# facebookresearch/gtn

Measured on AMD Instinct MI355X. Metric: CTC forward+backward losses/sec (T=1000, C=256), higher is better.
Workload: dtype f32; 1 GPU; BASELINE config C3: compose(ctc_target, emissions)+forwardScore CTC loss fwd+bwd, T=1000, C=256, U=100, batch=512 per GPU; global_batch=512, parallelism=dp1 (utterance sharding, all_gather of losses), rccl_ranks=0

## Files before the change

### gtn_amd/__init__.py

```python
from . import _capi
from .api import make_api, load_txt as _load_txt

_lib = _capi.load()
_api = make_api(_lib)

Graph = _api.Graph
Batch = _api.Batch
epsilon = _api.epsilon
negate = _api.negate
add = _api.add
subtract = _api.subtract
subtract_into = getattr(_api, "subtract_into", None)
compose = _api.compose
intersect = _api.intersect
forward_score = _api.forward_score
viterbi_score = _api.viterbi_score
viterbi_path = _api.viterbi_path
backward = _api.backward
scalar_graph = _api.scalar_graph
linear_graph = _api.linear_graph
linear_graph_n = _api.linear_graph_n
equal = _api.equal
isomorphic = _api.isomorphic
items = _api.items
items_to_device = _api.items_to_device
grads_to_device = _api.grads_to_device
parallel_for = _api.parallel_for
clone = _api.clone
project_input = _api.project_input
project_output = _api.project_output
closure = _api.closure
concat = _api.concat
union = _api.union
remove = _api.remove
sample = _api.sample
rand_equivalent = _api.rand_equivalent
load = _api.load
save = _api.save
loadtxt = _api.loadtxt
savetxt = _api.savetxt
write_dot = _api.write_dot
draw = _api.draw
backend = _api.backend
device_count = _api.device_count
synchronize = _api.synchronize
set_device = _api.set_device
set_stream = _api.set_stream
compose_mode = _api.compose_mode
memory_stats = _api.memory_stats
empty_cache = _api.empty_cache
prof_enable = _api.prof_enable
prof_reset = _api.prof_reset
prof_get = _api.prof_get
prof_names = _api.prof_names
debug_symbolic_route = _api.debug_symbolic_route
debug_viterbi_ties = _api.debug_viterbi_ties
debug_tie_ranks = _api.debug_tie_ranks
debug_align_stats = getattr(_api, "debug_align_stats", None)


def load_txt(text):
    return _load_txt(_api, text)


__version__ = _lib.gtnx_version().decode()


def _shutdown():
    try:
        _lib.gtnx_set_stream(None)
        _lib.gtnx_synchronize()
        _lib.gtnx_empty_cache()
    except Exception:
        pass


import atexit as _atexit

_atexit.register(_shutdown)
```

### gtn_amd/_capi.py

```python
import ctypes as C
import os

c_graph = C.c_void_p
c_graph_p = C.POINTER(C.c_void_p)
c_i32_p = C.POINTER(C.c_int)
c_i64_p = C.POINTER(C.c_int64)
c_u8_p = C.POINTER(C.c_uint8)
c_f32_p = C.POINTER(C.c_float)

GRAD_FN = C.CFUNCTYPE(C.c_int, C.c_void_p, c_graph_p, C.c_int, c_graph)
CTX_FREE = C.CFUNCTYPE(None, C.c_void_p)

OK, INVALID_ARGUMENT, LOGIC_ERROR, RUNTIME_ERROR, OUT_OF_RANGE, DEVICE_ERROR = range(6)

_SIGS = {
    "gtnx_set_device": [C.c_int],
    "gtnx_get_device": [c_i32_p],
    "gtnx_set_stream": [C.c_void_p],
    "gtnx_compose_mode": [C.c_int, C.POINTER(C.c_int)],
    "gtnx_synchronize": [],
    "gtnx_memory_stats": [C.POINTER(C.c_uint64), C.POINTER(C.c_uint64)],
    "gtnx_empty_cache": [],
    "gtnx_reclaim": [],
    "gtnx_graph_create": [C.c_int, c_graph_p],
# ... 41 lines not shown
    "gtnx_graph_id": [c_graph, C.POINTER(C.c_size_t)],
    "gtnx_graph_create_op": [c_graph_p, C.c_int, GRAD_FN, C.c_void_p, CTX_FREE, c_graph_p],
    "gtnx_graph_num_inputs": [c_graph, c_i64_p],
    "gtnx_graph_get_input": [c_graph, C.c_int, c_graph_p],
    "gtnx_graph_set_inputs": [c_graph, c_graph_p, C.c_int],
    "gtnx_graph_set_grad_fn": [c_graph, GRAD_FN, C.c_void_p, CTX_FREE],
    "gtnx_graph_has_grad_fn": [c_graph, c_i32_p],
    "gtnx_scalar_graph": [C.c_float, C.c_int, c_graph_p],
    "gtnx_linear_graph": [C.c_int, C.c_int, C.c_int, c_graph_p],
    "gtnx_linear_graph_n": [C.c_int, C.c_int, C.c_int, C.c_int, C.c_void_p, c_graph_p],
    "gtnx_linear_graph_borrow_n": [C.c_int, C.c_int, C.c_int, C.c_int, C.c_void_p, c_graph_p],
    "gtnx_negate": [c_graph, c_graph_p],
    "gtnx_add": [c_graph, c_graph, c_graph_p],
    "gtnx_subtract": [c_graph, c_graph, c_graph_p],
    "gtnx_compose": [c_graph, c_graph, c_graph_p],
    "gtnx_intersect": [c_graph, c_graph, c_graph_p],
    "gtnx_forward_score": [c_graph, c_graph_p],
    "gtnx_viterbi_score": [c_graph, c_graph_p],
    "gtnx_viterbi_path": [c_graph, c_graph_p],
    "gtnx_negate_n": [c_graph_p, C.c_int, c_graph_p],
    "gtnx_add_n": [c_graph_p, C.c_int, c_graph_p, C.c_int, c_graph_p],
    "gtnx_subtract_n": [c_graph_p, C.c_int, c_graph_p, C.c_int, c_graph_p],
    "gtnx_compose_n": [c_graph_p, C.c_int, c_graph_p, C.c_int, c_graph_p],
    "gtnx_intersect_n": [c_graph_p, C.c_int, c_graph_p, C.c_int, c_graph_p],
    "gtnx_forward_score_n": [c_graph_p, C.c_int, c_graph_p],
    "gtnx_viterbi_score_n": [c_graph_p, C.c_int, c_graph_p],
    "gtnx_viterbi_path_n": [c_graph_p, C.c_int, c_graph_p],
    "gtnx_items_n": [c_graph_p, C.c_int, C.c_void_p],
    "gtnx_items_device_n": [c_graph_p, C.c_int, C.c_void_p],
    "gtnx_grads_device_n": [c_graph_p, C.c_int, C.c_void_p, C.c_void_p],
    "gtnx_grads_bind_device_n": [c_graph_p, C.c_int, C.c_void_p, C.c_void_p],
    "gtnx_clone": [c_graph, C.c_int, c_graph_p],
    "gtnx_concat": [c_graph_p, C.c_int, c_graph_p],
    "gtnx_closure": [c_graph, c_graph_p],
    "gtnx_union": [c_graph_p, C.c_int, c_graph_p],
    "gtnx_batch_from_graphs": [c_graph_p, C.c_int, c_graph_p],
    "gtnx_batch_ctc_targets": [C.c_void_p, C.c_void_p, C.c_int, C.c_int, C.c_int, c_graph_p],
    "gtnx_batch_asg_force_align": [C.c_void_p, C.c_void_p, C.c_int, c_graph, C.c_int, c_graph_p],
    "gtnx_batch_linear": [C.c_int, C.c_int, C.c_int, C.c_int, C.c_void_p, C.c_int, c_graph_p],
    "gtnx_batch_destroy": [c_graph],
    "gtnx_batch_size": [c_graph, c_i32_p],
    "gtnx_batch_get": [c_graph, C.c_int, c_graph_p],
    "gtnx_batch_negate": [c_graph, c_graph_p],
    "gtnx_batch_add": [c_graph, c_graph, c_graph_p],
    "gtnx_batch_subtract": [c_graph, c_graph, c_graph_p],
    "gtnx_batch_subtract_into": [c_graph, c_graph, C.c_void_p, c_graph_p],
    "gtnx_batch_compose": [c_graph, c_graph, c_graph_p],
    "gtnx_batch_intersect": [c_graph, c_graph, c_graph_p],
    "gtnx_batch_forward_score": [c_graph, c_graph_p],
    "gtnx_batch_viterbi_score": [c_graph, c_graph_p],
    "gtnx_batch_viterbi_path": [c_graph, c_graph_p],
    "gtnx_batch_viterbi_align": [c_graph, C.c_void_p, C.c_void_p, C.c_int64, C.c_void_p, C.c_void_p],
    "gtnx_batch_align_stats": [c_i64_p, c_i64_p],
    "gtnx_batch_backward": [c_graph, C.c_int],
    "gtnx_batch_items": [c_graph, C.c_void_p],
    "gtnx_batch_items_device": [c_graph, C.c_void_p],
    "gtnx_batch_grads_bind_device": [c_graph, C.c_void_p, C.c_void_p],
    "gtnx_batch_grads_device": [c_graph, C.c_void_p, C.c_void_p],
    "gtnx_backward": [c_graph, C.c_int],
    "gtnx_backward_with_grad": [c_graph, c_graph, C.c_int],
    "gtnx_backward_n": [c_graph_p, C.c_int, C.c_int],
    "gtnx_equal": [c_graph, c_graph, c_i32_p],
    "gtnx_isomorphic": [c_graph, c_graph, c_i32_p],
    "gtnx_remove": [c_graph, C.c_int, C.c_int, c_graph_p],
    "gtnx_graph_load_buffer": [C.c_void_p, C.c_size_t, c_graph_p],
    "gtnx_parallel_enter": [],
    "gtnx_parallel_leave": [],
    "gtnx_parallel_flush": [],
    "gtnx_prof_enable": [C.c_int],
    "gtnx_prof_reset": [],
    "gtnx_prof_get": [C.c_char_p, C.POINTER(C.c_double), c_i64_p, C.POINTER(C.c_double)],
    "gtnx_prof_names": [C.c_char_p, C.c_size_t],
    "gtnx_debug_symbolic_route": [c_graph, C.c_int, c_i32_p],
    "gtnx_debug_route_name": [C.c_int, C.c_char_p, C.c_size_t],
    "gtnx_debug_viterbi_ties": [c_i64_p, c_i64_p],
    "gtnx_debug_tie_ranks": [c_graph, C.c_void_p, C.c_void_p, C.c_void_p],
    "gtnx_comm_create": [c_i32_p, C.c_int, C.POINTER(C.c_void_p)],
    "gtnx_comm_destroy": [C.c_void_p],
    "gtnx_comm_size": [C.c_void_p, c_i32_p],
    "gtnx_comm_all_gather_f32": [C.c_void_p, C.POINTER(C.c_void_p), C.POINTER(C.c_void_p), C.c_int64],
    "gtnx_comm_all_reduce_sum_f32": [C.c_void_p, C.POINTER(C.c_void_p), C.c_int64],
}

_RESTYPE = {
    "gtnx_last_error": (C.c_char_p, []),
    "gtnx_version": (C.c_char_p, []),
    "gtnx_backend": (C.c_char_p, []),
    "gtnx_device_count": (C.c_int, []),
}

ALL_SYMBOLS = sorted(list(_SIGS) + list(_RESTYPE))


def default_library_path():
    return os.path.join(os.path.dirname(os.path.abspath(__file__)), "lib", "libgtn_amd.so")


def load(path=None):
    path = path or default_library_path()
    if not os.path.exists(path):
        raise ImportError(
            f"gtn_amd: native library not found at {path}. Build it with "
            "`python -c 'import __graft_entry__ as g; g.build()'` (hipcc, gfx950). "
            "There is no CPU fallback."
        )
    lib = C.CDLL(path, mode=C.RTLD_GLOBAL if hasattr(C, "RTLD_GLOBAL") else 0)
# ... 17 lines not shown
```

### gtn_amd/api.py

```python
import ctypes as C
import types

import numpy as np

from . import _capi

_EXC = {
    _capi.INVALID_ARGUMENT: ValueError,
    _capi.LOGIC_ERROR: RuntimeError,
    _capi.RUNTIME_ERROR: RuntimeError,
    _capi.OUT_OF_RANGE: IndexError,
    _capi.DEVICE_ERROR: RuntimeError,
}


class GtnError(RuntimeError):
    pass


def _is_seq(x):
    return isinstance(x, (list, tuple))


def make_api(lib):
# ... 635 lines not shown

        def viterbi_align(self, labels_out, tokens_out=None, scores_out=None, frames=None, row_stride=None):
            n = len(self)
            stride = row_stride
            for t in (labels_out, tokens_out):
                if t is None or not hasattr(t, "data_ptr"):
                    continue
                if t.element_size() != 4 or t.dim() != 2 or t.shape[0] < n or (t.shape[1] > 1 and t.stride(1) != 1):
                    raise ValueError("viterbi_align: outputs must be int32 tensors [B, T] with contiguous rows")
                if stride is not None and t.stride(0) != stride:
                    raise ValueError("viterbi_align: labels_out and tokens_out must have the same row stride")
                stride = t.stride(0)
            if stride is None:
                raise ValueError("viterbi_align: a device address needs row_stride")
            fr = None if frames is None else np.ascontiguousarray(frames, dtype=np.int32)
            if fr is not None and fr.shape != (n,):
                raise ValueError("viterbi_align: one frame count per element")
            check(lib.gtnx_batch_viterbi_align(self._h, fr.ctypes.data if fr is not None else None,
                                               _as_dev_ptr(labels_out), int(stride),
                                               _as_dev_ptr(tokens_out) if tokens_out is not None else None,
                                               _as_dev_ptr(scores_out) if scores_out is not None else None))

    ns.Batch = Batch

    def _batch_fn(cfn, *args):
        h = C.c_void_p()
        check(cfn(*[a._h for a in args], C.byref(h)))
        return Batch._from_handle(h.value)

    def _with_batches(plain, cfn):
        def f(*args, **kw):
            if args and all(isinstance(a, Batch) for a in args) and not kw:
                return _batch_fn(cfn, *args)
            return plain(*args, **kw)
        f.__doc__ = plain.__doc__
        f.__name__ = getattr(plain, "__name__", "f")
        return f

    if hasattr(lib, "gtnx_batch_negate"):
        for _name in ("negate", "add", "subtract", "compose", "intersect", "forward_score", "viterbi_score",
                      "viterbi_path"):
            setattr(ns, _name, _with_batches(getattr(ns, _name), getattr(lib, "gtnx_batch_" + _name)))

    def subtract_into(a, b, items_device):
        h = C.c_void_p()
        check(lib.gtnx_batch_subtract_into(a._h, b._h, _as_dev_ptr(items_device), C.byref(h)))
        r = Batch._from_handle(h.value)
        r._keep = items_device
        return r

    if hasattr(lib, "gtnx_batch_subtract_into"):
        ns.subtract_into = subtract_into

    _plain_backward = ns.backward

    def backward(g, grad_or_retain=None, retain_graph=False):
        if isinstance(g, Batch):
            r = grad_or_retain if isinstance(grad_or_retain, bool) else retain_graph
            check(lib.gtnx_batch_backward(g._h, int(bool(r))))
            return
        return _plain_backward(g, grad_or_retain, retain_graph)

    ns.backward = backward

    def parallel_for(fn, iterable):
        for i in iterable:
            fn(i)

    ns.parallel_for = parallel_for

    def backend():
        return lib.gtnx_backend().decode()

    def device_count():
        return lib.gtnx_device_count()

    def synchronize():
        check(lib.gtnx_synchronize())

    def set_device(i):
        check(lib.gtnx_set_device(int(i)))

    def set_stream(stream):
        check(lib.gtnx_set_stream(int(stream) if stream else None))

    def compose_mode(mode):
        prev = C.c_int()
        check(lib.gtnx_compose_mode(int(mode), C.byref(prev)))
        return prev.value

    def memory_stats():
        r, u = C.c_uint64(), C.c_uint64()
        check(lib.gtnx_memory_stats(C.byref(r), C.byref(u)))
        return {"reserved": r.value, "in_use": u.value}

    def prof_enable(on=True):
        check(lib.gtnx_prof_enable(int(bool(on))))

    def prof_reset():
        check(lib.gtnx_prof_reset())

    def prof_get(name):
        ms, n, b = C.c_double(), C.c_int64(), C.c_double()
        check(lib.gtnx_prof_get(name.encode(), C.byref(ms), C.byref(n), C.byref(b)))
        return {"total_ms": ms.value, "launches": n.value, "algorithmic_bytes": b.value}

# ... 74 lines not shown
```

### gtn_amd/criteria/ctc_criterion.h

```cpp
#pragma once

#include <chrono>
#include <cstdint>
#include <vector>

#include "gtn/gtn.h"

namespace gtn {
namespace criteria {

inline Graph ctcTargetGraph(const std::vector<int>& target, int blank = 0, bool calcGrad = true) {
  const int L = 2 * (int)target.size() + 1;
  std::vector<uint8_t> st(L, 0), ac(L, 0);
  std::vector<int> src, dst, lab;
  src.reserve(3 * L);
  dst.reserve(3 * L);
  lab.reserve(3 * L);
  for (int l = 0; l < L; l++) {
    const int idx = (l - 1) / 2;
    st[l] = l == 0;
    ac[l] = l == L - 1 || l + 2 == L;
    const int label = l % 2 ? target[idx] : blank;
    src.push_back(l), dst.push_back(l), lab.push_back(label);
    if (l > 0) src.push_back(l - 1), dst.push_back(l), lab.push_back(label);
    if (l % 2 && l > 1 && label != target[idx - 1]) src.push_back(l - 2), dst.push_back(l), lab.push_back(label);
  }
  Graph ctc(calcGrad);
  detail::check(gtnx_graph_add_nodes(ctc.handle(), L, st.data(), ac.data()));
  detail::check(gtnx_graph_add_arcs(ctc.handle(), (int)src.size(), src.data(), dst.data(), lab.data(), lab.data(), nullptr));
  ctc.arcSort();
  return ctc;
}

struct CtcStepTimes {
  double build = 0, linear = 0, intersect = 0, forward = 0, backward = 0;
};

inline void ctcLossBatch(
    const void* emissions,
    const int* labels,
    const int* lengths,
    int B,
    int T,
    int C,
    int blank,
    void* lossDev,
    void* gradDev,
    bool targetGrad = true,
    CtcStepTimes* times = nullptr,
    Batch* targetsOut = nullptr) {
  auto now = [] { return std::chrono::steady_clock::now(); };
  auto ms = [](auto a, auto b) { return std::chrono::duration<double, std::milli>(b - a).count(); };
  auto t0 = now();
  Batch ctcs = Batch::ctcTargets(labels, lengths, B, blank, targetGrad);
  auto t1 = now();
  Batch ems = Batch::linear(B, T, C, emissions, gradDev != nullptr, true);
  std::vector<int64_t> off(B);
  for (int b = 0; b < B; ++b) off[b] = (int64_t)b * T * C;
  if (gradDev) ems.bindGrads(gradDev, off.data());
  auto t2 = now();
  Batch comp = batched::intersect(ctcs, ems);
  auto t3 = now();
  Batch score = batched::forwardScore(comp);
  Batch norm = batched::forwardScore(ems);
  Batch losses = batched::subtract(norm, score, lossDev);
  auto t4 = now();
  if (gradDev) batched::backward(losses);
  auto t5 = now();
  if (times) *times = {ms(t0, t1), ms(t1, t2), ms(t2, t3), ms(t3, t4), ms(t4, t5)};
  losses.itemsToDevice(lossDev);
  if (gradDev) ems.gradsToDevice(gradDev, off.data());
  if (targetsOut) *targetsOut = std::move(ctcs);
}

inline void ctcLossBatch(
    const void* emissions,
    const std::vector<std::vector<int>>& targets,
    int T,
    int C,
    int blank,
    void* lossDev,
    void* gradDev,
    bool targetGrad = true,
    CtcStepTimes* times = nullptr) {
  std::vector<int> flat, len;
  for (auto& t : targets) {
    flat.insert(flat.end(), t.begin(), t.end());
    len.push_back((int)t.size());
  }
  ctcLossBatch(emissions, flat.data(), len.data(), (int)targets.size(), T, C, blank, lossDev, gradDev, targetGrad, times);
}

inline void ctcAlignBatch(
    const void* emissions,
    const int* targets,
    const int* lengths,
    int B,
    int T,
    int C,
    int blank,
    const int* frames,
    void* labels,
    void* tokens,
    void* scores) {
  Batch ctcs = Batch::ctcTargets(targets, lengths, B, blank, false);
  Batch ems = Batch::linear(B, T, C, emissions, false, true);
  Batch comp = batched::intersect(ctcs, ems);
  batched::viterbiAlign(comp, static_cast<int*>(labels), T, static_cast<int*>(tokens), static_cast<float*>(scores), frames);
}

}
}
```

### gtn_amd/csrc/band.hip

```cpp
#include <hip/hip_runtime.h>

#include <algorithm>
#include <cstdlib>
#include <stdexcept>
#include <type_traits>

#include "kernels.h"

#ifdef GTNX_BAND_TIMING
__device__ long long g_band_timing[256];
#endif

namespace gtnx {
namespace {

constexpr float NEGF = -1.0e30f;
constexpr float DEADF = -1.0e29f;
constexpr float LOG2E = 1.44269504088896340736f;
constexpr double LN2 = 0.693147180559945309417;
constexpr int BW = 256;
constexpr int WG = 512;
constexpr int WGB = 768;
constexpr int NBE = 5;
constexpr int NBG = 7;
// ... 256 lines not shown
        }
      }
    }
  }
};

struct BandLds {
  int CS;
  int o_ering, o_aring, o_oring, o_snode, o_misc, total;
};
__host__ __device__ inline BandLds band_lds(int C, int K, int NSmax, bool backward) {
  BandLds L;
  L.CS = C + 4;
  int o = 0;
  L.o_ering = o;
  o += (backward ? NBGE : NBE) * K * L.CS;
  o = (o + 3) & ~3;
  L.o_aring = o;
  o += backward ? NBE * K * NSmax : 0;
  o = (o + 3) & ~3;
  L.o_oring = o;
  o += backward ? max(NBG * K * NSmax, 2 * C) : 0;
  o = (o + 3) & ~3;
  L.o_snode = o;
  o += backward ? 512 : 0;
  L.o_misc = o;
  o += 160 + 32 + 8 + 2 * NBE * K * 4 + 40 * K + 8 + 512;
  L.total = o;
  return L;
}
struct BandMisc {
  double *offr, *red, *find, *aofr;
  float *bndr, *fin, *lsep;
};
template <int K>
__device__ __forceinline__ BandMisc band_misc(float* lds, const BandLds& L) {
  BandMisc m;
  m.offr = reinterpret_cast<double*>(lds + L.o_misc);
  m.red = m.offr + 80;
  m.find = m.red + 16;
  m.aofr = m.find + 4;
  m.bndr = lds + L.o_misc + 200 + 2 * NBE * K * 4;
  m.fin = m.bndr + 40 * K;
  m.lsep = m.fin + 8;
  return m;
}

__device__ __forceinline__ float wave_max_of(const float* v, int n) {
  float mx = v[0];
  for (int j = 1; j < n; ++j) mx = fmaxf(mx, v[j]);
  return wave_max(mx);
}

template <int NPL, bool UNIT, int K, bool VEC>
__global__ __launch_bounds__(WG) void band_forward_kernel(const BandPair* __restrict__ pairs, int NSmax) {
#define GTNX_BAND_PAIR pairs[blockIdx.x]
#include "band_forward_body.inc"
#undef GTNX_BAND_PAIR
}
template <int NPL, bool UNIT, int K, bool VEC>
__global__ __launch_bounds__(WG) void band_forward_one_kernel(BandPair one, int NSmax) {
#define GTNX_BAND_PAIR one
#include "band_forward_body.inc"
#undef GTNX_BAND_PAIR
}

__device__ __forceinline__ BandPair band_patched(BandPair P, const BandPatch& pt) {
  if (pt.on) {
    const int b = P.bidx;
    P.delta = pt.delta + b;
    P.delta_norm = pt.delta_norm ? pt.delta_norm + b : nullptr;
    P.rowlse = pt.rowlse ? pt.rowlse + int64_t(b) * pt.M : nullptr;
    P.norm = nullptr;
    P.em_copy = nullptr;
    P.grad_em = pt.grad_em ? pt.grad_em + int64_t(b) * pt.A : nullptr;
    P.grad_fixed = pt.grad_fixed ? pt.grad_fixed + P.goff : nullptr;
  }
  return P;
}
template <int NPL, bool UNIT, bool GRADG, int K, bool VEC, bool BIG>
__global__ __launch_bounds__(WGB, BIG ? 3 : 6) void band_backward_kernel(const BandPair* __restrict__ pairs, int NSmax, BandPatch patch) {
#define GTNX_BAND_PAIR band_patched(pairs[blockIdx.x], patch)
#include "band_backward_body.inc"
#undef GTNX_BAND_PAIR
}
template <int NPL, bool UNIT, bool GRADG, int K, bool VEC, bool BIG>
__global__ __launch_bounds__(WGB, BIG ? 3 : 6) void band_backward_one_kernel(BandPair one, int NSmax) {
#define GTNX_BAND_PAIR one
#include "band_backward_body.inc"
#undef GTNX_BAND_PAIR
}


__global__ __launch_bounds__(512) void ctc_targets_kernel(const CtcTargetArgs* __restrict__ args, int blank) {
  const CtcTargetArgs a = args[blockIdx.x];
  __shared__ __attribute__((aligned(16))) int tl[256 + 4];
  __shared__ __attribute__((aligned(16))) int tk[256 + 4];
  const int N = a.N, U = (N - 1) >> 1, m = threadIdx.x;
  if (m < 260) {
    const int v = m < U ? a.labels[m] : 0x7fffffff;
    tl[m] = v;
    tk[m] = (m > 0 && m < U && v != a.labels[m - 1]) ? 1 : 0;
  }
  __syncthreads();
  if (m >= N) return;
  const bool odd = (m & 1) != 0;
  const int my = odd ? tl[(m - 1) >> 1] : blank;
  const int skip = odd ? tk[(m - 1) >> 1] : 0;
  const int mi = (m - 1) >> 1;
  const int before = odd ? mi : (m >> 1);
  int rank = 0, skips = 0;
  for (int o = 0; o < U; o += 4) {
    const gtnx_i4 l4 = *reinterpret_cast<const gtnx_i4*>(tl + o), k4 = *reinterpret_cast<const gtnx_i4*>(tk + o);
    const int lo[4] = {l4.x, l4.y, l4.z, l4.w}, ko[4] = {k4.x, k4.y, k4.z, k4.w};
#pragma unroll
    for (int k = 0; k < 4; ++k) {
      const bool front = o + k < before;
      rank += (lo[k] < my || (lo[k] == my && front)) ? 1 : 0;
      skips += front ? ko[k] : 0;
    }
  }
  rank += blank < my ? U + 1 : (blank == my ? (m + 1) >> 1 : 0);
  const int base = (m > 0 ? 2 * m - 1 : 0) + skips;
  GTNX_G BandNode* nd = const_cast<GTNX_G BandNode*>(a.nodes);
  nd[m].lab = my;
  nd[m].aid[0] = base;
  nd[m].aid[1] = m > 0 ? base + 1 : -1;
  nd[m].aid[2] = skip ? base + 2 : -1;
  a.nflags[m] = uint8_t((m == 0 ? NF_START : 0) | (m + 2 >= N ? NF_ACCEPT : 0));
  a.snode[rank] = m;
  a.slab[rank] = my;
  if (m == N - 1 && a.n_arcs) a.n_arcs[0] = base + 1 + (m > 0 ? 1 : 0) + skip;
}

__global__ __launch_bounds__(512) void band_viterbi_kernel(const BandDecode* __restrict__ pairs) {
  const BandDecode P = pairs[blockIdx.x];
  const int T = P.T, C = P.C, N = P.N, NS = P.NS;
  extern __shared__ float lds[];
  const float NINF = -__builtin_inff();
  float* a0 = lds;
  float* a1 = lds + 516;
  float* stage = lds + 1032;
  const int m = threadIdx.x;
  const GTNX_G gtnx_i4* nodes = reinterpret_cast<const GTNX_G gtnx_i4*>(P.nodes);
  int lab = 0;
  float wi[3] = {NINF, NINF, NINF};
  bool accept = false, start = false;
  if (m < N) {
    const gtnx_i4 q = nodes[m];
    lab = q.x >= 0 ? q.x : 0;
    const int a[3] = {q.y, q.z, q.w};
#pragma unroll
    for (int k = 0; k < 3; ++k)
      if (a[k] >= 0) wi[k] = P.w ? P.w[a[k]] : 0.0f;
    const uint8_t f = P.nflags[m];
    start = (f & NF_START) != 0;
    accept = (f & NF_ACCEPT) != 0;
  }
  if (m < 2) a0[m] = a1[m] = NINF;
  a0[2 + m] = start ? 0.0f : NINF;
  a1[2 + m] = NINF;
  int tie = 0;
  const int R = max(1, min(64, P.stage_floats / C));
  float* cur = a0;
  float* nxt = a1;
  __syncthreads();
  for (int t0 = 0; t0 < T; t0 += R) {
    const int rows = min(R, T - t0);
    for (int e = threadIdx.x; e < rows * C; e += blockDim.x) stage[e] = P.em[int64_t(t0) * C + e];
    __syncthreads();
    for (int i = 0; i < rows; ++i) {
      const float e = stage[i * C + lab];
      const float c0 = cur[2 + m] + (wi[0] + e), c1 = cur[1 + m] + (wi[1] + e), c2 = cur[m] + (wi[2] + e);
      float best = c0;
      int k = 0;
      if (c1 > best) best = c1, k = 1;
      if (c2 > best) best = c2, k = 2;
      if (best > NINF && ((k != 0 && c0 == best) || (k != 1 && c1 == best) || (k != 2 && c2 == best))) tie = 1;
      if (m < NS) P.bp[int64_t(t0 + i) * NS + m] = uint8_t(best > NINF ? k : 3);
      nxt[2 + m] = m < N ? best : NINF;
      __syncthreads();
      float* sw = cur;
      cur = nxt;
      nxt = sw;
    }
  }
// ... 292 lines not shown
    P.path_arc[t] = arc;
    P.path_lab[t] = q.x;
    P.path_w[t] = (arc >= 0 && P.w ? P.w[arc] : 0.0f) + P.em[int64_t(t) * C + (q.x >= 0 ? q.x : 0)];
  }
}

__global__ __launch_bounds__(512) void asg_fal_targets_kernel(const AsgFalArgs* __restrict__ args, int NL) {
  const AsgFalArgs a = args[blockIdx.x];
  __shared__ int lab[512];
  const int U = a.U, m = threadIdx.x;
  int my = -1;
  if (m >= 1 && m <= U) my = a.labels[m - 1];
  lab[m] = my;
  __syncthreads();
  if (m > U) return;
  GTNX_G BandNode* nd = const_cast<GTNX_G BandNode*>(a.nodes);
  nd[m].lab = my;
  nd[m].aid[0] = m >= 1 ? 2 * m - 1 : -1;
  nd[m].aid[1] = m >= 1 ? 2 * m - 2 : -1;
  nd[m].aid[2] = -1;
  a.nflags[m] = uint8_t((m == 0 ? NF_START : 0) | (m == U ? NF_ACCEPT : 0));
  if (m >= 1) {
    int rank = 0;
    for (int o = 1; o <= U; ++o) {
      const int lo = lab[o];
      rank += (lo < my || (lo == my && o < m)) ? 1 : 0;
    }
    a.snode[rank] = m;
    a.slab[rank] = my;
    const int step = m == 1 ? my : NL + my * NL + lab[m - 1];
    const int self = NL + my * NL + my;
    a.arc_map[2 * m - 2] = step;
    a.arc_map[2 * m - 1] = self;
    a.w[2 * m - 2] = a.trans_w[step];
    a.w[2 * m - 1] = a.trans_w[self];
  }
}
__global__ void asg_fal_scatter_kernel(const float* __restrict__ g, const int* __restrict__ maps,
                                       const int64_t* __restrict__ tab, float* __restrict__ trans_grad) {
  const int64_t* e = tab + int64_t(blockIdx.y) * 3;
  const int64_t n = e[2];
  const float* gb = g + e[0];
  const int* mb = maps + e[1];
  for (int64_t i = int64_t(blockIdx.x) * blockDim.x + threadIdx.x; i < n; i += int64_t(gridDim.x) * blockDim.x)
    if (mb[i] >= 0 && gb[i] != 0.0f) atomicAdd(trans_grad + mb[i], gb[i]);
}

template <class K>
void big_lds(K kern) {
  (void)hipFuncSetAttribute(reinterpret_cast<const void*>(kern), hipFuncAttributeMaxDynamicSharedMemorySize, 160 * 1024 - 512);
}

template <int NPL, int K, bool VEC>
void launch_fwd2(const BandPair* d, const BandPair* one, int n, int ns, size_t lds, bool unit, hipStream_t st) {
  static std::atomic<uint64_t> done{0};
  if (gtnx_first_on_device first{done}) {
    big_lds(band_forward_kernel<NPL, true, K, VEC>);
    big_lds(band_forward_kernel<NPL, false, K, VEC>);
    if constexpr (NPL == 1 && VEC) {
      big_lds(band_forward_one_kernel<NPL, true, K, VEC>);
      big_lds(band_forward_one_kernel<NPL, false, K, VEC>);
    }
  }
  if constexpr (NPL == 1 && VEC) {
    if (one) {
      if (unit) hipLaunchKernelGGL((band_forward_one_kernel<NPL, true, K, VEC>), dim3(1), dim3(WG), lds, st, *one, ns);
      else hipLaunchKernelGGL((band_forward_one_kernel<NPL, false, K, VEC>), dim3(1), dim3(WG), lds, st, *one, ns);
      return;
    }
  }
  if (unit) hipLaunchKernelGGL((band_forward_kernel<NPL, true, K, VEC>), dim3(n), dim3(WG), lds, st, d, ns);
  else hipLaunchKernelGGL((band_forward_kernel<NPL, false, K, VEC>), dim3(n), dim3(WG), lds, st, d, ns);
}
template <int NPL, int K>
void launch_fwd(const BandPair* d, const BandPair* one, int n, int ns, size_t lds, bool unit, bool vec, hipStream_t st) {
  if (vec) launch_fwd2<NPL, K, true>(d, one, n, ns, lds, unit, st);
  else launch_fwd2<NPL, K, false>(d, one, n, ns, lds, unit, st);
}
template <int NPL, int K, bool VEC, bool BIG>
void launch_bwd3(const BandPair* d, const BandPair* one, int n, int ns, size_t lds, bool unit, bool gradg, hipStream_t st,
                 const BandPatch& pt) {
  constexpr bool ONE = NPL == 1 && VEC && !BIG;
  static std::atomic<uint64_t> done{0};
  if (gtnx_first_on_device first{done}) {
    big_lds(band_backward_kernel<NPL, true, true, K, VEC, BIG>);
    big_lds(band_backward_kernel<NPL, true, false, K, VEC, BIG>);
    big_lds(band_backward_kernel<NPL, false, true, K, VEC, BIG>);
    big_lds(band_backward_kernel<NPL, false, false, K, VEC, BIG>);
    if constexpr (ONE) {
      big_lds(band_backward_one_kernel<NPL, true, true, K, VEC, BIG>);
      big_lds(band_backward_one_kernel<NPL, true, false, K, VEC, BIG>);
      big_lds(band_backward_one_kernel<NPL, false, true, K, VEC, BIG>);
      big_lds(band_backward_one_kernel<NPL, false, false, K, VEC, BIG>);
    }
  }
  if constexpr (ONE) {
    if (one) {
      if (unit) {
        if (gradg) hipLaunchKernelGGL((band_backward_one_kernel<NPL, true, true, K, VEC, BIG>), dim3(1), dim3(WGB), lds, st, *one, ns);
        else hipLaunchKernelGGL((band_backward_one_kernel<NPL, true, false, K, VEC, BIG>), dim3(1), dim3(WGB), lds, st, *one, ns);
      } else {
        if (gradg) hipLaunchKernelGGL((band_backward_one_kernel<NPL, false, true, K, VEC, BIG>), dim3(1), dim3(WGB), lds, st, *one, ns);
        else hipLaunchKernelGGL((band_backward_one_kernel<NPL, false, false, K, VEC, BIG>), dim3(1), dim3(WGB), lds, st, *one, ns);
      }
      return;
    }
  }
  if (unit) {
    if (gradg) hipLaunchKernelGGL((band_backward_kernel<NPL, true, true, K, VEC, BIG>), dim3(n), dim3(WGB), lds, st, d, ns, pt);
    else hipLaunchKernelGGL((band_backward_kernel<NPL, true, false, K, VEC, BIG>), dim3(n), dim3(WGB), lds, st, d, ns, pt);
  } else {
    if (gradg) hipLaunchKernelGGL((band_backward_kernel<NPL, false, true, K, VEC, BIG>), dim3(n), dim3(WGB), lds, st, d, ns, pt);
    else hipLaunchKernelGGL((band_backward_kernel<NPL, false, false, K, VEC, BIG>), dim3(n), dim3(WGB), lds, st, d, ns, pt);
  }
}
template <int NPL, int K>
void launch_bwd(const BandPair* d, const BandPair* one, int n, int ns, size_t lds, bool unit, bool gradg, bool vec, bool big,
                hipStream_t st, const BandPatch& pt) {
  if constexpr (K == 2) {
    if (big) {
      if (vec) launch_bwd3<NPL, K, true, true>(d, one, n, ns, lds, unit, gradg, st, pt);
      else launch_bwd3<NPL, K, false, true>(d, one, n, ns, lds, unit, gradg, st, pt);
      return;
    }
  }
  if (vec) launch_bwd3<NPL, K, true, false>(d, one, n, ns, lds, unit, gradg, st, pt);
  else launch_bwd3<NPL, K, false, false>(d, one, n, ns, lds, unit, gradg, st, pt);
}

constexpr size_t LDS_TWO = 78 * 1024;
constexpr size_t LDS_ONE = 156 * 1024;

}

int band_block_rows(int C, int max_NS, bool backward);
static int band_backward_lds_stride(int K, int max_NS) { return K == 4 ? (max_NS + 15) / 16 * 16 : max_NS; }
int band_max_nodes() { return 512; }
int band_max_labels() { return 1024; }
int band_min_labels() { return 4; }
int band_npl(int max_nodes) { return max_nodes <= 256 ? 1 : 2; }
int band_row_stride(int N, int) { return (N + 3) / 4 * 4; }
#ifndef GTNX_FWD_SHIFT_ROWS
#define GTNX_FWD_SHIFT_ROWS 4
#endif
int band_forward_lgrn(int C) {
  const int K = band_block_rows(C, 0, false);
  return K >= GTNX_FWD_SHIFT_ROWS ? (GTNX_FWD_SHIFT_ROWS == 8 ? 3 : 2) : (K >= 4 ? 2 : 1);
}
int band_block_rows(int C, int max_NS, bool backward) {
  for (int k = backward ? 4 : 8; k >= 2; k /= 2) {
    if (k * C > 2048 || k * max_NS > 2048) continue;
    if (backward && k > 2 && (k * C > 1024 || k * max_NS > 1024)) continue;
    const int ns_lds = backward ? band_backward_lds_stride(k, max_NS) : max_NS;
    if (4 * size_t(band_lds(C, k, ns_lds, backward).total) + 64 <= LDS_TWO) return k;
  }
  if (4 * size_t(band_lds(C, 2, max_NS, backward).total) + 64 <= LDS_ONE) return 2;
  return 0;
}

bool band_one_ok(int npl, int C, int max_NS, bool vec, bool backward) {
  if (npl != 1 || !vec) return false;
  if (!backward) return true;
  const int K = band_block_rows(C, max_NS, true);
  return !(K * C > 1024 || K * max_NS > 1024);
}
void launch_band_forward(const BandPair* d_pairs, int n, int npl, int C, int max_NS, bool unit, bool vec, hipStream_t st,
                         const BandPair* one) {
  if (n <= 0) return;
  if (one && (n != 1 || !band_one_ok(npl, C, max_NS, vec, false))) throw std::logic_error("band.hip: not a single-pair launch");
  const int K = band_block_rows(C, 0, false);
  const size_t lds = 4 * size_t(band_lds(C, K, max_NS, false).total) + 64;
  if (npl == 1) {
    if (K == 8) launch_fwd<1, 8>(d_pairs, one, n, max_NS, lds, unit, vec, st);
    else if (K == 4) launch_fwd<1, 4>(d_pairs, one, n, max_NS, lds, unit, vec, st);
    else launch_fwd<1, 2>(d_pairs, one, n, max_NS, lds, unit, vec, st);
  } else {
    if (K == 8) launch_fwd<2, 8>(d_pairs, one, n, max_NS, lds, unit, vec, st);
    else if (K == 4) launch_fwd<2, 4>(d_pairs, one, n, max_NS, lds, unit, vec, st);
    else launch_fwd<2, 2>(d_pairs, one, n, max_NS, lds, unit, vec, st);
  }
}

void launch_band_backward(const BandPair* d_pairs, int n, int npl, int C, int max_NS, bool unit, bool gradg, bool vec,
                          hipStream_t st, const BandPair* one, const BandPatch* patch) {
  if (n <= 0) return;
  if (one && patch) throw std::logic_error("band.hip: a patched launch reads a device table");
  BandPatch pt{};
  if (patch) pt = *patch;
  if (one && (n != 1 || !band_one_ok(npl, C, max_NS, vec, true))) throw std::logic_error("band.hip: not a single-pair launch");
  const int K = band_block_rows(C, max_NS, true);
  const bool big = K * C > 1024 || K * max_NS > 1024;
  const int ns_lds = band_backward_lds_stride(K, max_NS);
  const size_t lds = 4 * size_t(band_lds(C, K, ns_lds, true).total) + 64;
  if (npl == 1) {
    if (K == 4) launch_bwd<1, 4>(d_pairs, one, n, ns_lds, lds, unit, gradg, vec, big, st, pt);
    else launch_bwd<1, 2>(d_pairs, one, n, ns_lds, lds, unit, gradg, vec, big, st, pt);
  } else {
    if (K == 4) throw std::logic_error("band.hip: four rows per block with two nodes per lane");
    launch_bwd<2, 2>(d_pairs, one, n, ns_lds, lds, unit, gradg, vec, big, st, pt);
  }
}

template <int NPL>
static void launch_viterbi_wave(const BandDecode* d_pairs, int n, int ranked, hipStream_t st) {
  if (ranked) hipLaunchKernelGGL((band_viterbi_wave_kernel<NPL, true>), dim3(n), dim3(64), 0, st, d_pairs);
  else hipLaunchKernelGGL((band_viterbi_wave_kernel<NPL, false>), dim3(n), dim3(64), 0, st, d_pairs);
}
bool band_viterbi_wave_ok(int max_nodes, int max_labels, int vec) {
  static const bool force_wg = std::getenv("GTNX_VITERBI_WG") != nullptr;
  return !force_wg && vec && max_nodes <= 512 && max_labels <= VBLK;
}
void launch_band_viterbi(const BandDecode* d_pairs, int n, int stage_floats, int max_nodes, int max_labels, int vec,
                         hipStream_t st, int ranked) {
  if (n <= 0) return;
  if (band_viterbi_wave_ok(max_nodes, max_labels, vec)) {
    if (max_nodes <= 64) launch_viterbi_wave<1>(d_pairs, n, ranked, st);
    else if (max_nodes <= 128) launch_viterbi_wave<2>(d_pairs, n, ranked, st);
    else if (max_nodes <= 256) launch_viterbi_wave<4>(d_pairs, n, ranked, st);
    else launch_viterbi_wave<8>(d_pairs, n, ranked, st);
    return;
  }
  if (ranked) return;
  static std::atomic<uint64_t> done{0};
  if (gtnx_first_on_device first{done}) big_lds(band_viterbi_kernel);
  hipLaunchKernelGGL(band_viterbi_kernel, dim3(n), dim3(512), 4 * size_t(1032 + stage_floats) + 64, st, d_pairs);
}

void launch_asg_fal_targets(const AsgFalArgs* d_args, int n, int n_labels, hipStream_t st) {
  if (n > 0) hipLaunchKernelGGL(asg_fal_targets_kernel, dim3(n), dim3(512), 0, st, d_args, n_labels);
}
void launch_asg_fal_scatter(const float* g, const int* maps, const int64_t* tab, int n_seq, int64_t longest, float* trans_grad,
                            hipStream_t st) {
// ... 10 lines not shown
```

### gtn_amd/csrc/band_backward_body.inc

```
  constexpr int RNk = K >= 4 ? 4 : K;
  constexpr int NP = K / RNk;
  const BandPair P = GTNX_BAND_PAIR;
  const int T = P.T, C = P.C, NS = P.NS;
  extern __shared__ float lds[];
  const BandLds L = band_lds(C, K, NSmax, true);
  float* ering = lds + L.o_ering;
  float* aring = lds + L.o_aring;
  float* oring = lds + L.o_oring;
  int* snode = reinterpret_cast<int*>(lds + L.o_snode);
  const BandMisc M = band_misc<K>(lds, L);
  float* lser = M.lsep;
  const int CS = L.CS;
  const int wv = __builtin_amdgcn_readfirstlane(threadIdx.x >> 6);
  const bool sweeper = wv < 4;
  const int l = threadIdx.x & 63;
  const int nblocks = (T + K - 1) / K;
  const int nticks = nblocks + 5;
  const GTNX_G double* ao = P.aoff;
  const double z2 = uniform(ao[0]);
  const bool dead = !(z2 > double(DEADF));
  const float ds = uniform(P.delta[0]);
  const bool want_em = P.grad_em != nullptr;
  GTNX_TM_INIT(128);
  constexpr bool SPLIT = !BIG && K >= 2 && GTNX_BWD_SPLIT;
  const float dn_k = P.delta_norm ? uniform(P.delta_norm[0]) : 0.0f;
  float* const rnorm_k = lser + NBG * K;
  auto rows_of_k = [&](int c) { return c < nblocks ? min(K, T - c * K) : 0; };
  auto ring_start = [](int c, int M) { return ((c % M) + M) % M; };
  static_assert((NBGE & (NBGE - 1)) == 0, "the emission ring's position is a mask");
  auto ge_of = [](int c) { return int(unsigned(c) & unsigned(NBGE - 1)); };
  auto ring_step = [](int& v, int M) { v = v + 1 == M ? 0 : v + 1; };
  struct RowSumRegs {
    float in[NPL];
    gtnx_f4 hot[NPL];
  };
  auto rowsum_init = [&](RowSumRegs& R) {
#pragma unroll
    for (int q = 0; q < NPL; ++q) {
      const int mb = 256 * q + 4 * l;
      R.in[q] = mb < NSmax ? 1.0f : 0.0f;
      float hm[4];
#pragma unroll
      for (int k = 0; k < 4; ++k) {
        const int m = mb + k;
        int lab = -1;
        if (m < P.N) lab = P.nodes[m].lab;
        settle(lab);
        hm[k] = (P.hot >= 0 && lab == P.hot) ? 1.0f : 0.0f;
      }
      R.hot[q] = gtnx_f4{hm[0], hm[1], hm[2], hm[3]};
    }
  };
  auto rowsum_do = [&](const RowSumRegs& R, int c, int cg , int r, auto steady_tag) -> float {
    constexpr bool STEADY = decltype(steady_tag)::value;
    if (!want_em || (K < 4 && r >= K)) return 0.0f;
    if constexpr (!STEADY) {
      if (r >= rows_of_k(c)) return 0.0f;
    }
    const bool dead_r = STEADY ? false : dead;
    const float* ob = oring + (cg * K + r) * NSmax;
    gtnx_f4 v[NPL];
#pragma unroll
    for (int q = 0; q < NPL; ++q) v[q] = *reinterpret_cast<const gtnx_f4*>(ob + min(256 * q + 4 * l, NSmax - 4));
    const float em_hot = ering[(ge_of(c) * K + r) * CS + max(P.hot, 0)];
    const float ls_hot = lser[cg * K + r];
    float all = (v[0].x * R.in[0] + v[0].y * R.in[0]) + (v[0].z * R.in[0] + v[0].w * R.in[0]);
    float hotp = (v[0].x * R.hot[0].x + v[0].y * R.hot[0].y) + (v[0].z * R.hot[0].z + v[0].w * R.hot[0].w);
#pragma unroll
    for (int q = 1; q < NPL; ++q) {
      all += (v[q].x * R.in[q] + v[q].y * R.in[q]) + (v[q].z * R.in[q] + v[q].w * R.in[q]);
      hotp += (v[q].x * R.hot[q].x + v[q].y * R.hot[q].y) + (v[q].z * R.hot[q].z + v[q].w * R.hot[q].w);
    }
    if (dead_r) all = hotp = 0.0f;
    wave_sum63x2(all, hotp);
    all = __int_as_float(__builtin_amdgcn_readlane(__float_as_int(all), 63));
    const bool have = all != 0.0f && !dead_r;
    const float f = have ? ds * __builtin_amdgcn_rcpf(all) : 1.0f;
    if (l == 63 && P.hot >= 0) {
// ... 349 lines not shown
            if (FULL || i < rows) {
#pragma unroll
              for (int j = 0; j < NPL; ++j) ob[i * NSmax + j] = postv[i][j];
            }
        }
        if (GRADG) {
#pragma unroll
          for (int j = 0; j < NPL; ++j)
#pragma unroll
            for (int k = 0; k < 3; ++k) acc[k][j] += accb[k][j] * gscale;
        }
        if (NPL == 1 ? l < 2 : l == 0) {
#pragma unroll
          for (int i = 0; i < K; ++i)
            if (FULL || i < rows) {
              float* bp = bnd_own + ((beta & 3) * K + i) * 2;
              if (NPL == 1) {
                bp[l] = qh[i][0];
              } else {
                bp[0] = qh[i][0];
                bp[1] = qh[i][NPL - 1];
              }
            }
        }
      };
      if constexpr (STEADY) {
        block(std::true_type{});
      } else if (beta >= 0 && beta < nblocks && !dead) {
        if (beta * K + K <= T) block(std::true_type{});
        else block(std::false_type{});
      }
      GTNX_TM(5);
      lds_barrier();
      GTNX_TM(6);
      GTNX_TM_TICK();
    };
    {
      const int s0 = min(RS4 ? 5 : 4, nticks), s1 = dead ? s0 : max(s0, min(nticks, T / K + lag));
      auto step_rings = [&]() { ring_step(bm5, NBE), ring_step(bm7, NBG), ring_step(rm7, NBG); };
      int tau = 0;
      for (; tau < s0; ++tau, step_rings()) tick(tau, std::false_type{});
      for (; tau < s1; ++tau, step_rings()) tick(tau, std::true_type{});
      for (; tau < nticks; ++tau, step_rings()) tick(tau, std::false_type{});
    }
    GTNX_TM_DUMP();
    if (GRADG && P.grad_fixed) {
#pragma unroll
      for (int j = 0; j < NPL; ++j)
#pragma unroll
        for (int k = 0; k < 3; ++k)
          if (g.ao[k][j] >= 0) P.grad_fixed[g.ao[k][j]] = dead ? 0.0f : acc[k][j];
    }
  } else if (wv < 8) {
    const bool soft = P.delta_norm != nullptr && P.rowlse != nullptr;
    lds_barrier();
    if constexpr (!BIG) {
      const int h = wv - 4, q = h & 1;
      auto rows_of = [&](int c) { return c < nblocks ? min(K, T - c * K) : 0; };
      auto tlo_of = [&](int c) { return T - c * K - rows_of(c); };
      DrainRegs dr_s;
      const int hid_s = threadIdx.x - BW;
      auto drain_upper = [&](int tau) {
        if constexpr (SPLIT) {
          if (tau >= 5) drain_block(dr_s, hid_s, tau - 5, (tau - 5) % NBG, std::integral_constant<int, KH>{}, std::integral_constant<int, K>{});
        }
      };
      if (h < 2) {
        Stage<16, 64> se;
        if constexpr (VEC) se.init_offsets(C, CS, K, l);
        auto issue_em = [&](int c, auto steady_tag) {
          constexpr bool ST = decltype(steady_tag)::value;
          const int rows = ST ? K : rows_of(c);
          se.template issue<VEC>(P.em + int64_t(T - c * K - rows) * C, rows * C, l);
        };
        auto land_em = [&](int c, auto steady_tag) {
          constexpr bool ST = decltype(steady_tag)::value;
          const int rows = ST ? K : rows_of(c);
          se.settle_all();
          GTNX_TM(4);
          if (rows <= 0) return;
          float* eb = ering + ge_of(c) * K * CS;
          if constexpr (VEC) {
            se.each_vec(rows * C, (K - rows) * CS, l, [&](int, int o, gtnx_f4 v4) {
              typedef float f2v __attribute__((ext_vector_type(2)));
              const f2v lo = f2v{v4.x, v4.y} * LOG2E, hi = f2v{v4.z, v4.w} * LOG2E;
              *reinterpret_cast<gtnx_f4*>(eb + o) = gtnx_f4{fmaxf(lo.x, NEGF), fmaxf(lo.y, NEGF), fmaxf(hi.x, NEGF), fmaxf(hi.y, NEGF)};
            });
          } else {
            se.template each<false>(rows * C, C, l, [&](int, int, int r, int col, gtnx_f4 v4) {
              eb[(rows - 1 - r) * CS + col] = em2(v4.x);
            });
          }
        };
        issue_em(q, std::false_type{});
        land_em(q, std::false_type{});
        issue_em(q + 2, std::false_type{});
        RowSum4Regs rs4;
        if constexpr (RS4) rowsum4_init(rs4);
        lds_barrier();
        if constexpr (SPLIT) drain_init(dr_s, hid_s);
        lds_barrier();
        int r7 = ring_start(-4, NBG);
        auto tick = [&](int tau, auto steady_tag) {
          constexpr bool ST = decltype(steady_tag)::value;
          GTNX_TM(0);
#ifndef GTNX_EXP_NO_STAGE
          if (((tau + 2) & 1) == q) {
// ... 107 lines not shown
      float* eb = ering + ge_of(c) * K * CS;
      if constexpr (VEC) {
        se.each_vec(rows * C, (K - rows) * CS, l, [&](int, int o, gtnx_f4 q) {
          *reinterpret_cast<gtnx_f4*>(eb + o) = gtnx_f4{em2(q.x), em2(q.y), em2(q.z), em2(q.w)};
        });
      } else {
        se.template each<false>(rows * C, C, l, [&](int, int, int r, int col, gtnx_f4 q) {
          eb[(rows - 1 - r) * CS + col] = em2(q.x);
        });
      }
    };
    auto land_rest = [&](int c) {
      const int rows = rows_of(c);
      sa.settle_all();
      asm volatile("" : "+v"(lse_s), "+v"(af_s));
      if (rows <= 0) return;
      float* ab = aring + (c % NBE) * K * NSmax;
      sa.each_vec(rows * NS, (K - rows) * NSmax, l, [&](int, int o, gtnx_f4 q) { *reinterpret_cast<gtnx_f4*>(ab + o) = q; });
      if (l < rows) lser[(c % NBG) * K + rows - 1 - l] = lse_s;
      if (l < 4 * rows) M.aofr[((c % NBE) * K) * 4 + l] = af_s;
    };
    issue(h);
    if (h == 0) {
      land_em(0);
      land_rest(0);
      issue(4);
    }
    if (h == 1) land_em(1);
    lds_barrier();
    lds_barrier();
    for (int tau = 0; tau < nticks; ++tau) {
      GTNX_TM(0);
#ifndef GTNX_EXP_NO_STAGE
      if (((tau + 1) & 3) == h) {
        land_rest(tau + 1);
        GTNX_TM(1);
        issue(tau + 5);
        GTNX_TM(2);
      }
      if (((tau + 2) & 3) == h) {
        land_em(tau + 2);
        GTNX_TM(1);
      }
#endif
      GTNX_TM(3);
      lds_barrier();
      GTNX_TM(6);
      GTNX_TM_TICK();
    }
    GTNX_TM_DUMP();
    }
  } else {
    const int hid = threadIdx.x - 2 * BW;
    const bool soft = P.delta_norm != nullptr && P.rowlse != nullptr;
    int* cls = reinterpret_cast<int*>(oring);
    for (int c = hid; c < 2 * C; c += BW) cls[c] = 0;
    lds_barrier();
    for (int i = hid; i < P.n_lab; i += BW) {
      const int lab = P.slab[i];
      snode[i] = P.snode[i];
      if (i == 0 || P.slab[i - 1] != lab) cls[lab] = i;
      if (i == P.n_lab - 1 || P.slab[i + 1] != lab) cls[C + lab] = i + 1;
    }
    lds_barrier();
    DrainRegs dr;
    drain_init(dr, hid);
    RowSumRegs rsr;
    if constexpr (SPLIT) rowsum_init(rsr);
    const int dw = wv - 8;
    lds_barrier();
    int d7 = ring_start(-5, NBG);
    for (int tau = 0; tau < nticks; ++tau, ring_step(d7, NBG)) {
      GTNX_TM(0);
#ifndef GTNX_EXP_NO_DRAIN
      if (tau >= 5) drain_block(dr, hid, tau - 5, d7, std::integral_constant<int, 0>{}, std::integral_constant<int, KH>{});
#endif
      if constexpr (SPLIT) {
        if (tau >= 4) rowsum_do(rsr, tau - 4, (tau - 4) % NBG, dw, std::false_type{});
      }
      GTNX_TM(3);
      lds_barrier();
      GTNX_TM(6);
      GTNX_TM_TICK();
    }
    GTNX_TM_DUMP();
  }
```

### gtn_amd/csrc/band_forward_body.inc

```
#ifndef GTNX_FWD_SHIFT_ROWS
#define GTNX_FWD_SHIFT_ROWS 4
#endif
  constexpr int RNk = K >= GTNX_FWD_SHIFT_ROWS ? GTNX_FWD_SHIFT_ROWS : (K >= 4 ? 4 : K);
  constexpr int NP = K / RNk;
  constexpr int D = 8 / K > GTNX_FWD_DEPTH ? 8 / K : GTNX_FWD_DEPTH;
  const BandPair P = GTNX_BAND_PAIR;
  const int T = P.T, C = P.C, NS = P.NS;
  extern __shared__ float lds[];
  const BandLds L = band_lds(C, K, NSmax, false);
  float* ering = lds + L.o_ering;
  const BandMisc M = band_misc<K>(lds, L);
  const int CS = L.CS;
  const int wv = __builtin_amdgcn_readfirstlane(threadIdx.x >> 6);
  const bool sweeper = wv < 4;
  const int l = threadIdx.x & 63;
  const int nblocks = (T + K - 1) / K;
  const int nticks = nblocks + 3;
  GTNX_TM_INIT(0);

  if (sweeper) {
    __builtin_amdgcn_s_setprio(1);
    const int w = wv;
    const int m0 = threadIdx.x * NPL;
    NodeRegs<NPL> g;
// ... 279 lines not shown
      constexpr int DC = GTNX_FWD_COPY_DEPTH < 8 / K ? 8 / K : GTNX_FWD_COPY_DEPTH;
      constexpr int R = DC + 1;
      Stage<8> sc[R];
      issue(sc[0], 0);
      land(sc[0], 0, 0, std::true_type{});
#pragma unroll
      for (int c = 1; c <= DC; ++c) issue(sc[c % R], c);
      lds_barrier();
      int t5 = 0;
      for (int tau0 = 0; tau0 < nticks; tau0 += R) {
#pragma unroll
        for (int d = 0; d < R; ++d) {
          const int tau = tau0 + d;
          if (tau >= nticks) break;
          GTNX_TM(0);
          const int n5 = t5 + 1 == NBE ? 0 : t5 + 1;
          sc[(d + 1) % R].settle_all();
          issue(sc[d % R], tau + 1 + DC);
          GTNX_TM(2);
          land(sc[(d + 1) % R], tau + 1, n5, std::true_type{});
          GTNX_TM(1);
          if (want_lse) {
            if (tau >= 1 && tau - 1 < nblocks) lse_b(tau - 1);
            if (tau < nblocks) lse_a(tau, t5);
          }
          t5 = n5;
          GTNX_TM(4);
          lds_barrier();
          GTNX_TM(6);
          GTNX_TM_TICK();
        }
      }
    };
    if (em_copy) {
      if (GTNX_FWD_COPY_ROTATE) run_copy();
      else run(std::true_type{});
    } else {
      run(std::false_type{});
    }
    if (hid < 16) M.red[hid] = normacc;
  }
  GTNX_TM_DUMP();
  lds_barrier();
  if (threadIdx.x == 0) {
    double Mx = double(NEGF);
    for (int k = 0; k < 4; ++k)
      if (M.fin[2 * k] > DEADF) Mx = fmax(Mx, M.find[k] + double(M.fin[2 * k]));
    const bool dead = !(Mx > double(DEADF));
    float S = 0.0f;
    for (int k = 0; k < 4; ++k)
      if (M.fin[2 * k] > DEADF) S += M.fin[2 * k + 1] * ex2(float(M.find[k] + double(M.fin[2 * k]) - Mx));
    const double z2 = dead ? double(NEGF) : Mx + double(lg2(S));
    P.aoff[0] = z2;
    P.score[0] = dead ? -__builtin_inff() : float(z2 * LN2);
    if (P.norm) {
      double n2 = 0.0;
      for (int k = 0; k < 16; ++k) n2 += M.red[k];
      P.norm[0] = n2 < double(DEADF) ? -__builtin_inff() : float(n2 * LN2);
    }
  }
```

### gtn_amd/csrc/batch.cpp

```cpp
#include "batch.h"

#include <algorithm>
#include <atomic>
#include <limits>
#include <unordered_map>
#include <unordered_set>

namespace gtnx {

namespace {

std::atomic<uint64_t> g_batch_seq{1};

struct CompMode {
  int old;
  CompMode() : old(compose_mode_hint(2)) {}
  ~CompMode() { compose_mode_hint(old); }
};

BatchP make_batch(Batch::Kind k, int n, bool cg) {
  auto b = std::make_shared<Batch>();
  b->kind = k;
  b->n = n;
  b->calc_grad = cg;
// ... 15 lines not shown
  Runtime& rt = Runtime::get();
  b.g_off.resize(size_t(b.n) + 1);
  b.g_off[0] = 0;
  for (int i = 0; i < b.n; ++i) b.g_off[size_t(i) + 1] = b.g_off[size_t(i)] + b.elem_size(i);
  const size_t bytes = sizeof(float) * size_t(b.g_off[size_t(b.n)]);
  if (b.dest) {
    b.g_mem = b.dest_mem;
    b.g_dev = b.dest;
    b.dest = nullptr;
    if (zero && bytes) HIP_CHECK(hipMemsetAsync(b.g_dev, 0, bytes, rt.stream()));
  } else {
    b.g_mem = zero ? rt.alloc_zero(bytes ? bytes : 4) : rt.alloc(bytes ? bytes : 4);
    b.g_dev = b.g_mem->as<float>();
  }
}

struct GradTarget {
  float* ptr = nullptr;
  DevMemP scratch;
};
GradTarget grad_target(Batch& b, bool zero) {
  GradTarget t;
  if (!b.g_dev) {
    alloc_grad(b, zero);
    t.ptr = b.g_dev;
    return t;
  }
  Runtime& rt = Runtime::get();
  const size_t bytes = sizeof(float) * size_t(b.g_off[size_t(b.n)]);
  t.scratch = zero ? rt.alloc_zero(bytes ? bytes : 4) : rt.alloc(bytes ? bytes : 4);
  t.ptr = t.scratch->as<float>();
  return t;
}
void add_scratch(Batch& b, const GradTarget& t) {
  if (!t.scratch) return;
  launch_vec_axpby(b.g_dev, t.ptr, nullptr, size_t(b.g_off[size_t(b.n)]), 1.0f, 0.0f, 1, Runtime::get().stream());
}

struct BScalarOp : BatchOp {
  ScalarKind kind;
  void backward(Batch& out) override {
    Runtime& rt = Runtime::get();
    for (size_t i = 0; i < inputs.size(); ++i) {
      Batch& in = *inputs[i];
      if (!in.calc_grad) continue;
      const float s = (kind == SK_NEGATE || (kind == SK_SUBTRACT && i == 1)) ? -1.0f : 1.0f;
      const bool have = in.g_dev != nullptr;
      if (!have) alloc_grad(in, false);
      launch_vec_axpby(in.g_dev, out.g_dev, nullptr, size_t(in.n), s, 0.0f, have ? 1 : 0, rt.stream());
    }
  }
};

struct BackwardPlan {
  std::unordered_map<Batch*, Batch*> lin;
  std::unordered_set<Batch*> fused;
};
thread_local BackwardPlan* t_plan = nullptr;
thread_local bool t_batch_retain = false;

struct BFsLinearOp : BatchOp {
  void backward(Batch& out) override {
    Batch& e = *inputs[0];
    if (!e.calc_grad) return;
    if (t_plan && e.nc_rowlse && !t_plan->lin.count(&e)) {
      t_plan->lin[&e] = &out;
      return;
    }
    run(out);
  }
  void run(Batch& out) {
    Batch& e = *inputs[0];
    Runtime& rt = Runtime::get();
    if (e.w_pend) e.w_pend->settle();
    const bool have = e.g_dev != nullptr;
    if (!have) alloc_grad(e, false);
    std::vector<LinArgs> args;
    args.resize(size_t(e.n));
    const size_t A = size_t(e.M) * size_t(e.C);
    for (int b = 0; b < e.n; ++b) {
      LinArgs& a = args[size_t(b)];
      a.w = e.w_dev + size_t(b) * A;
      a.M = e.M;
      a.C = e.C;
      a.out_score = nullptr;
      a.partial = nullptr;
      a.delta = out.g_dev + b;
      a.grad = e.g_dev + size_t(b) * A;
      a.accumulate = have ? 1 : 0;
    }
    DevMemP d = upload_vec(args);
    const bool vec_rows = e.C % 4 == 0 && e.C <= 1024 && (reinterpret_cast<uintptr_t>(e.w_dev) & 15) == 0 &&
                          (reinterpret_cast<uintptr_t>(e.g_dev) & 15) == 0;
    GTNX_PROF("linear_forward_grad", (have ? 12.0 : 8.0) * double(A) * e.n);
    launch_linear_backward(d->as<LinArgs>(), e.n, 0, vec_rows ? 1 : 0, rt.stream());
  }
};

struct BFsBandOp : BatchOp {
  std::vector<BandPair> pairs;
  DevMemP arena;
  DevMemP fwd_table;
  DevMemP through_acc;
  void backward(Batch& out) override {
    Batch& prod = *inputs[0];
    Batch& fx = *prod.fixed;
    Batch& ch = *prod.chain;
    Runtime& rt = Runtime::get();
    const float* delta = out.g_dev;
    if (through_acc || t_batch_retain) {
      const size_t n = size_t(prod.n);
      if (!through_acc) through_acc = rt.alloc_zero(sizeof(float) * (n ? n : 1));
      launch_vec_axpby(through_acc->as<float>(), out.g_dev, nullptr, n, 1.0f, 0.0f, 1, rt.stream());
      delta = through_acc->as<float>();
    }
    GradTarget ge, gf;
    if (ch.calc_grad) ge = grad_target(ch, false);
    if (fx.calc_grad) gf = grad_target(fx, fx.fal);
    Batch* lin_out = nullptr;
    if (t_plan && ch.calc_grad && !ge.scratch) {
      auto it = t_plan->lin.find(&ch);
      if (it != t_plan->lin.end() && !t_plan->fused.count(&ch)) {
        lin_out = it->second;
        t_plan->fused.insert(&ch);
      }
    }
    std::vector<std::pair<BandLaunchKey, BandPair>> tab;
    tab.reserve(pairs.size());
    double bytes = 0;
    const size_t A = size_t(ch.M) * size_t(ch.C);
    bool one_key = true;
    int max_ns = 0;
    for (int b = 0; b < prod.n; ++b) {
      BandPair p = pairs[size_t(b)];
      p.delta = delta + b;
      p.delta_norm = lin_out ? lin_out->g_dev + b : nullptr;
      p.rowlse = lin_out ? ch.nc_rowlse + size_t(b) * size_t(ch.M) : nullptr;
      p.norm = nullptr;
      p.grad_em = ge.ptr ? ge.ptr + size_t(b) * A : nullptr;
      p.grad_fixed = gf.ptr ? gf.ptr + fx.g_off[size_t(b)] : nullptr;
      tab.push_back({BandLaunchKey{p.C, band_npl(p.N), fx.fal ? 0 : 1, p.grad_fixed ? 1 : 0, band_vec_ok(p)}, p});
      one_key = one_key && tab.back().first == tab.front().first;
      max_ns = std::max(max_ns, p.NS);
      bytes += 4.0 * p.T * p.C * (p.grad_em ? 2 : 1) + 4.0 * double(p.T + 1) * p.NS +
               (p.grad_fixed ? 4.0 * double(fx.elem_size(b)) : 0.0);
    }
    static const bool no_patch = std::getenv("GTNX_NO_BAND_PATCH") != nullptr;
    if (fwd_table && one_key && prod.n > 1 && !no_patch) {
      BandPatch pt{};
      pt.on = 1;
      pt.M = ch.M;
      pt.delta = delta;
      pt.delta_norm = lin_out ? lin_out->g_dev : nullptr;
      pt.rowlse = lin_out ? ch.nc_rowlse : nullptr;
      pt.grad_em = ge.ptr;
      pt.grad_fixed = gf.ptr;
      pt.A = int64_t(A);
      band_launch_patched(fwd_table, prod.n, tab.front().first, max_ns, pt, "band_forward_score_grad", bytes);
    } else {
      band_launch(tab, true, "band_forward_score_grad", bytes);
    }
    if (ch.calc_grad) add_scratch(ch, ge);
    if (fx.calc_grad) add_scratch(fx, gf);
    (void)rt;
  }
};


struct BFalOp : BatchOp {
  void backward(Batch& out) override {
    Graph& tr = out.trans;
    if (!tr.calc_grad() || !out.g_dev) return;
    Runtime& rt = Runtime::get();
    const int64_t A = tr.num_arcs();
    DevMemP gm = rt.alloc_zero(sizeof(float) * size_t(A ? A : 1));
    std::vector<int64_t> tab(size_t(out.n) * 3);
    int64_t longest = 0;
    for (int b = 0; b < out.n; ++b) {
      const int64_t len = out.g_off[size_t(b) + 1] - out.g_off[size_t(b)];
      tab[size_t(b) * 3 + 0] = out.g_off[size_t(b)];
      tab[size_t(b) * 3 + 1] = int64_t(out.map_off[size_t(b)] / sizeof(int));
      tab[size_t(b) * 3 + 2] = len;
      longest = std::max(longest, len);
    }
    DevMemP dt = upload_vec(tab);
    launch_asg_fal_scatter(out.g_dev, out.rec_mem->as<int>(), dt->as<int64_t>(), out.n, longest, gm->as<float>(), rt.stream());
    tr.add_grad_device(gm, gm->as<float>(), true);
  }
};

struct BFromGraphsOp : BatchOp {
  DevMemP passed;
  void backward(Batch& out) override {
    Batch& src = *inputs[0];
    Runtime& rt = Runtime::get();
    const size_t n = size_t(src.n);
    DevMemP delta = rt.alloc(sizeof(float) * (n ? n : 1));
    if (passed)
      launch_vec_axpby(delta->as<float>(), out.g_dev, passed->as<float>(), n, 1.0f, -1.0f, 0, rt.stream());
    else
      rt.d2d(delta->ptr, out.g_dev, sizeof(float) * n);
    if (retain) {
      if (!passed) passed = rt.alloc(sizeof(float) * (n ? n : 1));
      rt.d2d(passed->ptr, out.g_dev, sizeof(float) * n);
    }
    std::vector<Graph> roots;
// ... 29 lines not shown
    const size_t e = std::min(graphs.size(), i + 32);
    part->reserve(e - i);
    for (size_t k = i; k < e; ++k) part->push_back(std::move(graphs[k]));
    rt.defer_delete(part, [](void* q) { delete static_cast<std::vector<Graph>*>(q); }, e - i);
  }
  graphs.clear();
}

int64_t Batch::elem_size(int b) const {
  switch (kind) {
    case SCALAR: return 1;
    case LINEAR: return int64_t(M) * C;
    case CTC_TARGETS:
      if (fal) return 2 * int64_t(lab_off[size_t(b) + 1] - lab_off[size_t(b)]);
      return 3 * int64_t(2 * (lab_off[size_t(b) + 1] - lab_off[size_t(b)]) + 1);
    default: return 0;
  }
}

BatchP batch_from_graphs(std::vector<Graph> gs) {
  bool cg = false;
  for (auto& g : gs) cg |= g.calc_grad();
  BatchP b = make_batch(Batch::GRAPHS, int(gs.size()), cg);
  b->graphs = std::move(gs);
  b->materialised = true;
  return b;
}

namespace {
Graph ctc_target_graph_host(const int* t, int U, int blank, bool cg) {
  const int L = 2 * U + 1;
  std::vector<uint8_t> st(size_t(L), 0), ac(size_t(L), 0);
  std::vector<int> src, dst, lab;
  src.reserve(size_t(3 * L));
  dst.reserve(size_t(3 * L));
  lab.reserve(size_t(3 * L));
  for (int l = 0; l < L; ++l) {
    const int idx = (l - 1) / 2;
    st[size_t(l)] = l == 0;
    ac[size_t(l)] = l == L - 1 || l + 2 == L;
    const int label = l % 2 ? t[idx] : blank;
    src.push_back(l), dst.push_back(l), lab.push_back(label);
    if (l > 0) src.push_back(l - 1), dst.push_back(l), lab.push_back(label);
    if (l % 2 && l > 1 && label != t[idx - 1]) src.push_back(l - 2), dst.push_back(l), lab.push_back(label);
  }
  Graph g(cg);
  g.add_nodes(L, st.data(), ac.data());
  g.add_arcs(int(src.size()), src.data(), dst.data(), lab.data(), lab.data(), nullptr);
  g.arc_sort(false);
  return g;
}
}

BatchP batch_ctc_targets(const int* labels, const int* lengths, int n, int blank, bool calc_grad) {
  GTNX_HOST_T("batch.ctc_targets");
  if (n < 0) throw_invalid("[gtnx_batch_ctc_targets] negative batch size");
  BatchP b = make_batch(Batch::CTC_TARGETS, n, calc_grad);
  b->blank = blank;
  b->lab_off.resize(size_t(n) + 1);
  b->lab_off[0] = 0;
  for (int i = 0; i < n; ++i) {
    if (lengths[i] < 0) throw_invalid("[gtnx_batch_ctc_targets] negative length");
    b->lab_off[size_t(i) + 1] = b->lab_off[size_t(i)] + lengths[i];
    b->max_nodes = std::max(b->max_nodes, 2 * lengths[i] + 1);
  }
  const size_t total = size_t(b->lab_off[size_t(n)]);
  b->labels.assign(labels, labels + total);
  int mn = blank;
  b->max_label = blank;
  for (size_t i = 0; i < total; ++i) {
    b->max_label = std::max(b->max_label, labels[i]);
    mn = std::min(mn, labels[i]);
  }
  if (mn < 0 || b->max_nodes > band_max_nodes() || n == 0) {
    std::vector<Graph> gs;
    gs.reserve(size_t(n));
    for (int i = 0; i < n; ++i)
      gs.push_back(ctc_target_graph_host(labels + b->lab_off[size_t(i)], lengths[i], blank, calc_grad));
    return batch_from_graphs(std::move(gs));
  }
  Runtime& rt = Runtime::get();
  const size_t lab_bytes = align_up(sizeof(int) * (total ? total : 1), 256);
  const size_t arg_bytes = align_up(sizeof(CtcTargetArgs) * size_t(n), 256);
  size_t bytes = lab_bytes + arg_bytes;
  b->rec_off.resize(size_t(n));
  for (int i = 0; i < n; ++i) {
    const size_t N = size_t(2 * lengths[i] + 1);
    b->rec_off[size_t(i)] = bytes;
    bytes += align_up(sizeof(BandNode) * N, 64) + align_up(N, 64) + 2 * align_up(4 * N, 64) + 64;
  }
  b->rec_mem = rt.alloc(bytes);
  PinnedMemP pin = rt.alloc_pinned(lab_bytes + arg_bytes);
  std::memcpy(pin->ptr, labels, sizeof(int) * total);
  CtcTargetArgs* args = reinterpret_cast<CtcTargetArgs*>(static_cast<char*>(pin->ptr) + lab_bytes);
  for (int i = 0; i < n; ++i) {
    const size_t N = size_t(2 * lengths[i] + 1);
    char* base = b->rec_mem->as<char>(b->rec_off[size_t(i)]);
    CtcTargetArgs& a = args[size_t(i)];
    a.labels = b->rec_mem->as<int>() + b->lab_off[size_t(i)];
    a.nodes = reinterpret_cast<BandNode*>(base);
    base += align_up(sizeof(BandNode) * N, 64);
    a.nflags = reinterpret_cast<uint8_t*>(base);
    base += align_up(N, 64);
    a.snode = reinterpret_cast<int*>(base);
    base += align_up(4 * N, 64);
    a.slab = reinterpret_cast<int*>(base);
    base += align_up(4 * N, 64);
    a.n_arcs = reinterpret_cast<int*>(base);
    a.N = int(N);
    a.pad = 0;
  }
  rt.h2d_pinned(b->rec_mem->ptr, pin->ptr, lab_bytes + arg_bytes);
  launch_ctc_targets(reinterpret_cast<const CtcTargetArgs*>(b->rec_mem->as<char>(lab_bytes)), n, blank, rt.stream());
  return b;
}


BatchP batch_asg_force_align(const int* labels, const int* lengths, int n, Graph& transitions, int n_labels) {
  if (n < 0) throw_invalid("[gtnx_batch_asg_force_align] negative batch size");
  if (transitions.num_nodes() != int64_t(n_labels) + 1 || transitions.num_arcs() != int64_t(n_labels) * (n_labels + 1))
    throw_invalid("[gtnx_batch_asg_force_align] the transitions graph must have the asgTransitions(N) layout");
  BatchP b = make_batch(Batch::CTC_TARGETS, n, transitions.calc_grad());
  b->fal = true;
  b->trans = transitions;
  b->trans_labels = n_labels;
  b->lab_off.resize(size_t(n) + 1);
  b->lab_off[0] = 0;
  int max_u = 0;
  for (int i = 0; i < n; ++i) {
    if (lengths[i] < 0) throw_invalid("[gtnx_batch_asg_force_align] negative length");
    b->lab_off[size_t(i) + 1] = b->lab_off[size_t(i)] + lengths[i];
    max_u = std::max(max_u, lengths[i]);
  }
  b->max_nodes = max_u + 1;
  const size_t total = size_t(b->lab_off[size_t(n)]);
  b->labels.assign(labels, labels + total);
  int mn = 0;
  for (size_t i = 0; i < total; ++i) {
    b->max_label = std::max(b->max_label, labels[i]);
    mn = std::min(mn, labels[i]);
  }
  if (mn < 0 || b->max_label >= n_labels || b->max_nodes > band_max_nodes() || n == 0) {
    b->kind = Batch::GRAPHS;
    batch_materialise(*b);
    return b;
  }
  Runtime& rt = Runtime::get();
  std::vector<Weights*> ws{transitions.w.get()};
  ensure_weights_device_batch(ws);
  size_t bytes = align_up(sizeof(int) * (total ? total : 1), 256);
  b->rec_off.resize(size_t(n));
  b->w_off.resize(size_t(n));
  b->map_off.resize(size_t(n));
  for (int i = 0; i < n; ++i) {
    const size_t N = size_t(lengths[i]) + 1, A = 2 * size_t(lengths[i]);
    b->rec_off[size_t(i)] = bytes;
    bytes += align_up(sizeof(BandNode) * N, 64) + align_up(N, 64) + 2 * align_up(4 * N, 64);
    b->w_off[size_t(i)] = bytes;
    bytes += align_up(4 * (A ? A : 1), 64);
    b->map_off[size_t(i)] = bytes;
    bytes += align_up(4 * (A ? A : 1), 64);
  }
  b->rec_mem = rt.alloc(bytes);
  {
    PinnedMemP pin = rt.alloc_pinned(sizeof(int) * (total ? total : 1));
    std::memcpy(pin->ptr, labels, sizeof(int) * total);
// ... 255 lines not shown
          w.version++;
          gs.push_back(std::move(g));
        }
        break;
      }
      for (auto& in : x.op->inputs) batch_materialise(*in);
      if (auto* so = dynamic_cast<BScalarOp*>(x.op.get())) {
        std::vector<Graph> none;
        gs = op_scalar(so->kind, so->inputs[0]->graphs, so->inputs.size() > 1 ? so->inputs[1]->graphs : none);
      } else {
        gs = op_shortest_distance(x.op->inputs[0]->graphs, false);
      }
      break;
    }
  }
  if (x.kind != Batch::GRAPHS || x.fal) x.graphs = std::move(gs);
  x.materialised = true;
  if (x.g_dev && ((x.kind == Batch::CTC_TARGETS && !x.fal) || x.kind == Batch::LINEAR)) {
    for (int i = 0; i < x.n; ++i) x.graphs[size_t(i)].add_grad_device(x.g_mem, x.g_dev + x.g_off[size_t(i)], true);
    x.g_dev = nullptr;
    x.g_mem.reset();
  }
}

Graph batch_get(const BatchP& x, int i) {
  if (i < 0 || i >= x->n) throw_range("[gtnx_batch_get] element index out of range");
  batch_materialise(*x);
  return x->graphs[size_t(i)];
}

BatchP batch_compose(const BatchP& a, const BatchP& b, bool intersect) {
  const Batch *fx = nullptr, *ch = nullptr;
  bool chain_first = false;
  if (native(*a, Batch::CTC_TARGETS) && native(*b, Batch::LINEAR)) fx = a.get(), ch = b.get();
  if (native(*a, Batch::LINEAR) && native(*b, Batch::CTC_TARGETS)) fx = b.get(), ch = a.get(), chain_first = true;
  if (fx && a->n == b->n && ch->C >= band_min_labels() && ch->C <= band_max_labels() && fx->max_label < ch->C && ch->M <= (1 << 20)) {
    struct Op : BatchOp {
      void backward(Batch&) override {}
    };
    auto op = std::make_shared<Op>();
    op->inputs = {a, b};
    BatchP r = result(Batch::PRODUCT, a->n, op);
    r->fixed = chain_first ? b : a;
    r->chain = chain_first ? a : b;
    r->chain_first = chain_first;
    r->intersect = intersect;
    return r;
  }
  batch_materialise(*a);
  batch_materialise(*b);
  return batch_from_graphs(op_compose(a->graphs, b->graphs, intersect));
}

BatchP batch_shortest_distance(const BatchP& x, bool tropical) {
  GTNX_HOST_T("batch.shortest_distance");
  Runtime& rt = Runtime::get();
  if (!tropical && native(*x, Batch::PRODUCT) && !x->materialised) {
    Batch& fx = *x->fixed;
    Batch& ch = *x->chain;
    const int n = x->n, T = ch.M, C = ch.C;
    auto op = std::make_shared<BFsBandOp>();
    op->inputs = {x};
    const bool want_norm = ch.nc_norm == nullptr;
    size_t bytes = align_up(4 * size_t(n), 256);
    const size_t o_norm = bytes;
    bytes = align_up(bytes + 4 * size_t(n), 256);
    const size_t o_lse = bytes;
    bytes = align_up(bytes + 4 * size_t(n) * size_t(T > 0 ? T : 1), 256);
    std::vector<size_t> oo, ao;
    oo.resize(size_t(n));
    ao.resize(size_t(n));
    for (int b = 0; b < n; ++b) {
      const int Ub = fx.lab_off[size_t(b) + 1] - fx.lab_off[size_t(b)];
      const int N = fx.fal ? Ub + 1 : 2 * Ub + 1;
      const int ns = band_row_stride(N, band_npl(N));
      oo[size_t(b)] = bytes;
      bytes = align_up(bytes + 8 * (4 * size_t(T) + 16), 256);
      ao[size_t(b)] = bytes;
      bytes = align_up(bytes + 4 * size_t(T + 1) * size_t(ns), 256);
    }
    op->arena = rt.alloc(bytes);
    op->pairs.resize(size_t(n));
    std::vector<std::pair<BandLaunchKey, BandPair>> tab;
    tab.reserve(size_t(n));
    double abytes = 0;
    std::shared_ptr<PendingCopy> pend = ch.w_pend;
    std::unique_lock<std::mutex> pend_lock;
    bool fuse_copy = false;
    if (pend && !pend->done.load(std::memory_order_acquire)) {
      pend_lock = std::unique_lock<std::mutex>(pend->mu);
      fuse_copy = !pend->done.load(std::memory_order_relaxed) && pend->device == rt.device();
      const size_t A = size_t(T) * size_t(C);
      for (int b = 0; b < n && fuse_copy; ++b) fuse_copy = pend->src_of(ch.w_dev + size_t(b) * A) != nullptr;
      fuse_copy = fuse_copy && pend->segs.size() == size_t(n);
      if (!fuse_copy) {
        pend_lock.unlock();
        pend->settle();
      }
    }
    int64_t goff_run = 0;
    for (int b = 0; b < n; ++b) {
      BandPair& p = op->pairs[size_t(b)];
      p = BandPair{};
      const int U = fx.lab_off[size_t(b) + 1] - fx.lab_off[size_t(b)];
      const size_t N = fx.fal ? size_t(U) + 1 : size_t(2 * U + 1);
      char* base = fx.rec_mem->as<char>(fx.rec_off[size_t(b)]);
      p.nodes = reinterpret_cast<BandNode*>(base);
      base += align_up(sizeof(BandNode) * N, 64);
      p.nflags = reinterpret_cast<uint8_t*>(base);
      base += align_up(N, 64);
      p.snode = reinterpret_cast<int*>(base);
      base += align_up(4 * N, 64);
      p.slab = reinterpret_cast<int*>(base);
      p.n_lab = fx.fal ? U : int(N);
      p.w = fx.fal ? fx.rec_mem->as<float>(fx.w_off[size_t(b)]) : nullptr;
      p.em = ch.w_dev + size_t(b) * size_t(T) * size_t(C);
      p.N = int(N);
      p.T = T;
      p.C = C;
      p.NS = band_row_stride(p.N, band_npl(p.N));
      p.alpha = op->arena->as<float>(ao[size_t(b)]);
      p.aoff = op->arena->as<double>(oo[size_t(b)]);
      p.score = op->arena->as<float>(4 * size_t(b));
      if (want_norm) {
        p.norm = op->arena->as<float>(o_norm + 4 * size_t(b));
        p.rowlse = op->arena->as<float>(o_lse + 4 * size_t(b) * size_t(T));
      }
      p.hot = (!fx.fal && U + 1 >= 8) ? fx.blank : -1;
      p.lgrn = band_forward_lgrn(C);
      p.bidx = b;
      p.goff = goff_run;
      goff_run += int64_t(fx.elem_size(b));
      BandPair q = p;
      if (fuse_copy) {
        q.em = static_cast<const float*>(pend->src_of(p.em));
        q.em_copy = const_cast<float*>(p.em);
      }
      tab.push_back({BandLaunchKey{C, band_npl(q.N), fx.fal ? 0 : 1, 0, band_vec_ok(q)}, q});
      abytes += 4.0 * T * C + 4.0 * double(T + 1) * p.NS + (fuse_copy ? 4.0 * T * C : 0.0);
    }
    band_launch(tab, false, "band_forward_score", abytes, fuse_copy ? nullptr : &op->fwd_table);
    if (fuse_copy) pend->done.store(true, std::memory_order_release);
    if (want_norm) {
      ch.nc_mem = op->arena;
      ch.nc_norm = op->arena->as<float>(o_norm);
      ch.nc_rowlse = op->arena->as<float>(o_lse);
    }
    DevMemP arena = op->arena;
    BatchP r = result(Batch::SCALAR, n, op);
    r->v_mem = arena;
    r->v_dev = arena->as<float>();
    return r;
  }
  if (!tropical && native(*x, Batch::LINEAR) && !x->materialised && x->nc_norm) {
    auto op = std::make_shared<BFsLinearOp>();
    op->inputs = {x};
    BatchP r = result(Batch::SCALAR, x->n, op);
    r->v_mem = x->nc_mem;
    r->v_dev = x->nc_norm;
    return r;
  }
  if (!tropical && native(*x, Batch::LINEAR) && !x->materialised && x->n > 0 && x->M > 0) {
    if (x->w_pend) x->w_pend->settle();
    auto op = std::make_shared<BFsLinearOp>();
    op->inputs = {x};
    const int n = x->n;
    DevMemP res = rt.alloc(sizeof(float) * size_t(n) * 9);
    float* scal = res->as<float>();
    float* partial = scal + n;
    std::vector<LinArgs> args;
    args.resize(size_t(n));
    const size_t A = size_t(x->M) * size_t(x->C);
    for (int b = 0; b < n; ++b) {
      LinArgs& a = args[size_t(b)];
      a.w = x->w_dev + size_t(b) * A;
      a.M = x->M;
      a.C = x->C;
      a.out_score = scal + b;
      a.partial = partial + size_t(b) * 8;
      a.delta = nullptr;
      a.grad = nullptr;
      a.accumulate = 0;
    }
    DevMemP d = upload_vec(args);
    const bool vec_rows = x->C % 4 == 0 && x->C <= 1024 && (reinterpret_cast<uintptr_t>(x->w_dev) & 15) == 0 && (A % 4) == 0;
    {
      GTNX_PROF("linear_forward", 4.0 * double(A) * n);
      launch_linear_forward(d->as<LinArgs>(), n, 0, vec_rows ? 1 : 0, rt.stream());
    }
    BatchP r = result(Batch::SCALAR, n, op);
    r->v_mem = res;
    r->v_dev = scal;
    return r;
  }
  batch_materialise(*x);
  return batch_from_graphs(op_shortest_distance(x->graphs, tropical));
}

BatchP batch_viterbi_path(const BatchP& x) {
  batch_materialise(*x);
  return batch_from_graphs(op_viterbi_path(x->graphs));
}

namespace {
std::atomic<int64_t> g_align_fast{0}, g_align_fallback{0};

// ... 72 lines not shown
    for (int b = 0; b < n; ++b)
      if (frames[b] < 0 || frames[b] > T) throw_invalid("[gtnx_batch_viterbi_align] a frame count outside 0 .. T");
  if (ch.w_pend) ch.w_pend->settle();
  const int npl = align_npl(fx.max_nodes);
  const size_t plane = align_up((size_t(T) * size_t(npl) + 15) / 16 * 256 + 256, 256);
  DevMemP work = rt.alloc(plane * size_t(n));
  std::vector<AlignArgs> tab(static_cast<size_t>(n));
  double abytes = 0;
  for (int b = 0; b < n; ++b) {
    AlignArgs& a = tab[size_t(b)];
    a = AlignArgs{};
    const int* t = fx.labels.data() + fx.lab_off[size_t(b)];
    const int U = fx.lab_off[size_t(b) + 1] - fx.lab_off[size_t(b)];
    const size_t N = size_t(2 * U + 1);
    char* base = fx.rec_mem->as<char>(fx.rec_off[size_t(b)]);
    a.nodes = reinterpret_cast<BandNode*>(base);
    a.nflags = reinterpret_cast<uint8_t*>(base + align_up(sizeof(BandNode) * N, 64));
    a.em = ch.w_dev + size_t(b) * size_t(T) * size_t(C);
    a.bp = work->as<unsigned>(plane * size_t(b));
    a.labels = labels_dev + int64_t(b) * row_stride;
    a.tokens = tokens_dev ? tokens_dev + int64_t(b) * row_stride : nullptr;
    a.score = scores_dev ? scores_dev + b : nullptr;
    a.N = int(N);
    a.T = frames ? frames[b] : T;
    a.T_full = T;
    a.C = C;
    int p = 0;
    while (p + 1 < U && t[p] < t[p + 1]) ++p;
    a.p = p;
    abytes += 4.0 * a.T * C + 0.5 * double(a.T) * double(N) + 8.0 * a.T;
  }
  DevMemP d = upload_vec(tab);
  GTNX_PROF("band_viterbi_align", abytes);
  launch_band_align(d->as<AlignArgs>(), n, fx.max_nodes, rt.stream());
  g_align_fast.fetch_add(n);
}


namespace {
BatchP scalars_from_graphs(const BatchP& gsb) {
  Runtime& rt = Runtime::get();
  for (auto& g : gsb->graphs)
    if (g.num_arcs() != 1) return nullptr;
  auto op = std::make_shared<BFromGraphsOp>();
  op->inputs = {gsb};
  BatchP r = result(Batch::SCALAR, gsb->n, op);
  r->v_mem = rt.alloc(sizeof(float) * size_t(gsb->n ? gsb->n : 1));
  r->v_dev = r->v_mem->as<float>();
  items_device(gsb->graphs, r->v_dev);
  return r;
}
}

BatchP batch_scalar(ScalarKind k, const BatchP& a0, const BatchP& b0, void* items_dev) {
  BatchP a = a0, b = b0;
  const bool binary = k != SK_NEGATE;
  if (binary && a->n == b->n) {
    const bool an = a->kind == Batch::SCALAR && !a->materialised, bn = b->kind == Batch::SCALAR && !b->materialised;
    if (an && !bn && b->kind == Batch::GRAPHS) {
      if (BatchP w = scalars_from_graphs(b)) b = w;
    } else if (bn && !an && a->kind == Batch::GRAPHS) {
      if (BatchP w = scalars_from_graphs(a)) a = w;
    }
  }

  if (native(*a, Batch::SCALAR) && !a->materialised &&
      (!binary || (native(*b, Batch::SCALAR) && !b->materialised && b->n == a->n))) {
    Runtime& rt = Runtime::get();
    auto op = std::make_shared<BScalarOp>();
    op->kind = k;
    op->inputs = binary ? std::vector<BatchP>{a, b} : std::vector<BatchP>{a};
    BatchP r = result(Batch::SCALAR, a->n, op);
    if (items_dev) {
      r->v_dev = static_cast<float*>(items_dev);
    } else {
      r->v_mem = rt.alloc(sizeof(float) * size_t(a->n ? a->n : 1));
      r->v_dev = r->v_mem->as<float>();
    }
    launch_vec_axpby(r->v_dev, a->v_dev, binary ? b->v_dev : nullptr, size_t(a->n), k == SK_NEGATE ? -1.0f : 1.0f,
                     k == SK_SUBTRACT ? -1.0f : 1.0f, 0, rt.stream());
    return r;
  }
  batch_materialise(*a);
  std::vector<Graph> none;
  if (binary) batch_materialise(*b);
  BatchP r = batch_from_graphs(op_scalar(k, a->graphs, binary ? b->graphs : none));
  if (items_dev) batch_items_device(r, items_dev);
  return r;
}

void batch_backward(const BatchP& root, bool retain) {
  GTNX_HOST_T("batch.backward");
  if (root->tape_cleared)
    throw_invalid("[autograd::backward] Cannot Backward twice without retaining the graph.");
  if (root->materialised || !root->op || root->kind != Batch::SCALAR) {
    batch_materialise(*root);
    op_backward(root->graphs, nullptr, retain);
    return;
  }
  Runtime& rt = Runtime::get();
  std::vector<Batch*> order;
  std::unordered_set<Batch*> seen;
  std::vector<BatchP> hold;
  std::vector<BatchP> stack{root};
  while (!stack.empty()) {
    BatchP b = stack.back();
    stack.pop_back();
    if (!b->calc_grad || !seen.insert(b.get()).second) continue;
    hold.push_back(b);
    if (b->op) {
      order.push_back(b.get());
      for (auto& in : b->op->inputs) stack.push_back(in);
    }
  }
  std::sort(order.begin(), order.end(), [](Batch* a, Batch* b) { return a->op->seq > b->op->seq; });
  bool root_done = false;
  if (!root->g_dev) {
    alloc_grad(*root, false);
    auto* sop = dynamic_cast<BScalarOp*>(root->op.get());
    bool plain = sop != nullptr && !sop->inputs.empty() && sop->inputs.size() <= 2;
    if (plain)
      for (auto& in : sop->inputs) plain = plain && in->kind == Batch::SCALAR && !in->materialised && in->n == root->n;
    if (plain && sop->inputs.size() == 2 && sop->inputs[0].get() == sop->inputs[1].get()) plain = false;
    if (plain) {
      float* g[2] = {nullptr, nullptr};
      float sc[2] = {0.0f, 0.0f};
      int acc[2] = {0, 0};
      for (size_t i = 0; i < sop->inputs.size(); ++i) {
        Batch& in = *sop->inputs[i];
        if (!in.calc_grad) continue;
        sc[i] = (sop->kind == SK_NEGATE || (sop->kind == SK_SUBTRACT && i == 1)) ? -1.0f : 1.0f;
        acc[i] = in.g_dev != nullptr;
        if (!in.g_dev) alloc_grad(in, false);
        g[i] = in.g_dev;
      }
      launch_scalar_seed(root->g_dev, g[0], sc[0], acc[0], g[1], sc[1], acc[1], size_t(root->n), rt.stream());
      root_done = true;
    } else {
      launch_fill_f32(root->g_dev, 1.0f, size_t(root->n), rt.stream());
    }
  } else {
    DevMemP ones = rt.alloc(sizeof(float) * size_t(root->n ? root->n : 1));
    launch_fill_f32(ones->as<float>(), 1.0f, size_t(root->n), rt.stream());
    launch_vec_axpby(root->g_dev, ones->as<float>(), nullptr, size_t(root->n), 1.0f, 0.0f, 1, rt.stream());
  }
  std::vector<Batch*> from_graphs;
  BackwardPlan plan;
  t_plan = &plan;
  struct RetainScope {
    bool prev;
    explicit RetainScope(bool r) : prev(t_batch_retain) { t_batch_retain = r; }
    ~RetainScope() { t_batch_retain = prev; }
  } retain_scope(retain);
  try {
    for (Batch* b : order) {
      if (!b->g_dev) continue;
      if (root_done && b == root.get()) continue;
      if (auto* f = dynamic_cast<BFromGraphsOp*>(b->op.get())) {
        f->retain = retain;
        from_graphs.push_back(b);
        continue;
      }
      b->op->backward(*b);
    }
    for (auto& kv : plan.lin)
      if (!plan.fused.count(kv.first)) static_cast<BFsLinearOp*>(kv.second->op.get())->run(*kv.second);
  } catch (...) {
    t_plan = nullptr;
    throw;
  }
  t_plan = nullptr;
  for (Batch* b : seen)
    if ((b->materialised || b->leaf) && b->g_dev && !b->op) push_grads_to_graphs(*b);
  for (Batch* b : from_graphs) b->op->backward(*b);
  if (!retain)
    for (Batch* b : order) {
      if (b != root.get()) {
        b->g_dev = nullptr;
        b->g_mem.reset();
      }
      b->op.reset();
      b->tape_cleared = true;
    }
}

void batch_items_device(const BatchP& x, void* dev_out) {
  if (x->kind == Batch::SCALAR && !x->materialised) {
    if (static_cast<const void*>(x->v_dev) == dev_out) return;
    Runtime::get().d2d(dev_out, x->v_dev, sizeof(float) * size_t(x->n));
    return;
  }
  batch_materialise(*x);
  items_device(x->graphs, dev_out);
}
float batch_item_host(const BatchP& x, int i) {
  if (i < 0 || i >= x->n) throw_range("[gtnx_batch_get] element index out of range");
  if (!x->host_vals_valid) {
    x->host_vals.resize(size_t(x->n));
    if (x->host_ev) {
      Runtime::get().drain_until(x->host_ev);
      std::memcpy(x->host_vals.data(), x->host_pin->ptr, sizeof(float) * size_t(x->n));
      (void)hipEventDestroy(static_cast<hipEvent_t>(x->host_ev));
      x->host_ev = nullptr;
      x->host_pin.reset();
    } else {
      Runtime::get().d2h_sync(x->host_vals.data(), x->v_dev, sizeof(float) * size_t(x->n));
    }
    x->host_vals_valid = true;
  }
  return x->host_vals[size_t(i)];
}
void batch_prefetch_items(const BatchP& x) {
  if (!x || x->kind != Batch::SCALAR || x->materialised || x->host_vals_valid || x->host_ev || x->n <= 0 || !x->v_dev) return;
  Runtime& rt = Runtime::get();
  hipEvent_t ev;
  if (hipEventCreateWithFlags(&ev, hipEventDisableTiming) != hipSuccess) {
    (void)hipGetLastError();
// ... 57 lines not shown
```

### gtn_amd/csrc/batch.h

```cpp
#pragma once

#include <memory>
#include <vector>

#include "ops.h"

namespace gtnx {

struct Batch;
using BatchP = std::shared_ptr<Batch>;

struct BatchOp {
  uint64_t seq = 0;
  std::vector<BatchP> inputs;
  virtual void backward(Batch& out) = 0;
  virtual ~BatchOp() {}
};

struct Batch {
  enum Kind { GRAPHS, CTC_TARGETS, LINEAR, PRODUCT, SCALAR };
  Kind kind = GRAPHS;
  int n = 0;
  bool calc_grad = false;

// ... 5 lines not shown
    size_t begin, end;
  };
  std::vector<Origin> origins;
  void (*give_back)(const std::shared_ptr<void>& home, std::vector<Graph>* part) = nullptr;
  std::vector<float> host_vals;
  bool host_vals_valid = false;
  PinnedMemP host_pin;
  void* host_ev = nullptr;

  std::vector<int> labels, lab_off;
  int blank = 0;
  int max_label = -1, max_nodes = 0;
  DevMemP rec_mem;
  std::vector<size_t> rec_off;
  bool fal = false;
  Graph trans;
  int trans_labels = 0;
  std::vector<size_t> w_off, map_off;
  int M = 0, C = 0;
  DevMemP w_mem;
  float* w_dev = nullptr;
  std::shared_ptr<PendingCopy> w_pend;
  DevMemP nc_mem;
  float* nc_norm = nullptr;
  float* nc_rowlse = nullptr;
  BatchP fixed, chain;
  bool chain_first = false, intersect = false;
  DevMemP v_mem;
  float* v_dev = nullptr;

  std::shared_ptr<BatchOp> op;
  bool tape_cleared = false;
  DevMemP g_mem;
  float* g_dev = nullptr;
  std::vector<int64_t> g_off;
  DevMemP dest_mem;
  float* dest = nullptr;

  int64_t elem_size(int b) const;
  ~Batch();
};

BatchP batch_from_graphs(std::vector<Graph> gs);
BatchP batch_ctc_targets(const int* labels, const int* lengths, int n, int blank, bool calc_grad);
BatchP batch_asg_force_align(const int* labels, const int* lengths, int n, Graph& transitions, int n_labels);
BatchP batch_linear(int n, int M, int C, bool calc_grad, const void* dev, bool borrow);
BatchP batch_compose(const BatchP& a, const BatchP& b, bool intersect);
BatchP batch_shortest_distance(const BatchP& x, bool tropical);
BatchP batch_viterbi_path(const BatchP& x);
void batch_viterbi_align(const BatchP& x, const int* frames, int* labels_dev, int64_t row_stride, int* tokens_dev,
                         float* scores_dev);
void batch_align_stats(int64_t* fast, int64_t* fallback);
BatchP batch_scalar(ScalarKind k, const BatchP& a, const BatchP& b, void* items_dev = nullptr);
void batch_backward(const BatchP& root, bool retain);
void batch_items_host(const BatchP& x, float* out);
void batch_items_device(const BatchP& x, void* dev_out);
void batch_grads_device(const BatchP& x, void* dev_out, const int64_t* offsets);
void batch_grads_bind(const BatchP& x, void* dev_out, const int64_t* offsets);
Graph batch_get(const BatchP& x, int i);
float batch_item_host(const BatchP& x, int i);
void batch_prefetch_items(const BatchP& x);
BatchP batch_ctc_targets_from_graphs(const std::vector<Graph>& gs);
BatchP batch_linear_from_graphs(const std::vector<Graph>& gs);
void batch_materialise(Batch& x);

}
```

### gtn_amd/csrc/capi.cpp

```cpp
#include <atomic>
#include <chrono>
#include <condition_variable>
#include <cstdlib>
#include <cstring>
#include <mutex>
#include <string>
#include <vector>

#include "batch.h"
#include "ops.h"
#include "ops_internal.h"
#include "region.h"

#define GTNX_API extern "C" __attribute__((visibility("default")))

using namespace gtnx;

namespace {
thread_local std::string g_err;

gtnx_status_t fail(gtnx_status_t s, const std::string& m) {
  g_err = m;
  return s;
}
// ... 692 lines not shown
  });
}
GTNX_API gtnx_status_t gtnx_grads_bind_device_n(const gtnx_graph_t* g, int n, void* out, const int64_t* offsets) {
  return guard([&] {
    auto v = vec(g, n);
    grads_bind_device(v, out, offsets);
  });
}

GTNX_API gtnx_status_t gtnx_clone(gtnx_graph_t g, int projection, gtnx_graph_t* out) {
  return guard([&] {
    if (projection < 0 || projection > 2) throw_invalid("[gtnx_clone] projection must be 0, 1 or 2");
    std::vector<Graph> v{G(g)};
    *out = H(op_rational(RAT_CLONE, v, projection));
  });
}
GTNX_API gtnx_status_t gtnx_concat(const gtnx_graph_t* g, int n, gtnx_graph_t* out) {
  return guard([&] {
    auto v = vec(g, n);
    *out = H(op_rational(RAT_CONCAT, v, 0));
  });
}
GTNX_API gtnx_status_t gtnx_closure(gtnx_graph_t g, gtnx_graph_t* out) {
  return guard([&] {
    std::vector<Graph> v{G(g)};
    *out = H(op_rational(RAT_CLOSURE, v, 0));
  });
}
GTNX_API gtnx_status_t gtnx_union(const gtnx_graph_t* g, int n, gtnx_graph_t* out) {
  return guard([&] {
    auto v = vec(g, n);
    *out = H(op_rational(RAT_UNION, v, 0));
  });
}

GTNX_API gtnx_status_t gtnx_remove(gtnx_graph_t g, int ilabel, int olabel, gtnx_graph_t* out) {
  return guard([&] { *out = H(op_remove(G(g), ilabel, olabel)); });
}

namespace {
inline BatchP& BH(gtnx_batch_t h) {
  if (!h) throw_invalid("null batch handle");
  return *reinterpret_cast<BatchP*>(h);
}
inline gtnx_batch_t HB(BatchP b) { return reinterpret_cast<gtnx_batch_t>(new BatchP(std::move(b))); }
}
GTNX_API gtnx_status_t gtnx_batch_from_graphs(const gtnx_graph_t* g, int n, gtnx_batch_t* out) {
  return guard([&] { *out = HB(batch_from_graphs(vec(g, n, true))); });
}
GTNX_API gtnx_status_t gtnx_batch_ctc_targets(const int* labels, const int* lengths, int n, int blank, int cg,
                                              gtnx_batch_t* out) {
  return guard([&] { *out = HB(batch_ctc_targets(labels, lengths, n, blank, cg != 0)); });
}
GTNX_API gtnx_status_t gtnx_batch_asg_force_align(const int* labels, const int* lengths, int n, gtnx_graph_t transitions,
                                                  int n_labels, gtnx_batch_t* out) {
  return guard([&] { *out = HB(batch_asg_force_align(labels, lengths, n, G(transitions), n_labels)); });
}
GTNX_API gtnx_status_t gtnx_batch_linear(int n, int M, int N, int cg, const void* dev, int borrow, gtnx_batch_t* out) {
  return guard([&] { *out = HB(batch_linear(n, M, N, cg != 0, dev, borrow != 0)); });
}
GTNX_API gtnx_status_t gtnx_batch_destroy(gtnx_batch_t b) {
  return guard([&] {
    auto* p = reinterpret_cast<BatchP*>(b);
    if (!p) return;
    if (Runtime::initialized())
      Runtime::get().defer_delete(p, [](void* q) { delete static_cast<BatchP*>(q); },
                                  (*p && (*p)->materialised) ? size_t((*p)->n > 0 ? (*p)->n : 1) : 1);
    else
      delete p;
  });
}
GTNX_API gtnx_status_t gtnx_batch_size(gtnx_batch_t b, int* out) {
  return guard([&] { *out = BH(b)->n; });
}
GTNX_API gtnx_status_t gtnx_batch_get(gtnx_batch_t b, int i, gtnx_graph_t* out) {
  return guard([&] { *out = H(batch_get(BH(b), i)); });
}
GTNX_API gtnx_status_t gtnx_batch_negate(gtnx_batch_t a, gtnx_batch_t* out) {
  return guard([&] { *out = HB(batch_scalar(SK_NEGATE, BH(a), nullptr)); });
}
GTNX_API gtnx_status_t gtnx_batch_add(gtnx_batch_t a, gtnx_batch_t b, gtnx_batch_t* out) {
  return guard([&] { *out = HB(batch_scalar(SK_ADD, BH(a), BH(b))); });
}
GTNX_API gtnx_status_t gtnx_batch_subtract(gtnx_batch_t a, gtnx_batch_t b, gtnx_batch_t* out) {
  return guard([&] { *out = HB(batch_scalar(SK_SUBTRACT, BH(a), BH(b))); });
}
GTNX_API gtnx_status_t gtnx_batch_subtract_into(gtnx_batch_t a, gtnx_batch_t b, void* items_device, gtnx_batch_t* out) {
  return guard([&] { *out = HB(batch_scalar(SK_SUBTRACT, BH(a), BH(b), items_device)); });
}
GTNX_API gtnx_status_t gtnx_batch_compose(gtnx_batch_t a, gtnx_batch_t b, gtnx_batch_t* out) {
  return guard([&] { *out = HB(batch_compose(BH(a), BH(b), false)); });
}
GTNX_API gtnx_status_t gtnx_batch_intersect(gtnx_batch_t a, gtnx_batch_t b, gtnx_batch_t* out) {
  return guard([&] { *out = HB(batch_compose(BH(a), BH(b), true)); });
}
GTNX_API gtnx_status_t gtnx_batch_forward_score(gtnx_batch_t a, gtnx_batch_t* out) {
  return guard([&] { *out = HB(batch_shortest_distance(BH(a), false)); });
}
GTNX_API gtnx_status_t gtnx_batch_viterbi_score(gtnx_batch_t a, gtnx_batch_t* out) {
  return guard([&] { *out = HB(batch_shortest_distance(BH(a), true)); });
}
GTNX_API gtnx_status_t gtnx_batch_viterbi_path(gtnx_batch_t a, gtnx_batch_t* out) {
  return guard([&] { *out = HB(batch_viterbi_path(BH(a))); });
}
GTNX_API gtnx_status_t gtnx_batch_viterbi_align(gtnx_batch_t a, const int* frames, void* labels_device, int64_t row_stride,
                                                void* tokens_device, void* scores_device) {
// ... 109 lines not shown
```

### gtn_amd/csrc/kernels.h

```cpp
#pragma once

#include <hip/hip_runtime.h>

#include <cstdint>

#include <atomic>
#include <cstdint>
struct gtnx_first_on_device {
  std::atomic<uint64_t>& done;
  uint64_t bit;
  bool first;
  explicit gtnx_first_on_device(std::atomic<uint64_t>& d) : done(d) {
    int dev = 0;
    (void)hipGetDevice(&dev);
    bit = uint64_t(1) << (dev & 63);
    first = !(done.load(std::memory_order_acquire) & bit);
  }
  gtnx_first_on_device(const gtnx_first_on_device&) = delete;
  ~gtnx_first_on_device() {
    if (first) done.fetch_or(bit, std::memory_order_acq_rel);
  }
  explicit operator bool() const { return first; }
};

// ... 312 lines not shown
struct LazyPair {
  DGraph g;
  const GTNX_G float* em;
  GTNX_G float* alpha;
  GTNX_G float* score;
  const GTNX_G float* delta;
  GTNX_G float* grad_em;
  GTNX_G float* grad_fixed;
  int T, C, chain_first, pad;
};
int lazy_pair_max_nodes();
int lazy_pair_max_degree();
int lazy_pair_block(int max_nodes);
int lazy_pair_max_labels(int block);
void launch_lazy_pair_forward(const LazyPair* d_pairs, int n, int block, int C, int cus, hipStream_t st);
void launch_lazy_pair_backward(const LazyPair* d_pairs, int n, int block, int C, int cus, hipStream_t st);
struct BandNode {
  int lab;
  int aid[3];
};
struct BandPair {
  const GTNX_G BandNode* nodes;
  const GTNX_G uint8_t* nflags;
  const GTNX_G int* snode;
  const GTNX_G int* slab;
  const GTNX_G float* w;
  const GTNX_G float* em;
  GTNX_G float* em_copy;
  GTNX_G float* alpha;
  GTNX_G double* aoff;
  GTNX_G float* score;
  GTNX_G float* norm;
  GTNX_G float* rowlse;
  const GTNX_G float* delta;
  const GTNX_G float* delta_norm;
  GTNX_G float* grad_em;
  GTNX_G float* grad_fixed;
  int N, T, C, NS;
  int hot;
  int lgrn;
  int n_lab;
  int bidx;
  int64_t goff;
};
struct BandPatch {
  int on;
  int M;
  const GTNX_G float* delta;
  const GTNX_G float* delta_norm;
  GTNX_G float* rowlse;
  GTNX_G float* grad_em;
  GTNX_G float* grad_fixed;
  int64_t A;
};
struct BandDecode {
  const GTNX_G BandNode* nodes;
  const GTNX_G uint8_t* nflags;
  const GTNX_G float* w;
  const GTNX_G float* em;
  GTNX_G uint8_t* bp;
  GTNX_G int* pnode;
  GTNX_G int* path_arc;
  GTNX_G int* path_lab;
  GTNX_G float* path_w;
  GTNX_G int* path_len;
  GTNX_G float* score;
  GTNX_G int* tie;
  const GTNX_G int* rank_in;
  const GTNX_G int* rank_acc;
  int N, T, C, NS;
  int stage_floats, pad;
};
void launch_band_viterbi(const BandDecode* d_pairs, int n, int stage_floats, int max_nodes, int max_labels, int vec,
                         hipStream_t st, int ranked = 0);
bool band_viterbi_wave_ok(int max_nodes, int max_labels, int vec);
struct AlignArgs {
  const GTNX_G BandNode* nodes;
  const GTNX_G uint8_t* nflags;
  const GTNX_G float* em;
  GTNX_G unsigned* bp;
  GTNX_G int* labels;
  GTNX_G int* tokens;
  GTNX_G float* score;
  int N, T, T_full, C;
  int p, pad;
};
int align_npl(int max_nodes);
bool band_align_ok(int max_nodes, int max_labels, int vec);
void launch_band_align(const AlignArgs* d_args, int n, int max_nodes, hipStream_t st);
struct RationalSeg {
  DGraph g;
  int node_off, arc_off;
  int conn_off;
  int keep_start, keep_accept;
  int pad;
};
struct RationalOut {
  int N, A;
  GTNX_G int* src;
  GTNX_G int* dst;
  GTNX_G int* il;
  GTNX_G int* ol;
  GTNX_G float* w;
  GTNX_G uint8_t* nflags;
  GTNX_G int* start_list;
  GTNX_G int* accept_list;
// ... 7 lines not shown
                           int projection, int closure, void* temp, hipStream_t st);
void launch_rational_adjacency(const RationalOut& out, void* temp, hipStream_t st);
struct RemoveArgs {
  DGraph g;
  int ilabel, olabel;
  const GTNX_G int* new_id;
  const GTNX_G int* roots;
  int K, root0, rows;
  GTNX_G int* stamp;
  GTNX_G int* queue;
  GTNX_G int* arc_cnt;
  const GTNX_G int* arc_off;
  RationalOut out;
};
void launch_remove_keep(const DGraph& g, int ilabel, int olabel, int* keep, hipStream_t st);
void launch_remove_roots(const int* keep, const int* new_id, int N, int* roots, hipStream_t st);
void launch_remove_walk(const RemoveArgs& a, bool emit, hipStream_t st);
size_t scan_temp_bytes(int n);
void launch_exclusive_scan(const int* in, int* out, int n, void* temp, size_t temp_bytes, hipStream_t st);
void launch_rational_load(const void* rows, const float* w, const uint8_t* flags, const RationalOut& out, void* temp,
                          hipStream_t st);
struct CtcTargetArgs {
  const GTNX_G int* labels;
  GTNX_G BandNode* nodes;
  GTNX_G uint8_t* nflags;
  GTNX_G int* snode;
  GTNX_G int* slab;
  GTNX_G int* n_arcs;
  int N, pad;
};
void launch_ctc_targets(const CtcTargetArgs* d_args, int n, int blank, hipStream_t st);
struct AsgFalArgs {
  const GTNX_G int* labels;
  const GTNX_G float* trans_w;
  GTNX_G BandNode* nodes;
  GTNX_G uint8_t* nflags;
  GTNX_G int* snode;
  GTNX_G int* slab;
  GTNX_G float* w;
  GTNX_G int* arc_map;
  int U, pad;
};
void launch_asg_fal_targets(const AsgFalArgs* d_args, int n, int n_labels, hipStream_t st);
void launch_asg_fal_scatter(const float* g, const int* maps, const int64_t* tab , int n_seq, int64_t longest,
                            float* trans_grad, hipStream_t st);
int band_max_nodes();
int band_max_labels();
int band_min_labels();
int band_npl(int max_nodes);
int band_row_stride(int N, int npl);
int band_forward_lgrn(int C);
bool band_one_ok(int npl, int C, int max_NS, bool vec, bool backward);
void launch_band_forward(const BandPair* d_pairs, int n, int npl, int C, int max_NS, bool unit, bool vec, hipStream_t st,
                         const BandPair* one = nullptr);
void launch_band_backward(const BandPair* d_pairs, int n, int npl, int C, int max_NS, bool unit, bool gradg, bool vec,
                          hipStream_t st, const BandPair* one = nullptr, const BandPatch* patch = nullptr);
void launch_lazy_dense_prep(const LazyGroup& g, float* E, float* cmax, hipStream_t st);
void launch_lazy_dense_step(const LazyGroup& g, int t, int backward, hipStream_t st, const float* vin = nullptr,
                            float* vout = nullptr);
void launch_lazy_dense_fixed_grad(const LazyGroup& g, hipStream_t st);
size_t maxplus_w_floats(const LazyGroup& g);
void launch_maxplus_prep(const LazyGroup& g, hipStream_t st);
void launch_maxplus_step(const LazyGroup& g, int t, hipStream_t st);
void launch_maxplus_path(const LazyGroup& g, int* path_arc, int* path_il, int* path_ol, float* path_w, int* path_len,
                         hipStream_t st);
void launch_lazy_mfma_prep(const LazyGroup& g, hipStream_t st);
void launch_lazy_mfma_init(const LazyGroup& g, int which, hipStream_t st);
void launch_lazy_mfma_step(const LazyGroup& g, int t, int backward, hipStream_t st);
size_t lazy_mfma_chain_sync_ints(const LazyGroup& g);
bool launch_lazy_mfma_chain(const LazyGroup& g, int backward, int* zeroed_sync, int cus, hipStream_t st);
void launch_lazy_mfma_keys(float* keys, int64_t n, hipStream_t st);
void launch_lazy_mfma_rowmax(const LazyGroup& g, int which, hipStream_t st);
void launch_lazy_mfma_score(const LazyGroup& g, hipStream_t st);
size_t lazy_mfma_fixed_grad_scratch_bytes(const LazyGroup& g);
void launch_lazy_mfma_fixed_grad(const LazyGroup& g, void* pair_consts , hipStream_t st, void* partials = nullptr,
                                 size_t partials_bytes = 0);

void launch_fill_i32(int* p, int v, size_t n, hipStream_t st);
void launch_fill_f32(float* p, float v, size_t n, hipStream_t st);
void launch_scalar_seed(float* root, float* g0, float s0, int acc0, float* g1, float s1, int acc1, size_t n, hipStream_t st);
struct ScalarArgs {
  const GTNX_G float* a;
  const GTNX_G float* b;
  GTNX_G float* out;
  GTNX_G float* mirror;
};
void launch_scalar_combine(const ScalarArgs* d_args, int n, float sa, float sb, hipStream_t st);
void launch_copy_small(void* dst, const void* src, size_t bytes, hipStream_t st);
void launch_scalar_combine_one(const ScalarArgs& a, float sa, float sb, hipStream_t st);
struct ScalarFanArgs {
  const GTNX_G float* d;
  GTNX_G float* seed;
  GTNX_G float* o0;
  GTNX_G float* o1;
};
void launch_scalar_fan(const ScalarFanArgs* d_args, int n, float s0, float s1, hipStream_t st);
void launch_scalar_fan_one(const ScalarFanArgs& a, float s0, float s1, hipStream_t st);
struct AxpyArgs {
  GTNX_G float* dst;
  const GTNX_G float* src;
  int64_t n;
  float scale;
};
void launch_axpy_batch(const AxpyArgs* d_args, int n, int64_t maxn, int atomic, hipStream_t st);
struct CopySeg {
  void* dst;
  const void* src;
// ... 16 lines not shown
```

### gtn_amd/csrc/ops.h

```cpp
#pragma once

#include <cstring>
#include <tuple>
#include <vector>

#include "graph.h"

namespace gtnx {

struct Member {
  int idx;
  Graph out;
};

struct OpRecord {
  uint64_t seq = 0;
  virtual void backward(std::vector<Member>& members) = 0;
  virtual bool joins_chain_plan() const { return false; }
  virtual ~OpRecord() {}
};

struct GradSink {
  struct Item {
    Graph g;
    DevMemP owner;
    float* ptr;
  };
  std::vector<Item> items;
  void add(const Graph& g, const DevMemP& owner, float* ptr) {
    if (g.calc_grad()) items.push_back({g, owner, ptr});
  }
  void flush();
};

struct BandLaunchKey {
  int C, npl, unit, gradg, vec;
  bool operator<(const BandLaunchKey& o) const {
    return std::tie(C, npl, unit, gradg, vec) < std::tie(o.C, o.npl, o.unit, o.gradg, o.vec);
  }
  bool operator==(const BandLaunchKey& o) const { return !(*this < o) && !(o < *this); }
};
int band_vec_ok(const BandPair& p);
void band_launch(std::vector<std::pair<BandLaunchKey, BandPair>>& tab, bool backward, const char* prof_name = nullptr,
                 double prof_bytes = 0.0, DevMemP* table_out = nullptr);
void band_launch_patched(const DevMemP& table, int n, const BandLaunchKey& key, int max_ns, const BandPatch& patch,
                         const char* prof_name, double prof_bytes);

enum ScalarKind { SK_NEGATE = 0, SK_ADD = 1, SK_SUBTRACT = 2 };

std::vector<Graph> op_scalar(ScalarKind k, std::vector<Graph>& a, std::vector<Graph>& b);
std::vector<Graph> op_shortest_distance(std::vector<Graph>& gs, bool tropical);
std::vector<Graph> op_viterbi_path(std::vector<Graph>& gs);
std::vector<Graph> op_compose(std::vector<Graph>& a, std::vector<Graph>& b, bool intersect);
enum RationalKind { RAT_CLONE = 0, RAT_CONCAT = 1, RAT_CLOSURE = 2, RAT_UNION = 3 };
Graph op_rational(int kind, std::vector<Graph>& inputs, int projection);
Graph op_remove(Graph& g, int ilabel, int olabel);
Graph op_load_buffer(const void* data, size_t bytes);
void op_backward(std::vector<Graph>& roots, Graph* grad, bool retain, bool seed = true);
void backward_validate(Graph& root);
int compose_mode_hint(int mode);
void realize(Graph& g);

Graph make_scalar_graph(float v, bool calc_grad);
Graph make_linear_graph(int M, int N, bool calc_grad);
std::vector<Graph> make_linear_graphs_device(int B, int M, int N, bool calc_grad, const void* dev, bool borrow = false);
Graph make_user_op(std::vector<Graph>& inputs, gtnx_grad_fn fn, void* ctx, void (*ctx_free)(void*));
void set_user_grad_fn(Graph& g, gtnx_grad_fn fn, void* ctx, void (*ctx_free)(void*));

void items_host(std::vector<Graph>& gs, float* out);
void items_device(std::vector<Graph>& gs, void* dev_out);
void grads_device(std::vector<Graph>& gs, void* dev_out, const int64_t* offsets);
void grads_bind_device(std::vector<Graph>& gs, void* dev_out, const int64_t* offsets);

inline bool upload_in_place(size_t bytes) {
  static const size_t lim = [] {
    const char* e = std::getenv("GTNX_ARGS_IN_PLACE");
    return e ? size_t(std::atol(e)) : size_t(0);
  }();
  return bytes <= lim;
}
template <class T>
DevMemP upload_vec(const std::vector<T>& v) {
  Runtime& rt = Runtime::get();
  size_t bytes = sizeof(T) * v.size();
  if (bytes && upload_in_place(bytes)) {
    PinnedMemP p = rt.alloc_pinned(bytes);
    std::memcpy(p->ptr, v.data(), bytes);
    DevMemP d = std::make_shared<DevMem>();
    d->ptr = p->ptr;
    d->bytes = bytes;
    d->borrowed = true;
    d->keep = p;
    return d;
  }
  DevMemP d = rt.alloc(bytes ? bytes : 1);
  if (bytes) {
    PinnedMemP p = rt.alloc_pinned(bytes);
    std::memcpy(p->ptr, v.data(), bytes);
    rt.h2d_pinned(d->ptr, p->ptr, bytes);
// ... 6 lines not shown
```

### gtn_amd/csrc/ops_band.cpp

```cpp
#include "ops_internal.h"

#include <memory>

namespace gtnx {

int band_vec_ok(const BandPair& p) { return p.C % 4 == 0 && (reinterpret_cast<uintptr_t>(p.em) & 15) == 0; }
void band_launch_patched(const DevMemP& table, int n, const BandLaunchKey& k, int max_ns, const BandPatch& patch,
                         const char* prof_name, double prof_bytes) {
  Runtime& rt = Runtime::get();
  std::unique_ptr<Runtime::Scope> prof(prof_name ? new Runtime::Scope(&rt, prof_name, prof_bytes) : nullptr);
  launch_band_backward(table->as<BandPair>(), n, k.npl, k.C, max_ns, k.unit != 0, k.gradg != 0, k.vec != 0, rt.stream(), nullptr,
                       &patch);
}
void band_launch(std::vector<std::pair<BandLaunchKey, BandPair>>& tab, bool backward, const char* prof_name, double prof_bytes,
                 DevMemP* table_out) {
  Runtime& rt = Runtime::get();
  if (table_out) table_out->reset();
  if (tab.empty()) return;
  bool one_key = true;
  for (size_t i = 1; i < tab.size() && one_key; ++i) one_key = tab[i].first == tab[0].first;
  if (!one_key) std::stable_sort(tab.begin(), tab.end(), [](const auto& x, const auto& y) { return x.first < y.first; });
  if (tab.size() == 1) {
    const BandLaunchKey& k = tab[0].first;
    const BandPair& p = tab[0].second;
    if (band_one_ok(k.npl, k.C, p.NS, k.vec != 0, backward)) {
      std::unique_ptr<Runtime::Scope> prof(prof_name ? new Runtime::Scope(&rt, prof_name, prof_bytes) : nullptr);
      if (backward) launch_band_backward(nullptr, 1, k.npl, k.C, p.NS, k.unit != 0, k.gradg != 0, true, rt.stream(), &p);
      else launch_band_forward(nullptr, 1, k.npl, k.C, p.NS, k.unit != 0, true, rt.stream(), &p);
      return;
    }
  }
  std::vector<BandPair> flat;
  flat.reserve(tab.size());
  for (auto& e : tab) flat.push_back(e.second);
  DevMemP d = upload_vec(flat);
  const BandPair* dp = d->as<BandPair>();
  if (table_out && one_key) *table_out = d;
  std::unique_ptr<Runtime::Scope> prof(prof_name ? new Runtime::Scope(&rt, prof_name, prof_bytes) : nullptr);
  for (size_t i0 = 0; i0 < tab.size();) {
    size_t i1 = i0;
    int max_ns = 0;
    while (i1 < tab.size() && tab[i1].first == tab[i0].first) max_ns = std::max(max_ns, tab[i1++].second.NS);
    const BandLaunchKey& k = tab[i0].first;
    if (backward)
      launch_band_backward(dp + i0, int(i1 - i0), k.npl, k.C, max_ns, k.unit != 0, k.gradg != 0, k.vec != 0, rt.stream());
    else
      launch_band_forward(dp + i0, int(i1 - i0), k.npl, k.C, max_ns, k.unit != 0, k.vec != 0, rt.stream());
    i0 = i1;
  }
}
bool band_shape_ok(const Structure& cs, Structure& fs, bool chain_first) {
  if (cs.kind != KIND_LINEAR || cs.C < band_min_labels() || cs.C > band_max_labels() || cs.M < 0 || cs.M > (1 << 20)) return false;
  std::shared_ptr<BandInfo> b = band_info(fs, chain_first);
  return b->ok && b->max_label < cs.C;
}
bool band_ok(const LazyProduct& lp, std::shared_ptr<BandInfo>* out) {
  if (!band_shape_ok(*lp.chain.s, *lp.fixed.s, lp.chain_side == 1)) return false;
  if (out) *out = band_info(*lp.fixed.s, lp.chain_side == 1);
  return true;
}
static bool tie_ranks(Structure& fs, BandInfo& bi, bool use_ilabel);
void band_prepare(const std::vector<Graph*>& fixed, const std::vector<uint8_t>& chain_first, bool want_ranks) {
  std::vector<size_t> todo;
  std::unordered_set<Structure*> seen;
  for (size_t i = 0; i < fixed.size(); ++i) {
// ... 662 lines not shown
```

### gtn_amd/csrc/runtime.cpp

```cpp
#include "runtime.h"

#include "kernels.h"

#include <malloc.h>

#include <atomic>
#include <condition_variable>
#include <cstring>
#include <deque>
#include <thread>

namespace gtnx {

namespace {
constexpr int kMaxDevices = 64;
std::atomic<Runtime*> g_rts[kMaxDevices];
std::atomic<bool> g_any_rt{false};
std::mutex g_rt_mu;
std::atomic<int> g_default_device{-1};
thread_local int t_device = -1;

int hip_device_now() {
  int d = -1;
  if (hipGetDevice(&d) != hipSuccess) {
// ... 532 lines not shown
  if (reserved) *reserved = reserved_;
  if (in_use) *in_use = in_use_;
}

void Runtime::h2d(void* dst, const void* src, size_t bytes) {
  if (bytes) HIP_CHECK(hipMemcpyAsync(dst, src, bytes, hipMemcpyHostToDevice, stream_));
}
void Runtime::d2h_sync(void* dst, const void* src, size_t bytes) {
  if (bytes && bytes <= 4096) {
    PinnedMemP p = alloc_pinned(bytes);
    d2h_pinned_async(p->ptr, src, bytes);
    drain_while_busy();
    HIP_CHECK(hipStreamSynchronize(stream_));
    std::memcpy(dst, p->ptr, bytes);
    return;
  }
  if (bytes) HIP_CHECK(hipMemcpyAsync(dst, src, bytes, hipMemcpyDeviceToHost, stream_));
  drain_while_busy();
  HIP_CHECK(hipStreamSynchronize(stream_));
}
void Runtime::sync_while_draining() {
  drain_while_busy();
  HIP_CHECK(hipStreamSynchronize(stream_));
}
namespace {
bool local_to(const void* p, int dev) {
  static const int ndev = Runtime::device_count();
  if (ndev <= 1) return true;
  hipPointerAttribute_t a;
  if (hipPointerGetAttributes(&a, p) != hipSuccess) {
    (void)hipGetLastError();
    return false;
  }
  return a.type == hipMemoryTypeHost || (a.type == hipMemoryTypeDevice && a.device == dev);
}
}
bool ptr_local_to(const void* p, int dev) { return local_to(p, dev); }
void Runtime::d2d(void* dst, const void* src, size_t bytes) {
  if (!bytes) return;
  if (bytes <= (size_t(1) << 20) && local_to(src, device_) && local_to(dst, device_)) {
    launch_copy_small(dst, src, bytes, stream_);
    return;
  }
  HIP_CHECK(hipMemcpyAsync(dst, src, bytes, hipMemcpyDeviceToDevice, stream_));
}
void Runtime::d2h_pinned_async(void* pinned_dst, const void* src, size_t bytes) {
  if (!bytes) return;
  if (bytes <= (size_t(1) << 20) && local_to(src, device_)) {
    launch_copy_small(pinned_dst, src, bytes, stream_);
    return;
  }
  HIP_CHECK(hipMemcpyAsync(pinned_dst, src, bytes, hipMemcpyDeviceToHost, stream_));
}
void Runtime::h2d_pinned(void* dst, const void* pinned_src, size_t bytes) {
  if (!bytes) return;
  static const size_t lim = [] {
    const char* e = std::getenv("GTNX_H2D_KERNEL_BYTES");
    return e ? size_t(std::atol(e)) : size_t(1) << 20;
  }();
  if (bytes <= lim && local_to(dst, device_)) {
    launch_copy_small(dst, pinned_src, bytes, stream_);
    return;
  }
  HIP_CHECK(hipMemcpyAsync(dst, pinned_src, bytes, hipMemcpyHostToDevice, stream_));
}

Runtime::MirrorSlot Runtime::mirror_slot() {
  {
    std::lock_guard<std::mutex> lk(mu_);
    if (!mirror_ring_) {
      OnDevice here(device_);
      void* p = nullptr;
      HIP_CHECK(hipHostMalloc(&p, sizeof(float) * kMirrorSlots, hipHostMallocDefault));
      mirror_gen_ = new std::atomic<uint64_t>[kMirrorSlots];
      for (size_t i = 0; i < kMirrorSlots; ++i) mirror_gen_[i].store(0);
      mirror_ring_ = static_cast<float*>(p);
    }
  }
  const uint64_t g = mirror_next_.fetch_add(1) + 1;
  const size_t i = size_t(g % kMirrorSlots);
  mirror_gen_[i].store(g);
  return {mirror_ring_ + i, g};
}
bool Runtime::mirror_read(const MirrorSlot& m, float* out) {
  if (!m.ptr || !mirror_ring_) return false;
  const size_t i = size_t(m.ptr - mirror_ring_);
  if (i >= kMirrorSlots || mirror_gen_[i].load() != m.gen) return false;
  sync();
  const float v = *static_cast<volatile float*>(m.ptr);
  if (mirror_gen_[i].load() != m.gen) return false;
  *out = v;
  return true;
}

void Runtime::prof_enable(bool on) {
  if (!on) collect_prof();
  prof_on_ = on;
}
void Runtime::prof_reset() {
  collect_prof();
  prof_.clear();
}

Runtime::Scope::Scope(Runtime* r, const char* name, double bytes) : rt(r), idx(-1) {
  if (!rt->prof_on_) return;
  ProfRec rec;
  rec.name = name;
  rec.bytes = bytes;
  auto get_ev = [&]() {
    hipEvent_t e;
    HIP_CHECK(hipEventCreate(&e));
    return e;
// ... 96 lines not shown
```

### gtn_amd/csrc/runtime.h

```cpp
#pragma once

#include <atomic>
#include <functional>
#include <map>
#include <memory>
#include <mutex>
#include <string>
#include <vector>

#include "common.h"

namespace gtnx {

class Runtime;

struct DevMem {
  void* ptr = nullptr;
  size_t bytes = 0;
  bool borrowed = false;
  Runtime* owner = nullptr;
  std::shared_ptr<void> keep;
  ~DevMem();
  template <class T>
  T* as(size_t byte_off = 0) const { return reinterpret_cast<T*>(static_cast<char*>(ptr) + byte_off); }
// ... 16 lines not shown
  double bytes = 0;
};

class Runtime {
 public:
  static Runtime& get();
  static Runtime& of(int device);
  static int device_count();
  static bool initialized();
  static void set_current_device(int d);
  static int current_device();
  int device() const { return device_; }
  void activate();

  hipStream_t stream() const { return stream_; }
  void set_stream(hipStream_t s);
  void sync();

  DevMemP alloc(size_t bytes);
  DevMemP alloc_zero(size_t bytes);
  PinnedMemP alloc_pinned(size_t bytes);
  void release_dev(void* p, size_t bytes);
  void release_pinned(void* p, size_t bytes);
  void empty_cache();
  void stats(uint64_t* reserved, uint64_t* in_use);

  struct Inbox {
    std::mutex mu;
    std::vector<std::pair<void*, void (*)(void*)>> items;
    size_t load = 0;
    bool dead = false;
  };
  using InboxP = std::shared_ptr<Inbox>;
  static InboxP home();
  static void send(const InboxP& to, void* p, void (*del)(void*));
  static void drain_all_inboxes();
  static void defer_delete(void* p, void (*del)(void*), size_t weight = 1);
  static void drain_deferred();
  static bool drain_some(size_t max_items);
  static size_t deferred_count();
  void drain_until(void* hip_event);
  void drain_while_busy();
  void sync_while_draining();

  struct SideJob;
  using SideJobP = std::shared_ptr<SideJob>;
  SideJobP side_launch(std::function<void(hipStream_t)> fn);
  void side_join(const SideJobP& job);

  void h2d(void* dst, const void* src, size_t bytes);
  void d2h_sync(void* dst, const void* src, size_t bytes);
  void d2d(void* dst, const void* src, size_t bytes);
  void h2d_pinned(void* dst, const void* pinned_src, size_t bytes);
  void d2h_pinned_async(void* pinned_dst, const void* src, size_t bytes);

  struct MirrorSlot {
    float* ptr = nullptr;
    uint64_t gen = 0;
  };
  static constexpr size_t kMirrorSlots = 1024;
  MirrorSlot mirror_slot();
  bool mirror_read(const MirrorSlot& m, float* out);

  void prof_enable(bool on);
  void prof_add_bytes(const std::string& name, double bytes);
  void prof_reset();
  bool prof_on() const { return prof_on_; }
  struct Scope {
    Runtime* rt;
    int idx;
    Scope(Runtime* r, const char* name, double bytes);
    ~Scope();
  };
  ProfEntry prof_get(const std::string& name);
  std::string prof_names();
  int cu_count() const { return cu_count_; }

 private:
  explicit Runtime(int device);
  void collect_prof();
  float* mirror_ring_ = nullptr;
  std::atomic<uint64_t>* mirror_gen_ = nullptr;
  std::atomic<uint64_t> mirror_next_{0};
  hipStream_t own_stream_ = nullptr;
  hipStream_t stream_ = nullptr;
  int device_ = 0;
  int cu_count_ = 256;
  std::mutex mu_;
  std::multimap<size_t, void*> free_dev_;
  std::multimap<size_t, void*> free_pinned_;
  struct PinnedGroup {
    hipEvent_t ev;
    std::vector<std::pair<void*, size_t>> blocks;
  };
  static constexpr size_t kPinnedStampEvery = 8;
  std::vector<PinnedGroup> pending_pinned_;
  std::vector<std::pair<void*, size_t>> unstamped_pinned_;
  void stamp_pinned_locked();
  uint64_t reserved_ = 0, in_use_ = 0;
  bool prof_on_ = false;
  struct ProfRec {
    std::string name;
    double bytes;
    hipEvent_t a, b;
  };
  std::vector<ProfRec> prof_recs_;
// ... 26 lines not shown
```

### include/gtn/batch.h

```cpp
#pragma once
#include <cstdint>
#include <utility>
#include <vector>

#include "gtn/functions.h"

namespace gtn {

class Batch {
 public:
  Batch() = default;
  explicit Batch(const std::vector<Graph>& graphs) {
    auto h = detail::handles(graphs);
    detail::check(gtnx_batch_from_graphs(h.data(), static_cast<int>(h.size()), &h_));
  }
  Batch(const Batch&) = delete;
  Batch& operator=(const Batch&) = delete;
  Batch(Batch&& o) noexcept : h_(o.h_) { o.h_ = nullptr; }
  Batch& operator=(Batch&& o) noexcept {
    if (this != &o) {
      reset();
      h_ = o.h_;
      o.h_ = nullptr;
    }
// ... 47 lines not shown
  void itemsToDevice(void* deviceOut) const { detail::check(gtnx_batch_items_device(h_, deviceOut)); }
  void bindGrads(void* deviceOut, const int64_t* offsets) { detail::check(gtnx_batch_grads_bind_device(h_, deviceOut, offsets)); }
  void gradsToDevice(void* deviceOut, const int64_t* offsets) const {
    detail::check(gtnx_batch_grads_device(h_, deviceOut, offsets));
  }
  gtnx_batch_t handle() const { return h_; }
  static Batch fromHandle(gtnx_batch_t h) {
    Batch b;
    b.h_ = h;
    return b;
  }

 private:
  void reset() {
    if (h_) gtnx_batch_destroy(h_);
    h_ = nullptr;
  }
  gtnx_batch_t h_ = nullptr;
};

namespace detail {
template <class F>
Batch batchUnary(F f, const Batch& a) {
  gtnx_batch_t out;
  check(f(a.handle(), &out));
  return Batch::fromHandle(out);
}
template <class F>
Batch batchBinary(F f, const Batch& a, const Batch& b) {
  gtnx_batch_t out;
  check(f(a.handle(), b.handle(), &out));
  return Batch::fromHandle(out);
}
}

namespace batched {
inline Batch negate(const Batch& a) { return detail::batchUnary(&gtnx_batch_negate, a); }
inline Batch add(const Batch& a, const Batch& b) { return detail::batchBinary(&gtnx_batch_add, a, b); }
inline Batch subtract(const Batch& a, const Batch& b) { return detail::batchBinary(&gtnx_batch_subtract, a, b); }
inline Batch subtract(const Batch& a, const Batch& b, void* itemsDevice) {
  gtnx_batch_t out;
  detail::check(gtnx_batch_subtract_into(a.handle(), b.handle(), itemsDevice, &out));
  return Batch::fromHandle(out);
}
inline Batch compose(const Batch& a, const Batch& b) { return detail::batchBinary(&gtnx_batch_compose, a, b); }
inline Batch intersect(const Batch& a, const Batch& b) { return detail::batchBinary(&gtnx_batch_intersect, a, b); }
inline Batch forwardScore(const Batch& a) { return detail::batchUnary(&gtnx_batch_forward_score, a); }
inline Batch viterbiScore(const Batch& a) { return detail::batchUnary(&gtnx_batch_viterbi_score, a); }
inline Batch viterbiPath(const Batch& a) { return detail::batchUnary(&gtnx_batch_viterbi_path, a); }
inline void viterbiAlign(const Batch& product, int* labelsDevice, int64_t rowStride, int* tokensDevice = nullptr,
                         float* scoresDevice = nullptr, const int* frames = nullptr) {
  detail::check(gtnx_batch_viterbi_align(product.handle(), frames, labelsDevice, rowStride, tokensDevice, scoresDevice));
}
inline void backward(const Batch& a, bool retainGraph = false) { detail::check(gtnx_batch_backward(a.handle(), retainGraph)); }
}

}
```

### include/gtn_amd.h

```cpp
#ifndef GTN_AMD_H
#define GTN_AMD_H

#include <stddef.h>
#include <stdint.h>

#ifdef __cplusplus
extern "C" {
#endif

typedef int gtnx_status_t;
#define GTNX_OK 0
#define GTNX_INVALID_ARGUMENT 1
#define GTNX_LOGIC_ERROR 2
#define GTNX_RUNTIME_ERROR 3
#define GTNX_OUT_OF_RANGE 4
#define GTNX_DEVICE_ERROR 5

typedef struct gtnx_graph_s* gtnx_graph_t;

#define GTNX_EPSILON (-1)

const char* gtnx_last_error(void);
const char* gtnx_version(void);
const char* gtnx_backend(void);
// ... 57 lines not shown
gtnx_status_t gtnx_graph_zero_grad(gtnx_graph_t g);
gtnx_status_t gtnx_graph_add_grad(gtnx_graph_t g, const float* host_grad, int64_t n);
gtnx_status_t gtnx_graph_add_grad_graph(gtnx_graph_t g, gtnx_graph_t other);
gtnx_status_t gtnx_graph_id(gtnx_graph_t g, uintptr_t* out);
typedef gtnx_status_t (*gtnx_grad_fn)(void* ctx, gtnx_graph_t* inputs, int n_inputs, gtnx_graph_t deltas);
gtnx_status_t gtnx_graph_create_op(gtnx_graph_t* inputs, int n_inputs, gtnx_grad_fn grad_fn,
                                   void* ctx, void (*ctx_free)(void*), gtnx_graph_t* out);
gtnx_status_t gtnx_graph_num_inputs(gtnx_graph_t g, int64_t* out);
gtnx_status_t gtnx_graph_get_input(gtnx_graph_t g, int i, gtnx_graph_t* out);
gtnx_status_t gtnx_graph_set_inputs(gtnx_graph_t g, const gtnx_graph_t* inputs, int n);
gtnx_status_t gtnx_graph_set_grad_fn(gtnx_graph_t g, gtnx_grad_fn grad_fn, void* ctx,
                                     void (*ctx_free)(void*));
gtnx_status_t gtnx_graph_has_grad_fn(gtnx_graph_t g, int* out);

gtnx_status_t gtnx_scalar_graph(float value, int calc_grad, gtnx_graph_t* out);
gtnx_status_t gtnx_linear_graph(int M, int N, int calc_grad, gtnx_graph_t* out);
gtnx_status_t gtnx_linear_graph_n(int B, int M, int N, int calc_grad,
                                  const void* device_weights, gtnx_graph_t* out );
gtnx_status_t gtnx_linear_graph_borrow_n(int B, int M, int N, int calc_grad,
                                         const void* device_weights, gtnx_graph_t* out );

gtnx_status_t gtnx_negate(gtnx_graph_t g, gtnx_graph_t* out);
gtnx_status_t gtnx_add(gtnx_graph_t a, gtnx_graph_t b, gtnx_graph_t* out);
gtnx_status_t gtnx_subtract(gtnx_graph_t a, gtnx_graph_t b, gtnx_graph_t* out);
gtnx_status_t gtnx_compose(gtnx_graph_t a, gtnx_graph_t b, gtnx_graph_t* out);
gtnx_status_t gtnx_intersect(gtnx_graph_t a, gtnx_graph_t b, gtnx_graph_t* out);
gtnx_status_t gtnx_forward_score(gtnx_graph_t g, gtnx_graph_t* out);
gtnx_status_t gtnx_viterbi_score(gtnx_graph_t g, gtnx_graph_t* out);
gtnx_status_t gtnx_viterbi_path(gtnx_graph_t g, gtnx_graph_t* out);

gtnx_status_t gtnx_negate_n(const gtnx_graph_t* g, int n, gtnx_graph_t* out);
gtnx_status_t gtnx_add_n(const gtnx_graph_t* a, int na, const gtnx_graph_t* b, int nb, gtnx_graph_t* out);
gtnx_status_t gtnx_subtract_n(const gtnx_graph_t* a, int na, const gtnx_graph_t* b, int nb, gtnx_graph_t* out);
gtnx_status_t gtnx_compose_n(const gtnx_graph_t* a, int na, const gtnx_graph_t* b, int nb, gtnx_graph_t* out);
gtnx_status_t gtnx_intersect_n(const gtnx_graph_t* a, int na, const gtnx_graph_t* b, int nb, gtnx_graph_t* out);
gtnx_status_t gtnx_forward_score_n(const gtnx_graph_t* g, int n, gtnx_graph_t* out);
gtnx_status_t gtnx_viterbi_score_n(const gtnx_graph_t* g, int n, gtnx_graph_t* out);
gtnx_status_t gtnx_viterbi_path_n(const gtnx_graph_t* g, int n, gtnx_graph_t* out);
gtnx_status_t gtnx_items_n(const gtnx_graph_t* g, int n, float* out);
gtnx_status_t gtnx_items_device_n(const gtnx_graph_t* g, int n, void* device_out);
gtnx_status_t gtnx_grads_device_n(const gtnx_graph_t* g, int n, void* device_out, const int64_t* offsets);
gtnx_status_t gtnx_grads_bind_device_n(const gtnx_graph_t* g, int n, void* device_out, const int64_t* offsets);

gtnx_status_t gtnx_clone(gtnx_graph_t g, int projection , gtnx_graph_t* out);
gtnx_status_t gtnx_concat(const gtnx_graph_t* g, int n, gtnx_graph_t* out);
gtnx_status_t gtnx_closure(gtnx_graph_t g, gtnx_graph_t* out);
gtnx_status_t gtnx_union(const gtnx_graph_t* g, int n, gtnx_graph_t* out);
gtnx_status_t gtnx_remove(gtnx_graph_t g, int ilabel, int olabel, gtnx_graph_t* out);

typedef struct gtnx_batch_s* gtnx_batch_t;
gtnx_status_t gtnx_batch_from_graphs(const gtnx_graph_t* g, int n, gtnx_batch_t* out);
gtnx_status_t gtnx_batch_ctc_targets(const int* labels, const int* lengths, int n, int blank, int calc_grad,
                                     gtnx_batch_t* out);
gtnx_status_t gtnx_batch_asg_force_align(const int* labels, const int* lengths, int n, gtnx_graph_t transitions,
                                         int n_labels, gtnx_batch_t* out);
gtnx_status_t gtnx_batch_linear(int n, int M, int N, int calc_grad, const void* device_weights, int borrow,
                                gtnx_batch_t* out);
gtnx_status_t gtnx_batch_destroy(gtnx_batch_t b);
gtnx_status_t gtnx_batch_size(gtnx_batch_t b, int* out);
gtnx_status_t gtnx_batch_get(gtnx_batch_t b, int i, gtnx_graph_t* out);
gtnx_status_t gtnx_batch_negate(gtnx_batch_t a, gtnx_batch_t* out);
gtnx_status_t gtnx_batch_add(gtnx_batch_t a, gtnx_batch_t b, gtnx_batch_t* out);
gtnx_status_t gtnx_batch_subtract(gtnx_batch_t a, gtnx_batch_t b, gtnx_batch_t* out);
gtnx_status_t gtnx_batch_subtract_into(gtnx_batch_t a, gtnx_batch_t b, void* items_device, gtnx_batch_t* out);
gtnx_status_t gtnx_batch_compose(gtnx_batch_t a, gtnx_batch_t b, gtnx_batch_t* out);
gtnx_status_t gtnx_batch_intersect(gtnx_batch_t a, gtnx_batch_t b, gtnx_batch_t* out);
gtnx_status_t gtnx_batch_forward_score(gtnx_batch_t a, gtnx_batch_t* out);
gtnx_status_t gtnx_batch_viterbi_score(gtnx_batch_t a, gtnx_batch_t* out);
gtnx_status_t gtnx_batch_viterbi_path(gtnx_batch_t a, gtnx_batch_t* out);
gtnx_status_t gtnx_batch_viterbi_align(gtnx_batch_t a, const int* frames, void* labels_device, int64_t row_stride,
                                       void* tokens_device, void* scores_device);
gtnx_status_t gtnx_batch_align_stats(int64_t* fast, int64_t* fallback);
gtnx_status_t gtnx_batch_backward(gtnx_batch_t a, int retain_graph);
gtnx_status_t gtnx_batch_items(gtnx_batch_t a, float* out);
gtnx_status_t gtnx_batch_items_device(gtnx_batch_t a, void* device_out);
gtnx_status_t gtnx_batch_grads_bind_device(gtnx_batch_t a, void* device_out, const int64_t* offsets);
gtnx_status_t gtnx_batch_grads_device(gtnx_batch_t a, void* device_out, const int64_t* offsets);

gtnx_status_t gtnx_backward(gtnx_graph_t g, int retain_graph);
gtnx_status_t gtnx_backward_with_grad(gtnx_graph_t g, gtnx_graph_t grad, int retain_graph);
gtnx_status_t gtnx_backward_n(const gtnx_graph_t* g, int n, int retain_graph);

gtnx_status_t gtnx_equal(gtnx_graph_t a, gtnx_graph_t b, int* out);
gtnx_status_t gtnx_isomorphic(gtnx_graph_t a, gtnx_graph_t b, int* out);

gtnx_status_t gtnx_graph_load_buffer(const void* data, size_t bytes, gtnx_graph_t* out);

typedef struct gtnx_comm_s* gtnx_comm_t;
gtnx_status_t gtnx_comm_create(const int* devices, int n, gtnx_comm_t* out);
gtnx_status_t gtnx_comm_destroy(gtnx_comm_t c);
gtnx_status_t gtnx_comm_size(gtnx_comm_t c, int* n);
gtnx_status_t gtnx_comm_all_gather_f32(gtnx_comm_t c, const void* const* send, void* const* recv, int64_t count);
gtnx_status_t gtnx_comm_all_reduce_sum_f32(gtnx_comm_t c, void* const* bufs, int64_t count);

gtnx_status_t gtnx_prof_enable(int on);
gtnx_status_t gtnx_prof_reset(void);
gtnx_status_t gtnx_prof_get(const char* name, double* total_ms, int64_t* launches,
                            double* algorithmic_bytes);
gtnx_status_t gtnx_debug_viterbi_ties(int64_t* seen, int64_t* unresolved);
gtnx_status_t gtnx_debug_tie_ranks(gtnx_graph_t g, int* queue_rank, int* creation_rank, int* applies);
gtnx_status_t gtnx_prof_names(char* buf, size_t cap);
gtnx_status_t gtnx_debug_symbolic_route(gtnx_graph_t g, int tropical, int* route);
gtnx_status_t gtnx_debug_route_name(int route, char* buf, size_t cap);

#ifdef __cplusplus
}
// ... 3 lines not shown
```

Baseline: 936,300 losses/s.

## Fuse CTC target build, loss subtraction and backward seeding into band kernels

Adds a fused CTC loss-forward entry point. The CTC target graph construction runs at the head of the band forward kernel, the loss (norm minus score) is written directly by the forward kernel, and the backward seed values are written by the band backward kernel instead of separate launches. The aim is to remove several small kernel launches and host round trips per step (ctc_targets, subtract, seeding). In exchange the kernels become more complex, the forward kernel uses extra LDS for the head, and a runtime toggle and counters are added.

```diff
diff --git a/gtn_amd/__init__.py b/gtn_amd/__init__.py
--- a/gtn_amd/__init__.py
+++ b/gtn_amd/__init__.py
@@ -57,6 +57,9 @@
 debug_viterbi_ties = _api.debug_viterbi_ties
 debug_tie_ranks = _api.debug_tie_ranks
 debug_align_stats = getattr(_api, "debug_align_stats", None)
+ctc_loss_forward = getattr(_api, "ctc_loss_forward", None)
+debug_ctc_step_fusion = getattr(_api, "debug_ctc_step_fusion", None)
+debug_ctc_step_stats = getattr(_api, "debug_ctc_step_stats", None)
 
 
 def load_txt(text):
diff --git a/gtn_amd/_capi.py b/gtn_amd/_capi.py
--- a/gtn_amd/_capi.py
+++ b/gtn_amd/_capi.py
@@ -117,6 +117,10 @@
     "gtnx_batch_viterbi_path": [c_graph, c_graph_p],
     "gtnx_batch_viterbi_align": [c_graph, C.c_void_p, C.c_void_p, C.c_int64, C.c_void_p, C.c_void_p],
     "gtnx_batch_align_stats": [c_i64_p, c_i64_p],
+    "gtnx_batch_ctc_loss_forward": [C.c_void_p, C.c_void_p, C.c_int, C.c_int, C.c_int, c_graph, C.c_void_p, c_graph_p,
+                                    c_graph_p, C.c_void_p],
+    "gtnx_batch_ctc_step_fusion": [C.c_int],
+    "gtnx_batch_ctc_step_stats": [C.c_void_p],
     "gtnx_batch_backward": [c_graph, C.c_int],
     "gtnx_batch_items": [c_graph, C.c_void_p],
     "gtnx_batch_items_device": [c_graph, C.c_void_p],
diff --git a/gtn_amd/api.py b/gtn_amd/api.py
--- a/gtn_amd/api.py
+++ b/gtn_amd/api.py
@@ -711,6 +711,31 @@
     if hasattr(lib, "gtnx_batch_subtract_into"):
         ns.subtract_into = subtract_into
 
+    def ctc_loss_forward(targets, emissions, blank=0, target_grad=True, loss_out=None):
+        lens = np.asarray([len(t) for t in targets], dtype=np.int32)
+        flat = np.ascontiguousarray(np.concatenate([np.asarray(t, dtype=np.int32).reshape(-1) for t in targets])
+                                    if len(targets) else np.zeros(0, np.int32), dtype=np.int32)
+        ht, hl = C.c_void_p(), C.c_void_p()
+        check(lib.gtnx_batch_ctc_loss_forward(flat.ctypes.data, lens.ctypes.data, len(lens), int(blank), int(bool(target_grad)),
+                                              emissions._h, _as_dev_ptr(loss_out) if loss_out is not None else None,
+                                              C.byref(ht), C.byref(hl), None))
+        losses = Batch._from_handle(hl.value)
+        losses._keep = loss_out
+        return losses, Batch._from_handle(ht.value)
+
+    def debug_ctc_step_fusion(on):
+        check(lib.gtnx_batch_ctc_step_fusion(int(bool(on))))
+
+    def debug_ctc_step_stats():
+        v = (C.c_int64 * 4)()
+        check(lib.gtnx_batch_ctc_step_stats(C.addressof(v)))
+        return tuple(int(x) for x in v)
+
+    if hasattr(lib, "gtnx_batch_ctc_loss_forward"):
+        ns.ctc_loss_forward = ctc_loss_forward
+        ns.debug_ctc_step_fusion = debug_ctc_step_fusion
+        ns.debug_ctc_step_stats = debug_ctc_step_stats
+
     _plain_backward = ns.backward
 
     def backward(g, grad_or_retain=None, retain_graph=False):
diff --git a/gtn_amd/criteria/ctc_criterion.h b/gtn_amd/criteria/ctc_criterion.h
--- a/gtn_amd/criteria/ctc_criterion.h
+++ b/gtn_amd/criteria/ctc_criterion.h
@@ -51,23 +51,19 @@
     Batch* targetsOut = nullptr) {
   auto now = [] { return std::chrono::steady_clock::now(); };
   auto ms = [](auto a, auto b) { return std::chrono::duration<double, std::milli>(b - a).count(); };
-  auto t0 = now();
-  Batch ctcs = Batch::ctcTargets(labels, lengths, B, blank, targetGrad);
   auto t1 = now();
   Batch ems = Batch::linear(B, T, C, emissions, gradDev != nullptr, true);
   std::vector<int64_t> off(B);
   for (int b = 0; b < B; ++b) off[b] = (int64_t)b * T * C;
   if (gradDev) ems.bindGrads(gradDev, off.data());
   auto t2 = now();
-  Batch comp = batched::intersect(ctcs, ems);
-  auto t3 = now();
-  Batch score = batched::forwardScore(comp);
-  Batch norm = batched::forwardScore(ems);
-  Batch losses = batched::subtract(norm, score, lossDev);
+  Batch ctcs;
+  double hm[3] = {0, 0, 0};
+  Batch losses = batched::ctcLossForward(labels, lengths, B, blank, targetGrad, ems, lossDev, &ctcs, times ? hm : nullptr);
   auto t4 = now();
   if (gradDev) batched::backward(losses);
   auto t5 = now();
-  if (times) *times = {ms(t0, t1), ms(t1, t2), ms(t2, t3), ms(t3, t4), ms(t4, t5)};
+  if (times) *times = {hm[0], ms(t1, t2), hm[1], hm[2], ms(t4, t5)};
   losses.itemsToDevice(lossDev);
   if (gradDev) ems.gradsToDevice(gradDev, off.data());
   if (targetsOut) *targetsOut = std::move(ctcs);
diff --git a/gtn_amd/csrc/band.hip b/gtn_amd/csrc/band.hip
--- a/gtn_amd/csrc/band.hip
+++ b/gtn_amd/csrc/band.hip
@@ -332,55 +332,13 @@
   return wave_max(mx);
 }
 
-template <int NPL, bool UNIT, int K, bool VEC>
-__global__ __launch_bounds__(WG) void band_forward_kernel(const BandPair* __restrict__ pairs, int NSmax) {
-#define GTNX_BAND_PAIR pairs[blockIdx.x]
-#include "band_forward_body.inc"
-#undef GTNX_BAND_PAIR
-}
-template <int NPL, bool UNIT, int K, bool VEC>
-__global__ __launch_bounds__(WG) void band_forward_one_kernel(BandPair one, int NSmax) {
-#define GTNX_BAND_PAIR one
-#include "band_forward_body.inc"
-#undef GTNX_BAND_PAIR
-}
-
-__device__ __forceinline__ BandPair band_patched(BandPair P, const BandPatch& pt) {
-  if (pt.on) {
-    const int b = P.bidx;
-    P.delta = pt.delta + b;
-    P.delta_norm = pt.delta_norm ? pt.delta_norm + b : nullptr;
-    P.rowlse = pt.rowlse ? pt.rowlse + int64_t(b) * pt.M : nullptr;
-    P.norm = nullptr;
-    P.em_copy = nullptr;
-    P.grad_em = pt.grad_em ? pt.grad_em + int64_t(b) * pt.A : nullptr;
-    P.grad_fixed = pt.grad_fixed ? pt.grad_fixed + P.goff : nullptr;
-  }
-  return P;
-}
-template <int NPL, bool UNIT, bool GRADG, int K, bool VEC, bool BIG>
-__global__ __launch_bounds__(WGB, BIG ? 3 : 6) void band_backward_kernel(const BandPair* __restrict__ pairs, int NSmax, BandPatch patch) {
-#define GTNX_BAND_PAIR band_patched(pairs[blockIdx.x], patch)
-#include "band_backward_body.inc"
-#undef GTNX_BAND_PAIR
-}
-template <int NPL, bool UNIT, bool GRADG, int K, bool VEC, bool BIG>
-__global__ __launch_bounds__(WGB, BIG ? 3 : 6) void band_backward_one_kernel(BandPair one, int NSmax) {
-#define GTNX_BAND_PAIR one
-#include "band_backward_body.inc"
-#undef GTNX_BAND_PAIR
-}
-
-
-__global__ __launch_bounds__(512) void ctc_targets_kernel(const CtcTargetArgs* __restrict__ args, int blank) {
-  const CtcTargetArgs a = args[blockIdx.x];
-  __shared__ __attribute__((aligned(16))) int tl[256 + 4];
-  __shared__ __attribute__((aligned(16))) int tk[256 + 4];
+__device__ __forceinline__ void ctc_target_build(const CtcTargetArgs& a, const GTNX_G int* lab, int blank, int* tl, int* tk) {
   const int N = a.N, U = (N - 1) >> 1, m = threadIdx.x;
   if (m < 260) {
-    const int v = m < U ? a.labels[m] : 0x7fffffff;
+    const int v = m < U ? lab[m] : 0x7fffffff;
     tl[m] = v;
-    tk[m] = (m > 0 && m < U && v != a.labels[m - 1]) ? 1 : 0;
+    tk[m] = (m > 0 && m < U && v != lab[m - 1]) ? 1 : 0;
+    if (lab != a.labels && m < U) const_cast<GTNX_G int*>(a.labels)[m] = v;
   }
   __syncthreads();
   if (m >= N) return;
@@ -412,6 +370,85 @@
   a.slab[rank] = my;
   if (m == N - 1 && a.n_arcs) a.n_arcs[0] = base + 1 + (m > 0 ? 1 : 0) + skip;
 }
+__global__ __launch_bounds__(512) void ctc_targets_kernel(const CtcTargetArgs* __restrict__ args, int blank) {
+  __shared__ __attribute__((aligned(16))) int tl[256 + 4];
+  __shared__ __attribute__((aligned(16))) int tk[256 + 4];
+  const CtcTargetArgs a = args[blockIdx.x];
+  ctc_target_build(a, a.labels, blank, tl, tk);
+}
+
+template <int NPL, bool UNIT, int K, bool VEC>
+__global__ __launch_bounds__(WG) void band_forward_kernel(const BandPair* __restrict__ pairs, int NSmax, BandHead head) {
+  static_assert(WG == 512, "the target build is written for 512 lanes");
+  if (head.on && head.args) {
+    extern __shared__ __attribute__((aligned(16))) float lds_head[];
+    int* tl = reinterpret_cast<int*>(lds_head);
+    const CtcTargetArgs a = head.args[blockIdx.x];
+    ctc_target_build(a, reinterpret_cast<const GTNX_G int*>(reinterpret_cast<const GTNX_G char*>(a.labels) + head.lab_shift),
+                     head.blank, tl, tl + 264);
+    if (head.table) {
+      static_assert(sizeof(BandPair) % 4 == 0 && sizeof(BandPair) / 4 <= WG, "one dword per lane");
+      const int* src = reinterpret_cast<const int*>(pairs + blockIdx.x);
+      GTNX_G int* dst = reinterpret_cast<GTNX_G int*>(head.table + blockIdx.x);
+      if (threadIdx.x < sizeof(BandPair) / 4) dst[threadIdx.x] = src[threadIdx.x];
+    }
+    __syncthreads();
+  }
+#define GTNX_BAND_PAIR pairs[blockIdx.x]
+#define GTNX_BAND_LOSS (head.on ? head.loss : nullptr)
+#include "band_forward_body.inc"
+#undef GTNX_BAND_LOSS
+#undef GTNX_BAND_PAIR
+}
+template <int NPL, bool UNIT, int K, bool VEC>
+__global__ __launch_bounds__(WG) void band_forward_one_kernel(BandPair one, int NSmax) {
+#define GTNX_BAND_PAIR one
+#define GTNX_BAND_LOSS static_cast<GTNX_G float*>(nullptr)
+#include "band_forward_body.inc"
+#undef GTNX_BAND_LOSS
+#undef GTNX_BAND_PAIR
+}
+
+__device__ __forceinline__ BandPair band_patched(BandPair P, const BandPatch& pt) {
+  if (pt.on) {
+    const int b = P.bidx;
+    P.delta = pt.delta ? pt.delta + b : nullptr;
+    P.delta_norm = pt.delta_norm ? pt.delta_norm + b : nullptr;
+    P.rowlse = pt.rowlse ? pt.rowlse + int64_t(b) * pt.M : nullptr;
+    P.norm = nullptr;
+    P.em_copy = nullptr;
+    P.grad_em = pt.grad_em ? pt.grad_em + int64_t(b) * pt.A : nullptr;
+    P.grad_fixed = pt.grad_fixed ? pt.grad_fixed + P.goff : nullptr;
+  }
+  return P;
+}
+template <int NPL, bool UNIT, bool GRADG, int K, bool VEC, bool BIG>
+__global__ __launch_bounds__(WGB, BIG ? 3 : 6) void band_backward_kernel(const BandPair* __restrict__ pairs, int NSmax, BandPatch patch) {
+#define GTNX_BAND_PAIR band_patched(pairs[blockIdx.x], patch)
+#define GTNX_BAND_SEED_DS patch.cs
+#define GTNX_BAND_SEED_DN patch.cn
+#include "band_backward_body.inc"
+#undef GTNX_BAND_SEED_DN
+#undef GTNX_BAND_SEED_DS
+#undef GTNX_BAND_PAIR
+  if (patch.on && patch.seed_root && threadIdx.x == 0) {
+    const int b = pairs[blockIdx.x].bidx;
+    patch.seed_root[b] = 1.0f;
+    patch.seed_score[b] = patch.cs;
+    if (patch.seed_norm) patch.seed_norm[b] = patch.seed_cn;
+  }
+}
+template <int NPL, bool UNIT, bool GRADG, int K, bool VEC, bool BIG>
+__global__ __launch_bounds__(WGB, BIG ? 3 : 6) void band_backward_one_kernel(BandPair one, int NSmax) {
+#define GTNX_BAND_PAIR one
+#define GTNX_BAND_SEED_DS 0.0f
+#define GTNX_BAND_SEED_DN 0.0f
+#include "band_backward_body.inc"
+#undef GTNX_BAND_SEED_DN
+#undef GTNX_BAND_SEED_DS
+#undef GTNX_BAND_PAIR
+}
+
 
 __global__ __launch_bounds__(512) void band_viterbi_kernel(const BandDecode* __restrict__ pairs) {
   const BandDecode P = pairs[blockIdx.x];
@@ -810,7 +847,7 @@
 }
 
 template <int NPL, int K, bool VEC>
-void launch_fwd2(const BandPair* d, const BandPair* one, int n, int ns, size_t lds, bool unit, hipStream_t st) {
+void launch_fwd2(const BandPair* d, const BandPair* one, int n, int ns, size_t lds, bool unit, hipStream_t st, const BandHead& hd) {
   static std::atomic<uint64_t> done{0};
   if (gtnx_first_on_device first{done}) {
     big_lds(band_forward_kernel<NPL, true, K, VEC>);
@@ -827,13 +864,14 @@
       return;
     }
   }
-  if (unit) hipLaunchKernelGGL((band_forward_kernel<NPL, true, K, VEC>), dim3(n), dim3(WG), lds, st, d, ns);
-  else hipLaunchKernelGGL((band_forward_kernel<NPL, false, K, VEC>), dim3(n), dim3(WG), lds, st, d, ns);
+  if (unit) hipLaunchKernelGGL((band_forward_kernel<NPL, true, K, VEC>), dim3(n), dim3(WG), lds, st, d, ns, hd);
+  else hipLaunchKernelGGL((band_forward_kernel<NPL, false, K, VEC>), dim3(n), dim3(WG), lds, st, d, ns, hd);
 }
 template <int NPL, int K>
-void launch_fwd(const BandPair* d, const BandPair* one, int n, int ns, size_t lds, bool unit, bool vec, hipStream_t st) {
-  if (vec) launch_fwd2<NPL, K, true>(d, one, n, ns, lds, unit, st);
-  else launch_fwd2<NPL, K, false>(d, one, n, ns, lds, unit, st);
+void launch_fwd(const BandPair* d, const BandPair* one, int n, int ns, size_t lds, bool unit, bool vec, hipStream_t st,
+                const BandHead& hd) {
+  if (vec) launch_fwd2<NPL, K, true>(d, one, n, ns, lds, unit, st, hd);
+  else launch_fwd2<NPL, K, false>(d, one, n, ns, lds, unit, st, hd);
 }
 template <int NPL, int K, bool VEC, bool BIG>
 void launch_bwd3(const BandPair* d, const BandPair* one, int n, int ns, size_t lds, bool unit, bool gradg, hipStream_t st,
@@ -923,19 +961,22 @@
   return !(K * C > 1024 || K * max_NS > 1024);
 }
 void launch_band_forward(const BandPair* d_pairs, int n, int npl, int C, int max_NS, bool unit, bool vec, hipStream_t st,
-                         const BandPair* one) {
+                         const BandPair* one, const BandHead* head) {
   if (n <= 0) return;
+  if (one && head) throw std::logic_error("band.hip: a launch with a head reads a device table");
+  BandHead hd{};
+  if (head) hd = *head;
   if (one && (n != 1 || !band_one_ok(npl, C, max_NS, vec, false))) throw std::logic_error("band.hip: not a single-pair launch");
   const int K = band_block_rows(C, 0, false);
   const size_t lds = 4 * size_t(band_lds(C, K, max_NS, false).total) + 64;
   if (npl == 1) {
-    if (K == 8) launch_fwd<1, 8>(d_pairs, one, n, max_NS, lds, unit, vec, st);
-    else if (K == 4) launch_fwd<1, 4>(d_pairs, one, n, max_NS, lds, unit, vec, st);
-    else launch_fwd<1, 2>(d_pairs, one, n, max_NS, lds, unit, vec, st);
+    if (K == 8) launch_fwd<1, 8>(d_pairs, one, n, max_NS, lds, unit, vec, st, hd);
+    else if (K == 4) launch_fwd<1, 4>(d_pairs, one, n, max_NS, lds, unit, vec, st, hd);
+    else launch_fwd<1, 2>(d_pairs, one, n, max_NS, lds, unit, vec, st, hd);
   } else {
-    if (K == 8) launch_fwd<2, 8>(d_pairs, one, n, max_NS, lds, unit, vec, st);
-    else if (K == 4) launch_fwd<2, 4>(d_pairs, one, n, max_NS, lds, unit, vec, st);
-    else launch_fwd<2, 2>(d_pairs, one, n, max_NS, lds, unit, vec, st);
+    if (K == 8) launch_fwd<2, 8>(d_pairs, one, n, max_NS, lds, unit, vec, st, hd);
+    else if (K == 4) launch_fwd<2, 4>(d_pairs, one, n, max_NS, lds, unit, vec, st, hd);
+    else launch_fwd<2, 2>(d_pairs, one, n, max_NS, lds, unit, vec, st, hd);
   }
 }
 
diff --git a/gtn_amd/csrc/band_backward_body.inc b/gtn_amd/csrc/band_backward_body.inc
--- a/gtn_amd/csrc/band_backward_body.inc
+++ b/gtn_amd/csrc/band_backward_body.inc
@@ -19,11 +19,12 @@
   const GTNX_G double* ao = P.aoff;
   const double z2 = uniform(ao[0]);
   const bool dead = !(z2 > double(DEADF));
-  const float ds = uniform(P.delta[0]);
+  const float ds = P.delta ? uniform(P.delta[0]) : GTNX_BAND_SEED_DS;
   const bool want_em = P.grad_em != nullptr;
   GTNX_TM_INIT(128);
   constexpr bool SPLIT = !BIG && K >= 2 && GTNX_BWD_SPLIT;
-  const float dn_k = P.delta_norm ? uniform(P.delta_norm[0]) : 0.0f;
+  const float dn_k = P.delta_norm ? uniform(P.delta_norm[0]) : GTNX_BAND_SEED_DN;
+  const bool has_dn = P.delta_norm != nullptr || GTNX_BAND_SEED_DN != 0.0f;
   float* const rnorm_k = lser + NBG * K;
   auto rows_of_k = [&](int c) { return c < nblocks ? min(K, T - c * K) : 0; };
   auto ring_start = [](int c, int M) { return ((c % M) + M) % M; };
@@ -479,7 +480,7 @@
           if (g.ao[k][j] >= 0) P.grad_fixed[g.ao[k][j]] = dead ? 0.0f : acc[k][j];
     }
   } else if (wv < 8) {
-    const bool soft = P.delta_norm != nullptr && P.rowlse != nullptr;
+    const bool soft = has_dn && P.rowlse != nullptr;
     lds_barrier();
     if constexpr (!BIG) {
       const int h = wv - 4, q = h & 1;
@@ -693,7 +694,7 @@
     }
   } else {
     const int hid = threadIdx.x - 2 * BW;
-    const bool soft = P.delta_norm != nullptr && P.rowlse != nullptr;
+    const bool soft = has_dn && P.rowlse != nullptr;
     int* cls = reinterpret_cast<int*>(oring);
     for (int c = hid; c < 2 * C; c += BW) cls[c] = 0;
     lds_barrier();
diff --git a/gtn_amd/csrc/band_forward_body.inc b/gtn_amd/csrc/band_forward_body.inc
--- a/gtn_amd/csrc/band_forward_body.inc
+++ b/gtn_amd/csrc/band_forward_body.inc
@@ -355,10 +355,14 @@
       if (M.fin[2 * k] > DEADF) S += M.fin[2 * k + 1] * ex2(float(M.find[k] + double(M.fin[2 * k]) - Mx));
     const double z2 = dead ? double(NEGF) : Mx + double(lg2(S));
     P.aoff[0] = z2;
-    P.score[0] = dead ? -__builtin_inff() : float(z2 * LN2);
+    const float sv = dead ? -__builtin_inff() : float(z2 * LN2);
+    P.score[0] = sv;
     if (P.norm) {
       double n2 = 0.0;
       for (int k = 0; k < 16; ++k) n2 += M.red[k];
-      P.norm[0] = n2 < double(DEADF) ? -__builtin_inff() : float(n2 * LN2);
+      const float nv = n2 < double(DEADF) ? -__builtin_inff() : float(n2 * LN2);
+      P.norm[0] = nv;
+      GTNX_G float* const loss = GTNX_BAND_LOSS;
+      if (loss) loss[P.bidx] = nv - sv;
     }
   }
diff --git a/gtn_amd/csrc/batch.cpp b/gtn_amd/csrc/batch.cpp
--- a/gtn_amd/csrc/batch.cpp
+++ b/gtn_amd/csrc/batch.cpp
@@ -91,10 +91,32 @@
   }
 };
 
+std::atomic<int64_t> g_ctc_fwd_fused{0}, g_ctc_fwd_unfused{0}, g_seed_fused{0}, g_seed_launched{0};
 struct BackwardPlan {
   std::unordered_map<Batch*, Batch*> lin;
   std::unordered_set<Batch*> fused;
+  struct Seed {
+    bool pending = false;
+    Batch* root = nullptr;
+    Batch* score = nullptr;
+    Batch* norm = nullptr;
+    float* g[2] = {nullptr, nullptr};
+    float sc[2] = {0.0f, 0.0f};
+    int score_idx = 0;
+    void launch() {
+      if (!pending) return;
+      pending = false;
+      g_seed_launched.fetch_add(1);
+      launch_scalar_seed(root->g_dev, g[0], sc[0], 0, g[1], sc[1], 0, size_t(root->n), Runtime::get().stream());
+    }
+  } seed;
 };
+std::atomic<int> g_ctc_fusion_off{0};
+bool ctc_fusion_enabled() {
+  static const bool no_patch = std::getenv("GTNX_NO_BAND_PATCH") != nullptr;
+  if (no_patch || Runtime::h2d_kernel_limit() == 0) return false;
+  return !g_ctc_fusion_off.load(std::memory_order_relaxed) && std::getenv("GTNX_NO_FUSED_CTC_STEP") == nullptr;
+}
 thread_local BackwardPlan* t_plan = nullptr;
 thread_local bool t_batch_retain = false;
 
@@ -147,7 +169,9 @@
     Batch& ch = *prod.chain;
     Runtime& rt = Runtime::get();
     const float* delta = out.g_dev;
+    BackwardPlan::Seed* seed = (t_plan && t_plan->seed.pending && t_plan->seed.score == &out) ? &t_plan->seed : nullptr;
     if (through_acc || t_batch_retain) {
+      if (seed) seed->launch(), seed = nullptr;
       const size_t n = size_t(prod.n);
       if (!through_acc) through_acc = rt.alloc_zero(sizeof(float) * (n ? n : 1));
       launch_vec_axpby(through_acc->as<float>(), out.g_dev, nullptr, n, 1.0f, 0.0f, 1, rt.stream());
@@ -185,12 +209,27 @@
                (p.grad_fixed ? 4.0 * double(fx.elem_size(b)) : 0.0);
     }
     static const bool no_patch = std::getenv("GTNX_NO_BAND_PATCH") != nullptr;
+    if (seed && !(fwd_table && one_key && prod.n > 1 && !no_patch && seed->norm == lin_out))
+      seed->launch(), seed = nullptr;
     if (fwd_table && one_key && prod.n > 1 && !no_patch) {
       BandPatch pt{};
       pt.on = 1;
       pt.M = ch.M;
       pt.delta = delta;
       pt.delta_norm = lin_out ? lin_out->g_dev : nullptr;
+      if (seed) {
+        const int si = seed->score_idx, ni = 1 - si;
+        pt.delta = nullptr;
+        pt.delta_norm = nullptr;
+        pt.cs = seed->sc[si];
+        pt.cn = lin_out ? seed->sc[ni] : 0.0f;
+        pt.seed_root = seed->root->g_dev;
+        pt.seed_score = seed->g[si];
+        pt.seed_norm = seed->g[ni];
+        pt.seed_cn = seed->sc[ni];
+        seed->pending = false;
+        g_seed_fused.fetch_add(1);
+      }
       pt.rowlse = lin_out ? ch.nc_rowlse : nullptr;
       pt.grad_em = ge.ptr;
       pt.grad_fixed = gf.ptr;
@@ -326,8 +365,14 @@
 }
 }
 
-BatchP batch_ctc_targets(const int* labels, const int* lengths, int n, int blank, bool calc_grad) {
-  GTNX_HOST_T("batch.ctc_targets");
+namespace {
+struct CtcHostBlock {
+  PinnedMemP pin;
+  size_t lab_bytes = 0, arg_bytes = 0, extra_bytes = 0;
+  int blank = 0;
+};
+BatchP ctc_targets_host(const int* labels, const int* lengths, int n, int blank, bool calc_grad, size_t extra_bytes,
+                        CtcHostBlock& blk) {
   if (n < 0) throw_invalid("[gtnx_batch_ctc_targets] negative batch size");
   BatchP b = make_batch(Batch::CTC_TARGETS, n, calc_grad);
   b->blank = blank;
@@ -356,7 +401,8 @@
   Runtime& rt = Runtime::get();
   const size_t lab_bytes = align_up(sizeof(int) * (total ? total : 1), 256);
   const size_t arg_bytes = align_up(sizeof(CtcTargetArgs) * size_t(n), 256);
-  size_t bytes = lab_bytes + arg_bytes;
+  extra_bytes = align_up(extra_bytes, 256);
+  size_t bytes = lab_bytes + arg_bytes + extra_bytes;
   b->rec_off.resize(size_t(n));
   for (int i = 0; i < n; ++i) {
     const size_t N = size_t(2 * lengths[i] + 1);
@@ -364,7 +410,7 @@
     bytes += align_up(sizeof(BandNode) * N, 64) + align_up(N, 64) + 2 * align_up(4 * N, 64) + 64;
   }
   b->rec_mem = rt.alloc(bytes);
-  PinnedMemP pin = rt.alloc_pinned(lab_bytes + arg_bytes);
+  PinnedMemP pin = rt.alloc_pinned(lab_bytes + arg_bytes + extra_bytes);
   std::memcpy(pin->ptr, labels, sizeof(int) * total);
   CtcTargetArgs* args = reinterpret_cast<CtcTargetArgs*>(static_cast<char*>(pin->ptr) + lab_bytes);
   for (int i = 0; i < n; ++i) {
@@ -384,8 +430,25 @@
     a.N = int(N);
     a.pad = 0;
   }
-  rt.h2d_pinned(b->rec_mem->ptr, pin->ptr, lab_bytes + arg_bytes);
-  launch_ctc_targets(reinterpret_cast<const CtcTargetArgs*>(b->rec_mem->as<char>(lab_bytes)), n, blank, rt.stream());
+  blk.pin = pin;
+  blk.lab_bytes = lab_bytes;
+  blk.arg_bytes = arg_bytes;
+  blk.extra_bytes = extra_bytes;
+  blk.blank = blank;
+  return b;
+}
+void ctc_targets_upload(Batch& b, const CtcHostBlock& blk) {
+  Runtime& rt = Runtime::get();
+  rt.h2d_pinned(b.rec_mem->ptr, blk.pin->ptr, blk.lab_bytes + blk.arg_bytes);
+  launch_ctc_targets(reinterpret_cast<const CtcTargetArgs*>(b.rec_mem->as<char>(blk.lab_bytes)), b.n, blk.blank, rt.stream());
+}
+}
+
+BatchP batch_ctc_targets(const int* labels, const int* lengths, int n, int blank, bool calc_grad) {
+  GTNX_HOST_T("batch.ctc_targets");
+  CtcHostBlock blk;
+  BatchP b = ctc_targets_host(labels, lengths, n, blank, calc_grad, 0, blk);
+  if (blk.pin) ctc_targets_upload(*b, blk);
   return b;
 }
 
@@ -747,106 +810,157 @@
   return batch_from_graphs(op_compose(a->graphs, b->graphs, intersect));
 }
 
+namespace {
+struct FusedHead {
+  const CtcHostBlock* blk = nullptr;
+  float* loss = nullptr;
+  bool taken = false, loss_written = false;
+};
+BatchP band_forward_batch(const BatchP& x, FusedHead* head) {
+  Runtime& rt = Runtime::get();
+  Batch& fx = *x->fixed;
+  Batch& ch = *x->chain;
+  const int n = x->n, T = ch.M, C = ch.C;
+  auto op = std::make_shared<BFsBandOp>();
+  op->inputs = {x};
+  const bool want_norm = ch.nc_norm == nullptr;
+  size_t bytes = align_up(4 * size_t(n), 256);
+  const size_t o_norm = bytes;
+  bytes = align_up(bytes + 4 * size_t(n), 256);
+  const size_t o_lse = bytes;
+  bytes = align_up(bytes + 4 * size_t(n) * size_t(T > 0 ? T : 1), 256);
+  std::vector<size_t> oo, ao;
+  oo.resize(size_t(n));
+  ao.resize(size_t(n));
+  for (int b = 0; b < n; ++b) {
+    const int Ub = fx.lab_off[size_t(b) + 1] - fx.lab_off[size_t(b)];
+    const int N = fx.fal ? Ub + 1 : 2 * Ub + 1;
+    const int ns = band_row_stride(N, band_npl(N));
+    oo[size_t(b)] = bytes;
+    bytes = align_up(bytes + 8 * (4 * size_t(T) + 16), 256);
+    ao[size_t(b)] = bytes;
+    bytes = align_up(bytes + 4 * size_t(T + 1) * size_t(ns), 256);
+  }
+  op->arena = rt.alloc(bytes);
+  op->pairs.resize(size_t(n));
+  std::vector<std::pair<BandLaunchKey, BandPair>> tab;
+  tab.reserve(size_t(n));
+  double abytes = 0;
+  std::shared_ptr<PendingCopy> pend = ch.w_pend;
+  std::unique_lock<std::mutex> pend_lock;
+  bool fuse_copy = false;
+  if (pend && !pend->done.load(std::memory_order_acquire)) {
+    pend_lock = std::unique_lock<std::mutex>(pend->mu);
+    fuse_copy = !pend->done.load(std::memory_order_relaxed) && pend->device == rt.device();
+    const size_t A = size_t(T) * size_t(C);
+    for (int b = 0; b < n && fuse_copy; ++b) fuse_copy = pend->src_of(ch.w_dev + size_t(b) * A) != nullptr;
+    fuse_copy = fuse_copy && pend->segs.size() == size_t(n);
+    if (!fuse_copy) {
+      pend_lock.unlock();
+      pend->settle();
+    }
+  }
+  int64_t goff_run = 0;
+  for (int b = 0; b < n; ++b) {
+    BandPair& p = op->pairs[size_t(b)];
+    p = BandPair{};
+    const int U = fx.lab_off[size_t(b) + 1] - fx.lab_off[size_t(b)];
+    const size_t N = fx.fal ? size_t(U) + 1 : size_t(2 * U + 1);
+    char* base = fx.rec_mem->as<char>(fx.rec_off[size_t(b)]);
+    p.nodes = reinterpret_cast<BandNode*>(base);
+    base += align_up(sizeof(BandNode) * N, 64);
+    p.nflags = reinterpret_cast<uint8_t*>(base);
+    base += align_up(N, 64);
+    p.snode = reinterpret_cast<int*>(base);
+    base += align_up(4 * N, 64);
+    p.slab = reinterpret_cast<int*>(base);
+    p.n_lab = fx.fal ? U : int(N);
+    p.w = fx.fal ? fx.rec_mem->as<float>(fx.w_off[size_t(b)]) : nullptr;
+    p.em = ch.w_dev + size_t(b) * size_t(T) * size_t(C);
+    p.N = int(N);
+    p.T = T;
+    p.C = C;
+    p.NS = band_row_stride(p.N, band_npl(p.N));
+    p.alpha = op->arena->as<float>(ao[size_t(b)]);
+    p.aoff = op->arena->as<double>(oo[size_t(b)]);
+    p.score = op->arena->as<float>(4 * size_t(b));
+    if (want_norm) {
+      p.norm = op->arena->as<float>(o_norm + 4 * size_t(b));
+      p.rowlse = op->arena->as<float>(o_lse + 4 * size_t(b) * size_t(T));
+    }
+    p.hot = (!fx.fal && U + 1 >= 8) ? fx.blank : -1;
+    p.lgrn = band_forward_lgrn(C);
+    p.bidx = b;
+    p.goff = goff_run;
+    goff_run += int64_t(fx.elem_size(b));
+    BandPair q = p;
+    if (fuse_copy) {
+      q.em = static_cast<const float*>(pend->src_of(p.em));
+      q.em_copy = const_cast<float*>(p.em);
+    }
+    tab.push_back({BandLaunchKey{C, band_npl(q.N), fx.fal ? 0 : 1, 0, band_vec_ok(q)}, q});
+    abytes += 4.0 * T * C + 4.0 * double(T + 1) * p.NS + (fuse_copy ? 4.0 * T * C : 0.0);
+  }
+  bool one_key = true;
+  int max_ns = 0;
+  for (auto& e : tab) {
+    one_key = one_key && e.first == tab.front().first;
+    max_ns = std::max(max_ns, e.second.NS);
+  }
+  if (head && !fuse_copy && one_key && n > 1) {
+    const CtcHostBlock& blk = *head->blk;
+    const size_t tab_off = blk.lab_bytes + blk.arg_bytes;
+    BandPair* hp = blk.pin->as<BandPair>(tab_off);
+    for (int b = 0; b < n; ++b) hp[b] = tab[size_t(b)].second;
+    static const bool in_place = std::getenv("GTNX_CTC_HEAD_IN_PLACE") != nullptr;
+    if (!in_place) rt.h2d_pinned(fx.rec_mem->ptr, blk.pin->ptr, tab_off + sizeof(BandPair) * size_t(n));
+    DevMemP table = std::make_shared<DevMem>();
+    table->ptr = fx.rec_mem->as<char>(tab_off);
+    table->bytes = sizeof(BandPair) * size_t(n);
+    table->borrowed = true;
+    table->keep = fx.rec_mem;
+    BandHead hd{};
+    hd.on = 1;
+    hd.blank = blk.blank;
+    hd.args = reinterpret_cast<const CtcTargetArgs*>(fx.rec_mem->as<char>(blk.lab_bytes));
+    hd.loss = want_norm ? head->loss : nullptr;
+    DevMemP read = table;
+    if (in_place) {
+      hd.args = blk.pin->as<CtcTargetArgs>(blk.lab_bytes);
+      hd.table = table->as<BandPair>();
+      hd.lab_shift = static_cast<char*>(blk.pin->ptr) - fx.rec_mem->as<char>();
+      read = std::make_shared<DevMem>();
+      read->ptr = hp;
+      read->bytes = table->bytes;
+      read->borrowed = true;
+      read->keep = blk.pin;
+    }
+    band_launch_headed(read, n, tab.front().first, max_ns, hd, "band_forward_score", abytes);
+    op->fwd_table = table;
+    head->taken = true;
+    head->loss_written = hd.loss != nullptr;
+  } else {
+    if (head) ctc_targets_upload(fx, *head->blk);
+    band_launch(tab, false, "band_forward_score", abytes, fuse_copy ? nullptr : &op->fwd_table);
+  }
+  if (fuse_copy) pend->done.store(true, std::memory_order_release);
+  if (want_norm) {
+    ch.nc_mem = op->arena;
+    ch.nc_norm = op->arena->as<float>(o_norm);
+    ch.nc_rowlse = op->arena->as<float>(o_lse);
+  }
+  DevMemP arena = op->arena;
+  BatchP r = result(Batch::SCALAR, n, op);
+  r->v_mem = arena;
+  r->v_dev = arena->as<float>();
+  return r;
+}
+}
+
 BatchP batch_shortest_distance(const BatchP& x, bool tropical) {
   GTNX_HOST_T("batch.shortest_distance");
   Runtime& rt = Runtime::get();
-  if (!tropical && native(*x, Batch::PRODUCT) && !x->materialised) {
-    Batch& fx = *x->fixed;
-    Batch& ch = *x->chain;
-    const int n = x->n, T = ch.M, C = ch.C;
-    auto op = std::make_shared<BFsBandOp>();
-    op->inputs = {x};
-    const bool want_norm = ch.nc_norm == nullptr;
-    size_t bytes = align_up(4 * size_t(n), 256);
-    const size_t o_norm = bytes;
-    bytes = align_up(bytes + 4 * size_t(n), 256);
-    const size_t o_lse = bytes;
-    bytes = align_up(bytes + 4 * size_t(n) * size_t(T > 0 ? T : 1), 256);
-    std::vector<size_t> oo, ao;
-    oo.resize(size_t(n));
-    ao.resize(size_t(n));
-    for (int b = 0; b < n; ++b) {
-      const int Ub = fx.lab_off[size_t(b) + 1] - fx.lab_off[size_t(b)];
-      const int N = fx.fal ? Ub + 1 : 2 * Ub + 1;
-      const int ns = band_row_stride(N, band_npl(N));
-      oo[size_t(b)] = bytes;
-      bytes = align_up(bytes + 8 * (4 * size_t(T) + 16), 256);
-      ao[size_t(b)] = bytes;
-      bytes = align_up(bytes + 4 * size_t(T + 1) * size_t(ns), 256);
-    }
-    op->arena = rt.alloc(bytes);
-    op->pairs.resize(size_t(n));
-    std::vector<std::pair<BandLaunchKey, BandPair>> tab;
-    tab.reserve(size_t(n));
-    double abytes = 0;
-    std::shared_ptr<PendingCopy> pend = ch.w_pend;
-    std::unique_lock<std::mutex> pend_lock;
-    bool fuse_copy = false;
-    if (pend && !pend->done.load(std::memory_order_acquire)) {
-      pend_lock = std::unique_lock<std::mutex>(pend->mu);
-      fuse_copy = !pend->done.load(std::memory_order_relaxed) && pend->device == rt.device();
-      const size_t A = size_t(T) * size_t(C);
-      for (int b = 0; b < n && fuse_copy; ++b) fuse_copy = pend->src_of(ch.w_dev + size_t(b) * A) != nullptr;
-      fuse_copy = fuse_copy && pend->segs.size() == size_t(n);
-      if (!fuse_copy) {
-        pend_lock.unlock();
-        pend->settle();
-      }
-    }
-    int64_t goff_run = 0;
-    for (int b = 0; b < n; ++b) {
-      BandPair& p = op->pairs[size_t(b)];
-      p = BandPair{};
-      const int U = fx.lab_off[size_t(b) + 1] - fx.lab_off[size_t(b)];
-      const size_t N = fx.fal ? size_t(U) + 1 : size_t(2 * U + 1);
-      char* base = fx.rec_mem->as<char>(fx.rec_off[size_t(b)]);
-      p.nodes = reinterpret_cast<BandNode*>(base);
-      base += align_up(sizeof(BandNode) * N, 64);
-      p.nflags = reinterpret_cast<uint8_t*>(base);
-      base += align_up(N, 64);
-      p.snode = reinterpret_cast<int*>(base);
-      base += align_up(4 * N, 64);
-      p.slab = reinterpret_cast<int*>(base);
-      p.n_lab = fx.fal ? U : int(N);
-      p.w = fx.fal ? fx.rec_mem->as<float>(fx.w_off[size_t(b)]) : nullptr;
-      p.em = ch.w_dev + size_t(b) * size_t(T) * size_t(C);
-      p.N = int(N);
-      p.T = T;
-      p.C = C;
-      p.NS = band_row_stride(p.N, band_npl(p.N));
-      p.alpha = op->arena->as<float>(ao[size_t(b)]);
-      p.aoff = op->arena->as<double>(oo[size_t(b)]);
-      p.score = op->arena->as<float>(4 * size_t(b));
-      if (want_norm) {
-        p.norm = op->arena->as<float>(o_norm + 4 * size_t(b));
-        p.rowlse = op->arena->as<float>(o_lse + 4 * size_t(b) * size_t(T));
-      }
-      p.hot = (!fx.fal && U + 1 >= 8) ? fx.blank : -1;
-      p.lgrn = band_forward_lgrn(C);
-      p.bidx = b;
-      p.goff = goff_run;
-      goff_run += int64_t(fx.elem_size(b));
-      BandPair q = p;
-      if (fuse_copy) {
-        q.em = static_cast<const float*>(pend->src_of(p.em));
-        q.em_copy = const_cast<float*>(p.em);
-      }
-      tab.push_back({BandLaunchKey{C, band_npl(q.N), fx.fal ? 0 : 1, 0, band_vec_ok(q)}, q});
-      abytes += 4.0 * T * C + 4.0 * double(T + 1) * p.NS + (fuse_copy ? 4.0 * T * C : 0.0);
-    }
-    band_launch(tab, false, "band_forward_score", abytes, fuse_copy ? nullptr : &op->fwd_table);
-    if (fuse_copy) pend->done.store(true, std::memory_order_release);
-    if (want_norm) {
-      ch.nc_mem = op->arena;
-      ch.nc_norm = op->arena->as<float>(o_norm);
-      ch.nc_rowlse = op->arena->as<float>(o_lse);
-    }
-    DevMemP arena = op->arena;
-    BatchP r = result(Batch::SCALAR, n, op);
-    r->v_mem = arena;
-    r->v_dev = arena->as<float>();
-    return r;
-  }
+  if (!tropical && native(*x, Batch::PRODUCT) && !x->materialised) return band_forward_batch(x, nullptr);
   if (!tropical && native(*x, Batch::LINEAR) && !x->materialised && x->nc_norm) {
     auto op = std::make_shared<BFsLinearOp>();
     op->inputs = {x};
@@ -1025,6 +1139,10 @@
 }
 }
 
+namespace {
+thread_local bool t_scalar_values_written = false;
+}
+
 BatchP batch_scalar(ScalarKind k, const BatchP& a0, const BatchP& b0, void* items_dev) {
   BatchP a = a0, b = b0;
   const bool binary = k != SK_NEGATE;
@@ -1050,8 +1168,9 @@
       r->v_mem = rt.alloc(sizeof(float) * size_t(a->n ? a->n : 1));
       r->v_dev = r->v_mem->as<float>();
     }
-    launch_vec_axpby(r->v_dev, a->v_dev, binary ? b->v_dev : nullptr, size_t(a->n), k == SK_NEGATE ? -1.0f : 1.0f,
-                     k == SK_SUBTRACT ? -1.0f : 1.0f, 0, rt.stream());
+    if (!t_scalar_values_written)
+      launch_vec_axpby(r->v_dev, a->v_dev, binary ? b->v_dev : nullptr, size_t(a->n), k == SK_NEGATE ? -1.0f : 1.0f,
+                       k == SK_SUBTRACT ? -1.0f : 1.0f, 0, rt.stream());
     return r;
   }
   batch_materialise(*a);
@@ -1060,6 +1179,77 @@
   BatchP r = batch_from_graphs(op_scalar(k, a->graphs, binary ? b->graphs : none));
   if (items_dev) batch_items_device(r, items_dev);
   return r;
+}
+
+void batch_ctc_step_fusion(bool on) { g_ctc_fusion_off.store(on ? 0 : 1); }
+void batch_ctc_step_stats(int64_t* fwd_fused, int64_t* fwd_unfused, int64_t* seed_fused, int64_t* seed_launched) {
+  if (fwd_fused) *fwd_fused = g_ctc_fwd_fused.load();
+  if (fwd_unfused) *fwd_unfused = g_ctc_fwd_unfused.load();
+  if (seed_fused) *seed_fused = g_seed_fused.load();
+  if (seed_launched) *seed_launched = g_seed_launched.load();
+}
+
+BatchP batch_ctc_loss_forward(const int* labels, const int* lengths, int n, int blank, bool target_grad, const BatchP& ems,
+                              void* loss_dev, BatchP* targets_out, double* host_ms) {
+  GTNX_HOST_T("batch.ctc_loss_forward");
+  const double t0 = host_ms ? host_now_ms() : 0.0;
+  if (!ems) throw_invalid("[gtnx_batch_ctc_loss_forward] null emissions");
+  bool fuse = ctc_fusion_enabled() && n > 1 && ems->kind == Batch::LINEAR && !ems->materialised && ems->n == n &&
+              ems->nc_norm == nullptr && ems->C >= band_min_labels() && ems->C <= band_max_labels() && ems->M <= (1 << 20);
+  if (fuse && ems->w_pend && !ems->w_pend->done.load(std::memory_order_acquire)) fuse = false;
+  size_t total = 0;
+  if (fuse) {
+    const int npl0 = band_npl(2 * std::max(lengths[0], 0) + 1);
+    for (int i = 0; i < n && fuse; ++i) {
+      fuse = lengths[i] >= 0 && 2 * lengths[i] + 1 <= band_max_nodes() && band_npl(2 * lengths[i] + 1) == npl0;
+      total += size_t(std::max(lengths[i], 0));
+    }
+    fuse = fuse && blank >= 0 && blank < ems->C;
+    for (size_t i = 0; i < total && fuse; ++i) fuse = labels[i] >= 0 && labels[i] < ems->C;
+    fuse = fuse && align_up(sizeof(int) * (total ? total : 1), 256) + align_up(sizeof(CtcTargetArgs) * size_t(n), 256) +
+                           sizeof(BandPair) * size_t(n) <= Runtime::h2d_kernel_limit();
+  }
+  CtcHostBlock blk;
+  BatchP ctcs = ctc_targets_host(labels, lengths, n, blank, target_grad, fuse ? sizeof(BandPair) * size_t(n) : 0, blk);
+  if (!fuse && blk.pin) ctc_targets_upload(*ctcs, blk);
+  const double t1 = host_ms ? host_now_ms() : 0.0;
+  BatchP comp = batch_compose(ctcs, ems, true);
+  const double t2 = host_ms ? host_now_ms() : 0.0;
+  BatchP losses;
+  bool rode = false;
+  if (fuse && blk.pin && comp->kind == Batch::PRODUCT && !comp->materialised) {
+    Runtime& rt = Runtime::get();
+    DevMemP loss_mem;
+    if (!loss_dev) loss_mem = rt.alloc(sizeof(float) * size_t(n));
+    FusedHead head;
+    head.blk = &blk;
+    head.loss = loss_dev ? static_cast<float*>(loss_dev) : loss_mem->as<float>();
+    BatchP score = band_forward_batch(comp, &head);
+    BatchP norm = batch_shortest_distance(ems, false);
+    rode = head.taken;
+    t_scalar_values_written = head.loss_written;
+    try {
+      losses = batch_scalar(SK_SUBTRACT, norm, score, head.loss);
+    } catch (...) {
+      t_scalar_values_written = false;
+      throw;
+    }
+    t_scalar_values_written = false;
+    if (loss_mem) losses->v_mem = loss_mem;
+  } else {
+    if (fuse && blk.pin) ctc_targets_upload(*ctcs, blk);
+    BatchP score = batch_shortest_distance(comp, false);
+    BatchP norm = batch_shortest_distance(ems, false);
+    losses = batch_scalar(SK_SUBTRACT, norm, score, loss_dev);
+  }
+  (rode ? g_ctc_fwd_fused : g_ctc_fwd_unfused).fetch_add(1);
+  if (host_ms) {
+    host_ms[0] = t1 - t0;
+    host_ms[1] = t2 - t1;
+    host_ms[2] = host_now_ms() - t2;
+  }
+  if (targets_out) *targets_out = ctcs;
+  return losses;
 }
 
 void batch_backward(const BatchP& root, bool retain) {
@@ -1088,6 +1278,7 @@
   }
   std::sort(order.begin(), order.end(), [](Batch* a, Batch* b) { return a->op->seq > b->op->seq; });
   bool root_done = false;
+  BackwardPlan plan;
   if (!root->g_dev) {
     alloc_grad(*root, false);
     auto* sop = dynamic_cast<BScalarOp*>(root->op.get());
@@ -1107,7 +1298,30 @@
         if (!in.g_dev) alloc_grad(in, false);
         g[i] = in.g_dev;
       }
-      launch_scalar_seed(root->g_dev, g[0], sc[0], acc[0], g[1], sc[1], acc[1], size_t(root->n), rt.stream());
+      int si = -1;
+      BFsBandOp* bop = nullptr;
+      for (size_t i = 0; i < sop->inputs.size() && si < 0; ++i)
+        if (g[i] && (bop = dynamic_cast<BFsBandOp*>(sop->inputs[i]->op.get())) != nullptr) si = int(i);
+      bool ride = si >= 0 && !retain && root->n > 1 && !acc[0] && !acc[1] && ctc_fusion_enabled() && bop->fwd_table &&
+                  !bop->through_acc;
+      Batch* nb = nullptr;
+      if (ride && sop->inputs.size() == 2 && g[1 - si]) {
+        nb = sop->inputs[size_t(1 - si)].get();
+        Batch* chain = bop->inputs[0]->chain.get();
+        ride = dynamic_cast<BFsLinearOp*>(nb->op.get()) != nullptr && nb->op->inputs[0].get() == chain && chain->calc_grad &&
+               chain->nc_rowlse != nullptr;
+      }
+      if (ride) {
+        plan.seed.pending = true;
+        plan.seed.root = root.get();
+        plan.seed.score = sop->inputs[size_t(si)].get();
+        plan.seed.norm = nb;
+        plan.seed.score_idx = si;
+        for (int i = 0; i < 2; ++i) plan.seed.g[i] = g[i], plan.seed.sc[i] = sc[i];
+      } else {
+        launch_scalar_seed(root->g_dev, g[0], sc[0], acc[0], g[1], sc[1], acc[1], size_t(root->n), rt.stream());
+        g_seed_launched.fetch_add(1);
+      }
       root_done = true;
     } else {
       launch_fill_f32(root->g_dev, 1.0f, size_t(root->n), rt.stream());
@@ -1118,7 +1332,6 @@
     launch_vec_axpby(root->g_dev, ones->as<float>(), nullptr, size_t(root->n), 1.0f, 0.0f, 1, rt.stream());
   }
   std::vector<Batch*> from_graphs;
-  BackwardPlan plan;
   t_plan = &plan;
   struct RetainScope {
     bool prev;
@@ -1136,6 +1349,7 @@
       }
       b->op->backward(*b);
     }
+    plan.seed.launch();
     for (auto& kv : plan.lin)
       if (!plan.fused.count(kv.first)) static_cast<BFsLinearOp*>(kv.second->op.get())->run(*kv.second);
   } catch (...) {
diff --git a/gtn_amd/csrc/batch.h b/gtn_amd/csrc/batch.h
--- a/gtn_amd/csrc/batch.h
+++ b/gtn_amd/csrc/batch.h
@@ -81,6 +81,10 @@
                          float* scores_dev);
 void batch_align_stats(int64_t* fast, int64_t* fallback);
 BatchP batch_scalar(ScalarKind k, const BatchP& a, const BatchP& b, void* items_dev = nullptr);
+BatchP batch_ctc_loss_forward(const int* labels, const int* lengths, int n, int blank, bool target_grad, const BatchP& emissions,
+                              void* loss_dev, BatchP* targets_out, double* host_ms);
+void batch_ctc_step_fusion(bool on);
+void batch_ctc_step_stats(int64_t* fwd_fused, int64_t* fwd_unfused, int64_t* seed_fused, int64_t* seed_launched);
 void batch_backward(const BatchP& root, bool retain);
 void batch_items_host(const BatchP& x, float* out);
 void batch_items_device(const BatchP& x, void* dev_out);
diff --git a/gtn_amd/csrc/capi.cpp b/gtn_amd/csrc/capi.cpp
--- a/gtn_amd/csrc/capi.cpp
+++ b/gtn_amd/csrc/capi.cpp
@@ -768,6 +768,22 @@
                                               gtnx_batch_t* out) {
   return guard([&] { *out = HB(batch_ctc_targets(labels, lengths, n, blank, cg != 0)); });
 }
+GTNX_API gtnx_status_t gtnx_batch_ctc_loss_forward(const int* labels, const int* lengths, int n, int blank, int target_grad,
+                                                   gtnx_batch_t emissions, void* loss_device, gtnx_batch_t* targets_out,
+                                                   gtnx_batch_t* losses_out, double* host_ms) {
+  return guard([&] {
+    BatchP targets;
+    BatchP losses = batch_ctc_loss_forward(labels, lengths, n, blank, target_grad != 0, BH(emissions), loss_device, &targets, host_ms);
+    if (targets_out) *targets_out = HB(targets);
+    *losses_out = HB(losses);
+  });
+}
+GTNX_API gtnx_status_t gtnx_batch_ctc_step_fusion(int on) {
+  return guard([&] { batch_ctc_step_fusion(on != 0); });
+}
+GTNX_API gtnx_status_t gtnx_batch_ctc_step_stats(int64_t* stats4) {
+  return guard([&] { batch_ctc_step_stats(stats4, stats4 + 1, stats4 + 2, stats4 + 3); });
+}
 GTNX_API gtnx_status_t gtnx_batch_asg_force_align(const int* labels, const int* lengths, int n, gtnx_graph_t transitions,
                                                   int n_labels, gtnx_batch_t* out) {
   return guard([&] { *out = HB(batch_asg_force_align(labels, lengths, n, G(transitions), n_labels)); });
diff --git a/gtn_amd/csrc/kernels.h b/gtn_amd/csrc/kernels.h
--- a/gtn_amd/csrc/kernels.h
+++ b/gtn_amd/csrc/kernels.h
@@ -388,6 +388,21 @@
   GTNX_G float* grad_em;
   GTNX_G float* grad_fixed;
   int64_t A;
+  float cs, cn;
+  GTNX_G float* seed_root;
+  GTNX_G float* seed_score;
+  GTNX_G float* seed_norm;
+  float seed_cn;
+  int pad;
+};
+struct CtcTargetArgs;
+struct BandHead {
+  int on;
+  int blank;
+  const GTNX_G CtcTargetArgs* args;
+  GTNX_G float* loss;
+  GTNX_G BandPair* table;
+  int64_t lab_shift;
 };
 struct BandDecode {
   const GTNX_G BandNode* nodes;
@@ -501,7 +516,7 @@
 int band_forward_lgrn(int C);
 bool band_one_ok(int npl, int C, int max_NS, bool vec, bool backward);
 void launch_band_forward(const BandPair* d_pairs, int n, int npl, int C, int max_NS, bool unit, bool vec, hipStream_t st,
-                         const BandPair* one = nullptr);
+                         const BandPair* one = nullptr, const BandHead* head = nullptr);
 void launch_band_backward(const BandPair* d_pairs, int n, int npl, int C, int max_NS, bool unit, bool gradg, bool vec,
                           hipStream_t st, const BandPair* one = nullptr, const BandPatch* patch = nullptr);
 void launch_lazy_dense_prep(const LazyGroup& g, float* E, float* cmax, hipStream_t st);
diff --git a/gtn_amd/csrc/ops.h b/gtn_amd/csrc/ops.h
--- a/gtn_amd/csrc/ops.h
+++ b/gtn_amd/csrc/ops.h
@@ -45,6 +45,9 @@
                  double prof_bytes = 0.0, DevMemP* table_out = nullptr);
 void band_launch_patched(const DevMemP& table, int n, const BandLaunchKey& key, int max_ns, const BandPatch& patch,
                          const char* prof_name, double prof_bytes);
+
+void band_launch_headed(const DevMemP& table, int n, const BandLaunchKey& key, int max_ns, const BandHead& head,
+                        const char* prof_name, double prof_bytes);
 
 enum ScalarKind { SK_NEGATE = 0, SK_ADD = 1, SK_SUBTRACT = 2 };
 
diff --git a/gtn_amd/csrc/ops_band.cpp b/gtn_amd/csrc/ops_band.cpp
--- a/gtn_amd/csrc/ops_band.cpp
+++ b/gtn_amd/csrc/ops_band.cpp
@@ -11,6 +11,12 @@
   std::unique_ptr<Runtime::Scope> prof(prof_name ? new Runtime::Scope(&rt, prof_name, prof_bytes) : nullptr);
   launch_band_backward(table->as<BandPair>(), n, k.npl, k.C, max_ns, k.unit != 0, k.gradg != 0, k.vec != 0, rt.stream(), nullptr,
                        &patch);
+}
+void band_launch_headed(const DevMemP& table, int n, const BandLaunchKey& k, int max_ns, const BandHead& head,
+                        const char* prof_name, double prof_bytes) {
+  Runtime& rt = Runtime::get();
+  std::unique_ptr<Runtime::Scope> prof(prof_name ? new Runtime::Scope(&rt, prof_name, prof_bytes) : nullptr);
+  launch_band_forward(table->as<BandPair>(), n, k.npl, k.C, max_ns, k.unit != 0, k.vec != 0, rt.stream(), nullptr, &head);
 }
 void band_launch(std::vector<std::pair<BandLaunchKey, BandPair>>& tab, bool backward, const char* prof_name, double prof_bytes,
                  DevMemP* table_out) {
diff --git a/gtn_amd/csrc/runtime.cpp b/gtn_amd/csrc/runtime.cpp
--- a/gtn_amd/csrc/runtime.cpp
+++ b/gtn_amd/csrc/runtime.cpp
@@ -608,12 +608,16 @@
   }
   HIP_CHECK(hipMemcpyAsync(pinned_dst, src, bytes, hipMemcpyDeviceToHost, stream_));
 }
-void Runtime::h2d_pinned(void* dst, const void* pinned_src, size_t bytes) {
-  if (!bytes) return;
+size_t Runtime::h2d_kernel_limit() {
   static const size_t lim = [] {
     const char* e = std::getenv("GTNX_H2D_KERNEL_BYTES");
     return e ? size_t(std::atol(e)) : size_t(1) << 20;
   }();
+  return lim;
+}
+void Runtime::h2d_pinned(void* dst, const void* pinned_src, size_t bytes) {
+  if (!bytes) return;
+  const size_t lim = h2d_kernel_limit();
   if (bytes <= lim && local_to(dst, device_)) {
     launch_copy_small(dst, pinned_src, bytes, stream_);
     return;
diff --git a/gtn_amd/csrc/runtime.h b/gtn_amd/csrc/runtime.h
--- a/gtn_amd/csrc/runtime.h
+++ b/gtn_amd/csrc/runtime.h
@@ -92,6 +92,7 @@
   void d2h_sync(void* dst, const void* src, size_t bytes);
   void d2d(void* dst, const void* src, size_t bytes);
   void h2d_pinned(void* dst, const void* pinned_src, size_t bytes);
+  static size_t h2d_kernel_limit();
   void d2h_pinned_async(void* pinned_dst, const void* src, size_t bytes);
 
   struct MirrorSlot {
diff --git a/include/gtn/batch.h b/include/gtn/batch.h
--- a/include/gtn/batch.h
+++ b/include/gtn/batch.h
@@ -123,6 +123,14 @@
                          float* scoresDevice = nullptr, const int* frames = nullptr) {
   detail::check(gtnx_batch_viterbi_align(product.handle(), frames, labelsDevice, rowStride, tokensDevice, scoresDevice));
 }
+inline Batch ctcLossForward(const int* labels, const int* lengths, int n, int blank, bool targetGrad, const Batch& emissions,
+                            void* lossDevice = nullptr, Batch* targetsOut = nullptr, double* hostMs = nullptr) {
+  gtnx_batch_t targets = nullptr, losses = nullptr;
+  detail::check(gtnx_batch_ctc_loss_forward(labels, lengths, n, blank, targetGrad, emissions.handle(), lossDevice,
+                                            targetsOut ? &targets : nullptr, &losses, hostMs));
+  if (targetsOut) *targetsOut = Batch::fromHandle(targets);
+  return Batch::fromHandle(losses);
+}
 inline void backward(const Batch& a, bool retainGraph = false) { detail::check(gtnx_batch_backward(a.handle(), retainGraph)); }
 }
 
diff --git a/include/gtn_amd.h b/include/gtn_amd.h
--- a/include/gtn_amd.h
+++ b/include/gtn_amd.h
@@ -133,6 +133,11 @@
 gtnx_status_t gtnx_batch_from_graphs(const gtnx_graph_t* g, int n, gtnx_batch_t* out);
 gtnx_status_t gtnx_batch_ctc_targets(const int* labels, const int* lengths, int n, int blank, int calc_grad,
                                      gtnx_batch_t* out);
+gtnx_status_t gtnx_batch_ctc_loss_forward(const int* labels, const int* lengths, int n, int blank, int target_grad,
+                                          gtnx_batch_t emissions, void* loss_device, gtnx_batch_t* targets_out,
+                                          gtnx_batch_t* losses_out, double* host_ms);
+gtnx_status_t gtnx_batch_ctc_step_fusion(int on);
+gtnx_status_t gtnx_batch_ctc_step_stats(int64_t* stats4);
 gtnx_status_t gtnx_batch_asg_force_align(const int* labels, const int* lengths, int n, gtnx_graph_t transitions,
                                          int n_labels, gtnx_batch_t* out);
 gtnx_status_t gtnx_batch_linear(int n, int M, int N, int calc_grad, const void* device_weights, int borrow,
```

Result: faster. 948,900 losses/s (median of 6 runs) (+1.4%).
